# falcon-xu/DeViT

Measured on AMD Instinct MI355X. Metric: images/sec distill_sub step (DeiT-B->dedeit, bs256, 224^2), higher is better.
Workload: dtype bf16; 1 GPU; distill_sub step dedeit<-deit_base_distilled_patch16_224, num_division=4 (C=25), bs=256/GPU, 224x224, hard distillation, drop_path 0.1, AdamW+EMA; classes=25, global_batch=256, parallelism=dp1

## Files before the change

### devit_amd/_lib.py

```python
import ctypes as C
import os

import torch

_HERE = os.path.dirname(os.path.abspath(__file__))
LIB_PATH = os.environ.get("DEVIT_LIB_PATH") or os.path.join(_HERE, "libdevit_hip.so")

EPI_STORE_BF16, EPI_GELU_BF16, EPI_RESIDUAL_F32, EPI_PATCH_F32, EPI_DGELU_BF16, EPI_ATOMIC_F32, EPI_STORE_F32 = range(7)


class Epilogue(C.Structure):
    _fields_ = [("kind", C.c_int), ("out", C.c_void_p), ("ldc", C.c_int), ("bias", C.c_void_p),
                ("colscale", C.c_void_p), ("aux", C.c_void_p), ("aux_in", C.c_void_p), ("res", C.c_void_p),
                ("rowscale", C.c_void_p), ("rows_per_scale", C.c_int), ("pos", C.c_void_p),
                ("patch_tokens", C.c_int), ("extra_tokens", C.c_int), ("exact_gelu", C.c_int),
                ("out_batch_stride", C.c_longlong), ("m_valid", C.c_int), ("dtype16", C.c_int)]


class Operand(C.Structure):
    _fields_ = [("ptr", C.c_void_p), ("ld", C.c_int), ("kmajor", C.c_int), ("row_group", C.c_int),
                ("row_skip", C.c_int), ("batch_stride", C.c_longlong)]


ACT_LN1, ACT_MEAN1, ACT_RSTD1, ACT_QKV, ACT_ATTN_O, ACT_LSE, ACT_X1, ACT_ATT, ACT_LN2, ACT_MEAN2, ACT_RSTD2, ACT_H, ACT_H_PRE, \
    ACT_X2, ACT_COUNT = range(15)
BLK_SAVE, BLK_QKV_PAD, BLK_ATT = 1, 2, 4
BWD_DH_PRE, BWD_DLN2, BWD_DX1, BWD_G1, BWD_DATTN, BWD_DQKV, BWD_DLN1, BWD_LNWS, BWD_COUNT = range(9)


class BlockWeights(C.Structure):
    _fields_ = [(n, C.c_void_p) for n in ("n1w", "n1b", "qkv_b", "proj_b", "n2w", "n2b", "fc1_b", "fc2_b", "qkv_w16",
                                          "proj_w16", "fc1_w16", "fc2_w16", "head_gate", "neuron_gate")] + \
               [("num_heads", C.c_int), ("attn_width", C.c_int), ("hidden", C.c_int), ("dtype16", C.c_int), ("fc2_w16t", C.c_void_p)]


class BlockWgrads(C.Structure):
    _fields_ = [(n, C.c_void_p) for n in ("n1w", "n1b", "qkv_w", "qkv_b", "proj_w", "proj_b", "n2w", "n2b", "fc1_w",
                                          "fc1_b", "fc2_w", "fc2_b")]


class BlockActs(C.Structure):
    _fields_ = [("x", C.c_void_p), ("buf", C.c_void_p * 14), ("dp1", C.c_void_p), ("dp2", C.c_void_p), ("flags", C.c_int)]


class BlockBwdIO(C.Structure):
    _fields_ = [("dx", C.c_void_p), ("g2", C.c_void_p), ("dx_in", C.c_void_p), ("g_prev", C.c_void_p),
                ("prev_dp2", C.c_void_p), ("prev_fc2_b_grad", C.c_void_p), ("g2_bias_done", C.c_int),
                ("dqkv_add", C.c_void_p), ("ws", C.c_void_p * 8), ("lnws_bytes", C.c_size_t),
                ("defer_jobs", C.c_void_p), ("defer_count", C.c_void_p)]


class IndexJob(C.Structure):
    _fields_ = [("src", C.c_void_p), ("dst", C.c_void_p), ("idx", C.c_void_p), ("rows", C.c_int), ("cols", C.c_int),
                ("src_ld", C.c_int), ("dst_ld", C.c_int), ("mode", C.c_int), ("elem", C.c_int)]


class WgradJob(C.Structure):
    _fields_ = [("a", C.c_void_p), ("lda", C.c_int), ("a_cols", C.c_int), ("b", C.c_void_p), ("ldb", C.c_int), ("out", C.c_void_p),
                ("ldc", C.c_int), ("transposed", C.c_int), ("a_colsum", C.c_void_p)]


WGRAD_MAX_JOBS = 48
ABI_VERSION = 2
ABI_STRUCTS = {0: Epilogue, 1: Operand, 2: BlockWeights, 3: BlockWgrads, 4: BlockActs, 5: BlockBwdIO, 6: IndexJob, 7: WgradJob}


class DevitError(RuntimeError):
    pass


_P, _I, _F, _Z, _LL = C.c_void_p, C.c_int, C.c_float, C.c_size_t, C.c_longlong

SIGNATURES = {
    "devit_version": (_I, []),
    "devit_last_error": (C.c_char_p, []),
    "devit_check_device": (_I, [_I]),
    "devit_abi_struct_size": (_Z, [_I]),
    "devit_gemm_full_row_selected": (_I, [_I, _I, _I, _I]),
    "devit_wgrad_grouped": (_I, [C.POINTER(WgradJob), _I, _I, _I, _P]),
    "devit_gemm_bf16": (_I, [C.POINTER(Operand), C.POINTER(Operand), _I, _I, _I, _I, _I, C.POINTER(Epilogue), _P]),
    "devit_set_reserved_cus": (_I, [_I]),
    "devit_get_reserved_cus": (_I, []),
    "devit_layernorm_fwd": (_I, [_P, _I, _I, _I, _I, _P, _P, _F, _P, _P, _P, _P, _I, _P]),
    "devit_layernorm_bwd_workspace": (_Z, [_I, _I]),
    "devit_layernorm_bwd": (_I, [_P, _I, _P, _I, _I, _I, _I, _P, _P, _P, _P, _P, _P, _P, _I, _P, _P, _P, _I, _P, _Z, _P]),
    "devit_block_acts_sizes": (_I, [_I, _I, _I, _I, _I, _I, C.POINTER(C.c_size_t)]),
    "devit_block_bwd_sizes": (_I, [_I, _I, _I, _I, _I, C.POINTER(C.c_size_t)]),
    "devit_encoder_fwd": (_I, [_I, C.POINTER(BlockWeights), C.POINTER(BlockActs), _I, _I, _I, _F, _P]),
    "devit_block_bwd": (_I, [C.POINTER(BlockWeights), C.POINTER(BlockActs), C.POINTER(BlockWgrads), C.POINTER(BlockBwdIO),
                             _I, _I, _I, _F, _P]),
    "devit_attn_fwd": (_I, [_P, _P, _P, _P, _I, _I, _I, _I, _F, _I, _P]),
    "devit_attn_bwd": (_I, [_P, _P, _P, _P, _P, _P, _P, _I, _I, _I, _I, _F, _P]),
    "devit_attn_fwd_rows": (_I, [_P, _I, _P, _I, _P, _P, _P, _I, _I, _I, _I, _I, _F, _I, _P]),
    "devit_attn_bwd_rows": (_I, [_P, _I, _P, _I, _P, _P, _P, _P, _P, _I, _P, _I, _I, _I, _I, _I, _I, _F, _P]),
    "devit_index_copy": (_I, [_P, _I, _I, _P]),
    "devit_im2row_bf16": (_I, [_P, _P, _I, _I, _I, _I, _I, _I, _P]),
    "devit_mix_im2row_bf16": (_I, [_P, _P, _P, _I, _I, C.c_double, _I, _I, _I, _I, _P]),
    "devit_mix_targets": (_I, [_P, _P, _I, _I, C.c_double, C.c_double, _P]),
    "devit_embed_tokens": (_I, [_P, _P, _P, _P, _I, _I, _I, _P]),
    "devit_embed_bwd": (_I, [_P, _I, _I, _I, _I, _P, _P, _P, _P, _P, _I, _P]),
    "devit_cast_bf16": (_I, [_P, _P, _Z, _I, _P]),
    "devit_scale_cast_bf16": (_I, [_P, _P, _P, _I, _I, _I, _P]),
    "devit_colsum_workspace": (_Z, [_I, _I]),
    "devit_colsum_bf16": (_I, [_P, _I, _I, _I, _I, _I, _P, _I, _P, _Z, _P]),
    "devit_sgemm_small": (_I, [_P, _LL, _LL, _P, _LL, _LL, _P, _P, _I, _I, _I, _I, _F, _I, _P]),
    "devit_sumsq_workspace": (_Z, []),
    "devit_sumsq_f32": (_I, [_P, _Z, _P, _P, _Z, _P]),
    "devit_adamw_step": (_I, [_P, _P, _P, _P, _P, _P, _P, _P, _P, _Z, _F, _F, _F, _F, _F, _F, _F, _P]),
    "devit_cls_distill_loss": (_I, [_P, _P, _P, _P, _I, _I, _I, _F, _F, _P, _P, _P, _P]),
    "devit_token_mse": (_I, [_P, _P, _Z, _P, _P, _I, _P]),
    "devit_relation_stats": (_I, [_P, _P, _I, _I, _I, _I, _I, _P, _P, _P, _P, _P]),
    "devit_relation_grad": (_I, [_P, _P, _P, _P, _P, _I, _I, _I, _I, _I, _P, _I, _P]),
    "devit_gemm_f32": (_I, [_P, _LL, _LL, _LL, _LL, _P, _LL, _LL, _LL, _LL, _I, _I, _I, _I, _I, _LL, _LL, _I, _I, _F, _P, _I,
                            C.POINTER(Epilogue), _P]),
    "devit_softmax_rows_f32": (_I, [_P, _I, _I, _I, _F, _P, _P]),
    "devit_softmax_bwd_rows_f32": (_I, [_P, _P, _I, _I, _I, _F, _P]),
    "devit_im2row_f32": (_I, [_P, _P, _I, _P]),
    "devit_scale_rows_f32": (_I, [_P, _P, _P, _I, _I, _I, _P]),
    "devit_colsum_f32": (_I, [_P, _I, _I, _I, _P, _I, _P]),
    "devit_comm_unique_id": (_I, [_P]),
    "devit_comm_init": (_I, [_P, _I, _I, C.POINTER(C.c_void_p)]),
    "devit_comm_allreduce_f32": (_I, [_P, _P, _Z, _P]),
    "devit_comm_destroy": (_I, [_P]),
}

_lib = None
_checked_devices = set()


def load():
    global _lib
    if _lib is None:
        if not os.path.exists(LIB_PATH):
            raise DevitError(
                f"{LIB_PATH} not found: build it with `python -c 'import __graft_entry__ as g; g.build()'` "
                "(or devit_amd/csrc/build.sh).  devit_amd has no CPU / PyTorch fallback.")
        lib = C.CDLL(LIB_PATH)
        for name, (res, args) in SIGNATURES.items():
            fn = getattr(lib, name)
            fn.restype, fn.argtypes = res, args
        if lib.devit_version() != ABI_VERSION:
            raise DevitError(f"libdevit_hip.so ABI version {lib.devit_version()} != {ABI_VERSION} of this binding: rebuild (devit_amd/csrc/build.sh)")
        for which, cls in ABI_STRUCTS.items():
            if lib.devit_abi_struct_size(which) != C.sizeof(cls):
                raise DevitError(f"libdevit_hip.so: sizeof struct {which} = {lib.devit_abi_struct_size(which)}, the binding's {cls.__name__} has "
                                 f"{C.sizeof(cls)} bytes: header and binding disagree")
        _lib = lib
    return _lib


def require_device(t: torch.Tensor):
    if not t.is_cuda:
        raise DevitError("devit_amd ops run on MI355X (gfx950) only; got a %s tensor. There is no CPU fallback "
                         "(the CPU restatement lives in oracle/ and is test infrastructure)." % t.device)
    idx = t.device.index if t.device.index is not None else torch.cuda.current_device()
    if idx not in _checked_devices:
        call("devit_check_device", idx)
        _checked_devices.add(idx)


def call(name, *args):
    lib = load()
    rc = getattr(lib, name)(*args)
    if rc != 0:
        raise DevitError(f"{name} failed ({rc}): {lib.devit_last_error().decode()}")
    return rc


def stream_ptr():
    return C.c_void_p(torch.cuda.current_stream().cuda_stream)


def ptr(t):
    return None if t is None else C.c_void_p(t.data_ptr())
```

### devit_amd/csrc/devit_common.h

```cpp
#pragma once
#include <hip/hip_runtime.h>
#include <stdint.h>

#include "../../include/devit_hip.h"

typedef __attribute__((ext_vector_type(8))) __bf16 bf16x8;
typedef __attribute__((ext_vector_type(4))) __bf16 bf16x4;
typedef __attribute__((ext_vector_type(2))) __bf16 bf16x2;
typedef __attribute__((ext_vector_type(4))) short short4v;
typedef __attribute__((ext_vector_type(4))) float f32x4;
typedef __attribute__((ext_vector_type(2))) float f32x2;

#define LDS_PTR(p) ((__attribute__((address_space(3))) void*)(p))
#define GLB_PTR(p) ((const __attribute__((address_space(1))) void*)(p))

void devit_set_error(const char* fmt, ...);
#define DEVIT_CHECK(cond, code, ...)      \
  do {                                    \
    if (!(cond)) {                        \
      devit_set_error(__VA_ARGS__);       \
      return (code);                      \
    }                                     \
  } while (0)
#define DEVIT_LAUNCH_CHECK()                                            \
  do {                                                                  \
    hipError_t e__ = hipGetLastError();                                 \
    if (e__ != hipSuccess) {                                            \
      devit_set_error("%s:%d launch failed: %s", __FILE__, __LINE__,    \
                      hipGetErrorString(e__));                          \
      return DEVIT_ERR_LAUNCH;                                          \
    }                                                                   \
  } while (0)


__device__ __forceinline__ float bf2f(__bf16 v) { return (float)v; }
__device__ __forceinline__ __bf16 f2bf(float v) { return (__bf16)v; }

__device__ __forceinline__ float wave_sum(float v) {
#pragma unroll
  for (int o = 32; o > 0; o >>= 1) v += __shfl_xor(v, o, 64);
  return v;
}
__device__ __forceinline__ float wave_max(float v) {
#pragma unroll
  for (int o = 32; o > 0; o >>= 1) v = fmaxf(v, __shfl_xor(v, o, 64));
  return v;
}

constexpr float GELU_C0 = 1.59500523f, GELU_C1 = 7.40208836e-2f, GELU_C2 = -7.04591421e-4f;
constexpr float LOG2E = 1.44269504088896341f;
template <bool EXACT>
__device__ __forceinline__ float gelu_fwd(float x) {
  if (EXACT) return 0.5f * x * (1.0f + erff(x * 0.70710678118654752f));
  const float x2 = fminf(x * x, 36.0f);
  const float p = fmaf(fmaf(-GELU_C2 * LOG2E, x2, -GELU_C1 * LOG2E), x2, -GELU_C0 * LOG2E);
  const float t = __builtin_amdgcn_exp2f(x * p);
  return x * __builtin_amdgcn_rcpf(1.0f + t);
}
template <bool EXACT>
__device__ __forceinline__ float gelu_bwd(float x) {
  if (EXACT) {
    const float pdf = 0.3989422804014327f * __expf(-0.5f * x * x);
    return 0.5f * (1.0f + erff(x * 0.70710678118654752f)) + x * pdf;
  }
  const float x2 = fminf(x * x, 36.0f);
  const float p = fmaf(fmaf(-GELU_C2 * LOG2E, x2, -GELU_C1 * LOG2E), x2, -GELU_C0 * LOG2E);
  const float q = fmaf(fmaf(5.0f * GELU_C2, x2, 3.0f * GELU_C1), x2, GELU_C0);
  const float s = __builtin_amdgcn_rcpf(1.0f + __builtin_amdgcn_exp2f(x * p));
  return fmaf(x * fmaf(-s, s, s), q, s);
}

__device__ __forceinline__ void store16_stream(void* p, f32x4 v) { *(f32x4*)p = v; }
__device__ __forceinline__ void store8_stream(void* p, bf16x4 v) { *(bf16x4*)p = v; }
template <typename T>
__device__ __forceinline__ T load_stream(const T* p) {
  return __builtin_nontemporal_load(p);
}

__device__ __forceinline__ f32x4 mfma16(bf16x8 a, bf16x8 b, f32x4 c) {
  return __builtin_amdgcn_mfma_f32_16x16x32_bf16(a, b, c, 0, 0, 0);
}

typedef __attribute__((ext_vector_type(8))) _Float16 f16x8;
typedef __attribute__((ext_vector_type(4))) _Float16 f16x4;
template <bool F16>
__device__ __forceinline__ f32x4 mfma16t(bf16x8 a, bf16x8 b, f32x4 c) {
  if constexpr (F16)
    return __builtin_amdgcn_mfma_f32_16x16x32_f16(__builtin_bit_cast(f16x8, a), __builtin_bit_cast(f16x8, b), c, 0, 0, 0);
  else
    return __builtin_amdgcn_mfma_f32_16x16x32_bf16(a, b, c, 0, 0, 0);
}
template <bool F16>
__device__ __forceinline__ bf16x4 cvt4(f32x4 v) {
  if constexpr (F16) {
    const f16x4 h = {(_Float16)v[0], (_Float16)v[1], (_Float16)v[2], (_Float16)v[3]};
    return __builtin_bit_cast(bf16x4, h);
  } else {
    return (bf16x4){f2bf(v[0]), f2bf(v[1]), f2bf(v[2]), f2bf(v[3])};
  }
}
template <bool F16>
__device__ __forceinline__ bf16x8 cvt8(f32x4 a, f32x4 b) {
  if constexpr (F16) {
    const f16x8 h = {(_Float16)a[0], (_Float16)a[1], (_Float16)a[2], (_Float16)a[3],
                     (_Float16)b[0], (_Float16)b[1], (_Float16)b[2], (_Float16)b[3]};
    return __builtin_bit_cast(bf16x8, h);
  } else {
    return (bf16x8){f2bf(a[0]), f2bf(a[1]), f2bf(a[2]), f2bf(a[3]), f2bf(b[0]), f2bf(b[1]), f2bf(b[2]), f2bf(b[3])};
  }
}

template <typename V>
__device__ __forceinline__ void swap_half_rows(V& a, V& b, bool hi) {
  static_assert(sizeof(V) == 16, "16-byte chunks");
  typedef unsigned u32x4 __attribute__((ext_vector_type(4)));
  const u32x4 ua = __builtin_bit_cast(u32x4, a), ub = __builtin_bit_cast(u32x4, b);
  u32x4 recv;
#pragma unroll
  for (int e = 0; e < 4; ++e) {
    const unsigned send = hi ? ua[e] : ub[e];
    recv[e] = __builtin_amdgcn_update_dpp(0u, send, 0x128 , 0xf, 0xf, false);
  }
  u32x4 oa, obb;
#pragma unroll
  for (int e = 0; e < 4; ++e) {
    oa[e] = hi ? recv[e] : ua[e];
    obb[e] = hi ? ub[e] : recv[e];
  }
  a = __builtin_bit_cast(V, oa);
  b = __builtin_bit_cast(V, obb);
}

__device__ __forceinline__ bf16x4 lds_tr_read(const void* lds_addr) {
  short4v v = __builtin_amdgcn_ds_read_tr16_b64_v4i16((__attribute__((address_space(3))) short4v*)(lds_addr));
  return __builtin_bit_cast(bf16x4, v);
}
__device__ __forceinline__ bf16x8 cat8(bf16x4 lo, bf16x4 hi) {
  return __builtin_shufflevector(lo, hi, 0, 1, 2, 3, 4, 5, 6, 7);
}
```

### devit_amd/csrc/encoder.hip

```cpp
#include <mutex>

#include "devit_common.h"

namespace {

inline int pad_rows(int m) { return (m + 255) / 256 * 256; }
inline size_t align256(size_t b) { return (b + 255) / 256 * 256; }

inline int split_k_for(int out_rows, int out_cols, int ksteps) {
  const int tiles = (out_rows / 128) * (out_cols / 128);
  int s = 512 / (tiles > 0 ? tiles : 1);
  if (s > ksteps) s = ksteps;
  return s < 1 ? 1 : s;
}

struct Ctx {
  int M, Mp, B, N, D;
  float eps;
  void* stream;
};

int zero_pad(const Ctx& c, void* buf, int cols, size_t elem, int extra_rows = 0) {
  if (!buf) return DEVIT_OK;
  const int rows = c.Mp + extra_rows - c.M;
  if (rows <= 0) return DEVIT_OK;
  hipError_t e = hipMemsetAsync((char*)buf + (size_t)c.M * cols * elem, 0, (size_t)rows * cols * elem, (hipStream_t)c.stream);
  DEVIT_CHECK(e == hipSuccess, DEVIT_ERR_LAUNCH, "hipMemsetAsync: %s", hipGetErrorString(e));
  return DEVIT_OK;
}

devit_epilogue make_ep(int kind, void* out, int ldc, int m_valid, int dtype16 = 0) {
  devit_epilogue ep = {};
  ep.kind = kind;
  ep.out = out;
  ep.ldc = ldc;
  ep.m_valid = m_valid;
  ep.dtype16 = dtype16;
  return ep;
}

int linear_fwd(const Ctx& c, const void* x, const void* w, int Nout, int K, devit_epilogue ep) {
  devit_operand A = {x, K, 0, 0, 0, 0}, Bo = {w, K, 0, 0, 0, 0};
  return devit_gemm_bf16(&A, &Bo, c.Mp, Nout, K, 1, 1, &ep, c.stream);
}
int linear_dgrad(const Ctx& c, const void* dy, const void* w, int Nw, int K, devit_epilogue ep) {
  devit_operand A = {dy, Nw, 0, 0, 0, 0}, Bo = {w, K, 1, 0, 0, 0};
  return devit_gemm_bf16(&A, &Bo, c.Mp, K, Nw, 1, 1, &ep, c.stream);
}
int linear_wgrad(const Ctx& c, const void* dy, const void* x, float* w_grad, float* b_grad, int Nw, int K) {
  devit_operand A = {dy, Nw, 1, 0, 0, 0}, Bo = {x, K, 1, 0, 0, 0};
  devit_epilogue ep = make_ep(DEVIT_EPI_ATOMIC_F32, w_grad, K, 0);
  ep.aux = b_grad;
  return devit_gemm_bf16(&A, &Bo, Nw, K, c.Mp, 1, split_k_for(Nw, K, c.Mp / 64), &ep, c.stream);
}

bool wgrad_job(devit_wgrad_job* j, const void* dy, const void* x, float* w_grad, float* b_grad, int Nw, int K) {
  if (K == 384 && Nw % 128 == 0) {
    *j = devit_wgrad_job{dy, Nw, Nw, x, K, w_grad, K, 0, b_grad};
    return true;
  }
  if (Nw == 384 && K % 128 == 0 && b_grad == nullptr) {
    *j = devit_wgrad_job{x, K, K, dy, Nw, w_grad, K, 1, nullptr};
    return true;
  }
  return false;
}
int wgrad_mode() {
  const char* e = getenv("DEVIT_WGRADFR");
  return (e && *e) ? atoi(e) != 0 : 1;
}

#define TRY(x)                 \
  do {                         \
    int rc__ = (x);            \
    if (rc__ != DEVIT_OK) return rc__; \
  } while (0)

struct WgradSide {
  hipStream_t stream;
  hipEvent_t ev[5];
  bool ok = false;
};
constexpr int MAX_DEVICES = 16;
int wgrad_side(WgradSide** out) {
  const char* env = getenv("DEVIT_WGRAD_STREAM");
  const bool on = !(env && atoi(env) == 0);
  static WgradSide per_dev[MAX_DEVICES];
  static std::once_flag once[MAX_DEVICES];
  *out = nullptr;
  if (!on) return DEVIT_OK;
  int dev = 0;
  DEVIT_CHECK(hipGetDevice(&dev) == hipSuccess && dev >= 0, DEVIT_ERR_DEVICE, "devit_block_bwd: hipGetDevice");
  if (dev >= MAX_DEVICES) return DEVIT_OK;
  std::call_once(once[dev], [dev]() {
    WgradSide& s = per_dev[dev];
    if (hipStreamCreateWithFlags(&s.stream, hipStreamNonBlocking) != hipSuccess) return;
    for (auto& e : s.ev)
      if (hipEventCreateWithFlags(&e, hipEventDisableTiming) != hipSuccess) return;
    s.ok = true;
  });
  DEVIT_CHECK(per_dev[dev].ok, DEVIT_ERR_DEVICE, "devit_block_bwd: cannot create the weight-gradient stream / its events");
  *out = &per_dev[dev];
  return DEVIT_OK;
}

int check_dims(int B, int N, int D, int Da, int Hd) {
  DEVIT_CHECK(B > 0 && N > 0 && N <= 208 && D > 0 && D % 128 == 0 && Da > 0 && Da % 128 == 0 && Hd > 0 && Hd % 128 == 0,
              DEVIT_ERR_SHAPE, "block: B=%d N=%d D=%d attn_width=%d hidden=%d not supported", B, N, D, Da, Hd);
  return DEVIT_OK;
}

int block_fwd(const Ctx& c, const devit_block_weights& w, const devit_block_acts& a) {
  const int D = c.D, Da = w.attn_width, Hd = w.hidden, H = w.num_heads;
  TRY(check_dims(c.B, c.N, D, Da, Hd));
  DEVIT_CHECK(H > 0 && Da == H * 64, DEVIT_ERR_SHAPE, "block: attn_width %d != heads %d * 64", Da, H);
  const bool save = a.flags & DEVIT_BLK_SAVE;
  const int t16 = w.dtype16;
  DEVIT_CHECK(t16 == 0 || (t16 == 1 && !save), DEVIT_ERR_ARG,
              "devit_encoder_fwd: dtype16 = %d; f16 is the frozen-teacher forward (no DEVIT_BLK_SAVE: the backward kernels are bf16)", t16);
  void* const* b = a.buf;
  DEVIT_CHECK(a.x && b[DEVIT_ACT_LN1] && b[DEVIT_ACT_QKV] && b[DEVIT_ACT_ATTN_O] && b[DEVIT_ACT_X1] && b[DEVIT_ACT_LN2] &&
                  b[DEVIT_ACT_H] && b[DEVIT_ACT_X2],
              DEVIT_ERR_ARG, "devit_encoder_fwd: null activation buffer");
  DEVIT_CHECK(!save || (b[DEVIT_ACT_MEAN1] && b[DEVIT_ACT_RSTD1] && b[DEVIT_ACT_LSE] && b[DEVIT_ACT_MEAN2] &&
                        b[DEVIT_ACT_RSTD2] && b[DEVIT_ACT_H_PRE]),
              DEVIT_ERR_ARG, "devit_encoder_fwd: DEVIT_BLK_SAVE needs the mean/rstd/lse/h_pre buffers");
  DEVIT_CHECK(!(a.flags & DEVIT_BLK_ATT) || b[DEVIT_ACT_ATT], DEVIT_ERR_ARG, "devit_encoder_fwd: DEVIT_BLK_ATT needs att");
  TRY(zero_pad(c, b[DEVIT_ACT_LN1], D, 2));
  TRY(zero_pad(c, b[DEVIT_ACT_QKV], 3 * Da, 2, (a.flags & DEVIT_BLK_QKV_PAD) ? 128 : 0));
  TRY(zero_pad(c, b[DEVIT_ACT_ATTN_O], Da, 2));
  TRY(zero_pad(c, b[DEVIT_ACT_LN2], D, 2));
  TRY(zero_pad(c, b[DEVIT_ACT_H], Hd, 2));
  if (save) TRY(zero_pad(c, b[DEVIT_ACT_H_PRE], Hd, 2));
  TRY(devit_layernorm_fwd(a.x, c.M, D, 0, 0, w.n1w, w.n1b, c.eps, b[DEVIT_ACT_LN1], nullptr,
                          save ? (float*)b[DEVIT_ACT_MEAN1] : nullptr, save ? (float*)b[DEVIT_ACT_RSTD1] : nullptr, t16, c.stream));
  {
    devit_epilogue ep = make_ep(DEVIT_EPI_STORE_BF16, b[DEVIT_ACT_QKV], 3 * Da, c.M, t16);
    ep.bias = w.qkv_b;
    TRY(linear_fwd(c, b[DEVIT_ACT_LN1], w.qkv_w16, 3 * Da, D, ep));
  }
  TRY(devit_attn_fwd(b[DEVIT_ACT_QKV], b[DEVIT_ACT_ATTN_O], save ? (float*)b[DEVIT_ACT_LSE] : nullptr, w.head_gate, c.B, c.N, H,
                     64, 0.125f, t16, c.stream));
  {
    devit_epilogue ep = make_ep(DEVIT_EPI_RESIDUAL_F32, b[DEVIT_ACT_X1], D, c.M, t16);
    ep.bias = w.proj_b;
    ep.res = a.x;
    ep.rowscale = a.dp1;
    ep.rows_per_scale = c.N;
    ep.aux = (a.flags & DEVIT_BLK_ATT) ? b[DEVIT_ACT_ATT] : nullptr;
    TRY(linear_fwd(c, b[DEVIT_ACT_ATTN_O], w.proj_w16, D, Da, ep));
  }
  TRY(devit_layernorm_fwd((const float*)b[DEVIT_ACT_X1], c.M, D, 0, 0, w.n2w, w.n2b, c.eps, b[DEVIT_ACT_LN2], nullptr,
                          save ? (float*)b[DEVIT_ACT_MEAN2] : nullptr, save ? (float*)b[DEVIT_ACT_RSTD2] : nullptr, t16, c.stream));
  {
    devit_epilogue ep = make_ep(DEVIT_EPI_GELU_BF16, b[DEVIT_ACT_H], Hd, c.M, t16);
    ep.bias = w.fc1_b;
    ep.colscale = w.neuron_gate;
    ep.aux = save ? b[DEVIT_ACT_H_PRE] : nullptr;
    TRY(linear_fwd(c, b[DEVIT_ACT_LN2], w.fc1_w16, Hd, D, ep));
  }
  {
    devit_epilogue ep = make_ep(DEVIT_EPI_RESIDUAL_F32, b[DEVIT_ACT_X2], D, c.M, t16);
    ep.bias = w.fc2_b;
    ep.res = (const float*)b[DEVIT_ACT_X1];
    ep.rowscale = a.dp2;
    ep.rows_per_scale = c.N;
    if (w.fc2_w16t && !t16 && devit_gemm_full_row_selected(c.Mp, D, Hd, DEVIT_EPI_RESIDUAL_F32)) {
      devit_operand A = {b[DEVIT_ACT_H], Hd, 0, 0, 0, 0}, Bo = {w.fc2_w16t, D, 1, 0, 0, 0};
      TRY(devit_gemm_bf16(&A, &Bo, c.Mp, D, Hd, 1, 1, &ep, c.stream));
    } else {
      TRY(linear_fwd(c, b[DEVIT_ACT_H], w.fc2_w16, D, Hd, ep));
    }
  }
  return DEVIT_OK;
}

}

extern "C" int devit_block_acts_sizes(int B, int N, int D, int Da, int Hd, int flags, size_t* sizes) {
  DEVIT_CHECK(sizes != nullptr, DEVIT_ERR_ARG, "devit_block_acts_sizes: null");
  TRY(check_dims(B, N, D, Da, Hd));
  const size_t M = (size_t)B * N, Mp = pad_rows((int)M);
  const bool save = flags & DEVIT_BLK_SAVE;
  sizes[DEVIT_ACT_LN1] = Mp * D * 2;
  sizes[DEVIT_ACT_MEAN1] = sizes[DEVIT_ACT_RSTD1] = sizes[DEVIT_ACT_MEAN2] = sizes[DEVIT_ACT_RSTD2] = save ? M * 4 : 0;
  sizes[DEVIT_ACT_QKV] = (Mp + ((flags & DEVIT_BLK_QKV_PAD) ? 128 : 0)) * 3 * (size_t)Da * 2;
  sizes[DEVIT_ACT_ATTN_O] = Mp * Da * 2;
  sizes[DEVIT_ACT_LSE] = save ? (size_t)B * (Da / 64) * N * 4 : 0;
  sizes[DEVIT_ACT_X1] = M * D * 4;
  sizes[DEVIT_ACT_ATT] = (flags & DEVIT_BLK_ATT) ? M * D * 2 : 0;
  sizes[DEVIT_ACT_LN2] = Mp * D * 2;
  sizes[DEVIT_ACT_H] = Mp * Hd * 2;
  sizes[DEVIT_ACT_H_PRE] = save ? Mp * Hd * 2 : 0;
  sizes[DEVIT_ACT_X2] = M * D * 4;
  for (int i = 0; i < DEVIT_ACT_COUNT; ++i) sizes[i] = align256(sizes[i]);
  return DEVIT_OK;
}

extern "C" int devit_block_bwd_sizes(int B, int N, int D, int Da, int Hd, size_t* sizes) {
  DEVIT_CHECK(sizes != nullptr, DEVIT_ERR_ARG, "devit_block_bwd_sizes: null");
  TRY(check_dims(B, N, D, Da, Hd));
  const size_t M = (size_t)B * N, Mp = pad_rows((int)M);
  sizes[DEVIT_BWD_DH_PRE] = Mp * Hd * 2;
  sizes[DEVIT_BWD_DLN2] = sizes[DEVIT_BWD_G1] = sizes[DEVIT_BWD_DLN1] = Mp * D * 2;
  sizes[DEVIT_BWD_DATTN] = Mp * (size_t)Da * 2;
  sizes[DEVIT_BWD_DX1] = M * D * 4;
  sizes[DEVIT_BWD_DQKV] = Mp * 3 * (size_t)Da * 2;
  sizes[DEVIT_BWD_LNWS] = devit_layernorm_bwd_workspace((int)M, D);
  for (int i = 0; i < DEVIT_BWD_COUNT; ++i) sizes[i] = align256(sizes[i]);
  return DEVIT_OK;
}

extern "C" int devit_encoder_fwd(int nblocks, const devit_block_weights* w, const devit_block_acts* acts, int B, int N, int D,
                                 float eps, void* stream) {
  DEVIT_CHECK(nblocks > 0 && w && acts, DEVIT_ERR_ARG, "devit_encoder_fwd: bad argument");
  Ctx c{B * N, pad_rows(B * N), B, N, D, eps, stream};
  for (int i = 0; i < nblocks; ++i) {
    DEVIT_CHECK(i == 0 || acts[i].x == (const float*)acts[i - 1].buf[DEVIT_ACT_X2], DEVIT_ERR_ARG,
                "devit_encoder_fwd: block %d does not read block %d's output", i, i - 1);
    TRY(block_fwd(c, w[i], acts[i]));
  }
  return DEVIT_OK;
}

extern "C" int devit_block_bwd(const devit_block_weights* wp, const devit_block_acts* ap, const devit_block_wgrads* gp,
                               const devit_block_bwd_io* io, int B, int N, int D, float eps, void* stream) {
  DEVIT_CHECK(wp && ap && gp && io, DEVIT_ERR_ARG, "devit_block_bwd: null argument");
  const devit_block_weights& w = *wp;
  const devit_block_acts& a = *ap;
  const devit_block_wgrads& g = *gp;
  const int Hd = w.hidden, H = w.num_heads, Da = w.attn_width;
  TRY(check_dims(B, N, D, Da, Hd));
  DEVIT_CHECK(H > 0 && Da == H * 64, DEVIT_ERR_SHAPE, "devit_block_bwd: attn_width %d != heads %d * 64", Da, H);
  DEVIT_CHECK(a.flags & DEVIT_BLK_SAVE, DEVIT_ERR_ARG, "devit_block_bwd: the forward ran without DEVIT_BLK_SAVE");
  DEVIT_CHECK(w.dtype16 == 0, DEVIT_ERR_ARG, "devit_block_bwd: f16 blocks have no backward");
  DEVIT_CHECK(io->dx && io->g2 && io->dx_in, DEVIT_ERR_ARG, "devit_block_bwd: dx / g2 / dx_in");
  for (int i = 0; i < DEVIT_BWD_COUNT; ++i) DEVIT_CHECK(io->ws[i], DEVIT_ERR_ARG, "devit_block_bwd: workspace %d is null", i);
  DEVIT_CHECK(g.n1w && g.n1b && g.qkv_w && g.qkv_b && g.proj_w && g.proj_b && g.n2w && g.n2b && g.fc1_w && g.fc1_b &&
                  g.fc2_w && g.fc2_b, DEVIT_ERR_ARG, "devit_block_bwd: null gradient accumulator");
  Ctx c{B * N, pad_rows(B * N), B, N, D, eps, stream};
  WgradSide* sd = nullptr;
  TRY(wgrad_side(&sd));
  Ctx cs = c;
  bool forked = false;
  auto fork = [&](int i) -> int {
    if (!sd) return DEVIT_OK;
    DEVIT_CHECK(hipEventRecord(sd->ev[i], (hipStream_t)stream) == hipSuccess && hipStreamWaitEvent(sd->stream, sd->ev[i], 0) == hipSuccess,
                DEVIT_ERR_LAUNCH, "devit_block_bwd: cannot fork the weight-gradient stream");
    cs.stream = sd->stream;
    forked = true;
    return DEVIT_OK;
  };
  const int rc = [&]() -> int {
  void* const* b = a.buf;
  void* dh_pre = io->ws[DEVIT_BWD_DH_PRE];
  void* dln2 = io->ws[DEVIT_BWD_DLN2];
  float* dx1 = (float*)io->ws[DEVIT_BWD_DX1];
  void* g1 = io->ws[DEVIT_BWD_G1];
  void* dattn = io->ws[DEVIT_BWD_DATTN];
  void* dqkv = io->ws[DEVIT_BWD_DQKV];
  void* dln1 = io->ws[DEVIT_BWD_DLN1];
  TRY(zero_pad(c, dh_pre, Hd, 2));
  TRY(zero_pad(c, dln2, D, 2));
  TRY(zero_pad(c, g1, D, 2));
  TRY(zero_pad(c, dattn, Da, 2));
  TRY(zero_pad(c, dqkv, 3 * Da, 2));
  TRY(zero_pad(c, dln1, D, 2));
  TRY(zero_pad(c, io->g_prev, D, 2));
  const int wmode = (D == 384 && c.Mp / 64 >= 3) ? wgrad_mode() : 0;
  if (io->defer_count) *io->defer_count = 0;
  devit_wgrad_job jobs[4];
  int nj = 0;
  auto wgrad = [&](int ev, const void* dy, const void* x, float* w_grad, float* b_grad, int Nw, int K) -> int {
    if (wmode && wgrad_job(&jobs[nj], dy, x, w_grad, b_grad, Nw, K)) {
      ++nj;
      return DEVIT_OK;
    }
    TRY(fork(ev));
    return linear_wgrad(cs, dy, x, w_grad, b_grad, Nw, K);
  };
  auto flush = [&](int ev) -> int {
    if (io->defer_jobs) {
      for (int i = 0; i < nj; ++i) io->defer_jobs[i] = jobs[i];
      if (io->defer_count) *io->defer_count = nj;
      nj = 0;
      return DEVIT_OK;
    }
    if (nj == 0) return DEVIT_OK;
    TRY(fork(ev));
    const int n = nj;
    nj = 0;
    return devit_wgrad_grouped(jobs, n, c.Mp, 0, cs.stream);
  };
  bool fc2_bias_here = !io->g2_bias_done;
  if (fc2_bias_here && wmode && Hd % 128 == 0 && io->lnws_bytes >= devit_colsum_workspace(c.Mp, D)) {
    TRY(devit_colsum_bf16(io->g2, c.Mp, D, D, 0, 0, g.fc2_b, 1, io->ws[DEVIT_BWD_LNWS], io->lnws_bytes, stream));
    fc2_bias_here = false;
  }
  TRY(wgrad(0, io->g2, b[DEVIT_ACT_H], g.fc2_w, fc2_bias_here ? g.fc2_b : nullptr, D, Hd));
  {
    devit_epilogue ep = make_ep(DEVIT_EPI_DGELU_BF16, dh_pre, Hd, c.M);
    ep.colscale = w.neuron_gate;
    ep.aux_in = b[DEVIT_ACT_H_PRE];
    TRY(linear_dgrad(c, io->g2, w.fc2_w16, D, Hd, ep));
  }
  TRY(linear_dgrad(c, dh_pre, w.fc1_w16, Hd, D, make_ep(DEVIT_EPI_STORE_BF16, dln2, D, c.M)));
  TRY(wgrad(1, dh_pre, b[DEVIT_ACT_LN2], g.fc1_w, g.fc1_b, Hd, D));
  TRY(devit_layernorm_bwd(dln2, 0, (const float*)b[DEVIT_ACT_X1], c.M, D, 0, 0, (const float*)b[DEVIT_ACT_MEAN2],
                          (const float*)b[DEVIT_ACT_RSTD2], w.n2w, io->dx, dx1, g1, a.dp1, N, g.n2w, g.n2b, g.proj_b, 1,
                          io->ws[DEVIT_BWD_LNWS], io->lnws_bytes, stream));
  TRY(linear_dgrad(c, g1, w.proj_w16, D, Da, make_ep(DEVIT_EPI_STORE_BF16, dattn, Da, c.M)));
  TRY(wgrad(2, g1, b[DEVIT_ACT_ATTN_O], g.proj_w, nullptr, D, Da));
  TRY(devit_attn_bwd(b[DEVIT_ACT_QKV], b[DEVIT_ACT_ATTN_O], dattn, (const float*)b[DEVIT_ACT_LSE], w.head_gate, io->dqkv_add,
                     dqkv, B, N, H, 64, 0.125f, stream));
  TRY(linear_dgrad(c, dqkv, w.qkv_w16, 3 * Da, D, make_ep(DEVIT_EPI_STORE_BF16, dln1, D, c.M)));
  TRY(wgrad(3, dqkv, b[DEVIT_ACT_LN1], g.qkv_w, g.qkv_b, 3 * Da, D));
  TRY(flush(3));
  TRY(devit_layernorm_bwd(dln1, 0, a.x, c.M, D, 0, 0, (const float*)b[DEVIT_ACT_MEAN1], (const float*)b[DEVIT_ACT_RSTD1],
                          w.n1w, dx1, io->dx_in, io->g_prev, io->prev_dp2, N, g.n1w, g.n1b,
                          io->g_prev ? io->prev_fc2_b_grad : nullptr, 1, io->ws[DEVIT_BWD_LNWS], io->lnws_bytes, stream));
  return DEVIT_OK;
  }();
  if (sd && forked) {
    const bool joined = hipEventRecord(sd->ev[4], sd->stream) == hipSuccess && hipStreamWaitEvent((hipStream_t)stream, sd->ev[4], 0) == hipSuccess;
    if (rc == DEVIT_OK) DEVIT_CHECK(joined, DEVIT_ERR_LAUNCH, "devit_block_bwd: cannot join the weight-gradient stream");
  }
  return rc;
}
```

### devit_amd/csrc/gemm.hip

```cpp
#include <stdlib.h>

#include <type_traits>

#include "devit_common.h"

namespace {

constexpr int BK = 64;
#ifndef DEVIT_PP_SPREAD
#define DEVIT_PP_SPREAD 0
#endif
#ifndef DEVIT_PP_SPLIT
#define DEVIT_PP_SPLIT 1
#endif
#ifndef DEVIT_PP_MFMA_AT
#define DEVIT_PP_MFMA_AT 1
#endif
#ifdef DEVIT_DMA_A_NT
constexpr bool DMA_A_NT = true;
#else
constexpr bool DMA_A_NT = false;
#endif
#ifdef DEVIT_DMA_B_NT
constexpr bool DMA_B_NT = true;
#else
constexpr bool DMA_B_NT = false;
#endif
#ifndef DEVIT_RAGGED_MIN_K
#define DEVIT_RAGGED_MIN_K 384
#endif

struct FastDiv {
  unsigned mul, shift;
  int d;
};
__host__ inline FastDiv make_fastdiv(int d) {
  FastDiv f;
  f.d = d;
  unsigned s = 0;
  while ((1ll << s) < d) ++s;
  f.shift = 31 + s;
  f.mul = (unsigned)(((1ull << f.shift) / (unsigned long long)d) + 1ull);
  return f;
}
__device__ __forceinline__ int fdiv(int n, const FastDiv& f) {
  return (int)(((unsigned long long)(unsigned)n * f.mul) >> f.shift);
}

struct GemmArgs {
  const __bf16* A;
  const __bf16* B;
  int lda, ldb;
  int a_group, a_skip, b_group, b_skip;
  long long a_bs, b_bs;
  int M, N, K;
  int tiles_m, tiles_n, split_k, total_tiles;
  FastDiv d_per_z, d_chunk, d_gn, d_last, d_split;
  int gn;
  devit_epilogue ep;
};

__device__ __forceinline__ int phys_row(int r, int group, int skip) {
  return group > 0 ? r + skip * (r / group + 1) : r;
}

__device__ __forceinline__ int swz_row(int row) { return ((row >> 1) & 7) ^ (((row >> 4) & 1) << 1); }
__device__ __forceinline__ int swz_krow(int krow) { return ((krow & 3) << 2) | (((krow >> 3) & 1) << 1); }

template <bool KM, int W, int NWAVES>
__device__ __forceinline__ unsigned lane_offset(int ld, int wave, int lane, int i, int valid) {
  constexpr int CNT = (W / 8) / NWAVES;
  const int slab = wave * CNT + i;
  if (!KM) {
    const int row = slab * 8 + (lane >> 3);
    const int chunk = (lane & 7) ^ swz_row(row);
    return (unsigned)(min(row, valid - 1) * ld + chunk * 8) * 2u;
  } else {
    constexpr int LPR = W / 8, RPS = 64 / LPR;
    const int krow = slab * RPS + lane / LPR;
    const int chunk = (lane % LPR) ^ swz_krow(krow);
    return (unsigned)(krow * ld + min(chunk, valid / 8 - 1) * 8) * 2u;
  }
}

template <bool NT = false>
__device__ __forceinline__ void dma2_uniform(const char* ubase, unsigned off0, unsigned off1, unsigned lds) {
  unsigned keep;
  if (NT) {
    asm volatile(
        "s_mov_b32 %0, m0\n\t"
        "s_mov_b32 m0, %1\n\t"
        "s_nop 2\n\t"
        "global_load_lds_dwordx4 %3, %2 nt\n\t"
        "s_add_u32 m0, %1, 0x400\n\t"
        "s_nop 0\n\t"
        "global_load_lds_dwordx4 %4, %2 nt\n\t"
        "s_mov_b32 m0, %0"
        : "=&s"(keep)
        : "s"(lds), "s"(ubase), "v"(off0), "v"(off1)
        : "memory", "scc");
    return;
  }
  asm volatile(
      "s_mov_b32 %0, m0\n\t"
      "s_mov_b32 m0, %1\n\t"
      "s_nop 2\n\t"
      "global_load_lds_dwordx4 %3, %2\n\t"
      "s_add_u32 m0, %1, 0x400\n\t"
      "s_nop 0\n\t"
      "global_load_lds_dwordx4 %4, %2\n\t"
      "s_mov_b32 m0, %0"
      : "=&s"(keep)
      : "s"(lds), "s"(ubase), "v"(off0), "v"(off1)
      : "memory", "scc");
}
__device__ __forceinline__ void dma2_perlane(const void* p0, const void* p1, unsigned lds) {
  unsigned keep;
  asm volatile(
      "s_mov_b32 %0, m0\n\t"
      "s_mov_b32 m0, %1\n\t"
      "s_nop 2\n\t"
      "global_load_lds_dwordx4 %2, off\n\t"
      "s_add_u32 m0, %1, 0x400\n\t"
      "s_nop 0\n\t"
      "global_load_lds_dwordx4 %3, off\n\t"
      "s_mov_b32 m0, %0"
      : "=&s"(keep)
      : "s"(lds), "v"(p0), "v"(p1)
      : "memory", "scc");
}

template <bool KM, int W, int NWAVES, bool NT = false>
__device__ __forceinline__ void stage_tile(const __bf16* org, int ld, int k0, int group, int skip,
                                           char* lds_tile, int wave, int lane, int valid = W, int only_pair = -1) {
  constexpr int CNT = (W / 8) / NWAVES;
  static_assert(CNT % 2 == 0, "slabs are issued in pairs");
  const unsigned lds0 = (unsigned)(size_t)LDS_PTR(lds_tile) + (unsigned)(wave * CNT) * 1024u;
  if (KM && group > 0) {
#pragma unroll
    for (int i = 0; i < CNT; i += 2) {
      const __bf16* src[2];
#pragma unroll
      for (int e = 0; e < 2; ++e) {
        constexpr int LPR = W / 8, RPS = 64 / LPR;
        const int slab = wave * CNT + i + e;
        const int krow = slab * RPS + lane / LPR;
        const int chunk = (lane % LPR) ^ swz_krow(krow);
        src[e] = org + (size_t)phys_row(k0 + krow, group, skip) * ld + chunk * 8;
      }
      dma2_perlane(src[0], src[1], lds0 + i * 1024u);
    }
    return;
  }
  const char* ubase = (const char*)org + (size_t)k0 * (KM ? (size_t)ld : (size_t)1) * 2;
#pragma unroll
  for (int i = 0; i < CNT; i += 2)
    if (only_pair < 0 || i == 2 * only_pair)
    dma2_uniform<NT>(ubase, lane_offset<KM, W, NWAVES>(ld, wave, lane, i, valid), lane_offset<KM, W, NWAVES>(ld, wave, lane, i + 1, valid),
                     lds0 + i * 1024u);
}

template <bool PAIRED>
__device__ __forceinline__ int tile_row(int j, int p) {
  return PAIRED ? 32 * (j >> 1) + 8 * (p >> 2) + 4 * (j & 1) + (p & 3) : 16 * j + p;
}

template <bool KM, int W, bool PAIRED>
__device__ __forceinline__ bf16x8 read_frag(const char* tile, int base, int j, int kk, int lane) {
  if (!KM) {
    const int row = base + tile_row<PAIRED>(j, lane & 15);
#ifdef DEVIT_GEMM_NOSWZ
    const int chunk = (kk * 4 + (lane >> 4));
#else
    const int chunk = (kk * 4 + (lane >> 4)) ^ swz_row(row);
#endif
    return *(const bf16x8*)(tile + row * 128 + chunk * 16);
  } else {
    const int G = lane >> 4, q = (lane >> 2) & 3, p = lane & 3;
    const int col0 = base + tile_row<PAIRED>(j, 4 * p);
    const int krow = kk * 32 + G * 8 + q;
    const int chunk = (col0 >> 3) ^ swz_krow(krow);
    const char* a = tile + krow * (W * 2) + chunk * 16 + ((col0 >> 2) & 1) * 8;
    return cat8(lds_tr_read(a), lds_tr_read(a + 4 * (W * 2)));
  }
}

template <int N>
__device__ __forceinline__ void wait_vmcnt() {
  asm volatile("s_waitcnt vmcnt(%0)" ::"n"(N) : "memory");
}

template <typename T>
__device__ __forceinline__ void st_out(T* p, T v) {
#ifdef DEVIT_GEMM_NOSTORE
  if (__builtin_expect(((size_t)p & 0xfffff0) == 0x7ffff0, 0))
#endif
  *p = v;
}

template <bool F16 = false>
__device__ __forceinline__ bf16x8 pack8(const float (&x)[8]) {
  if constexpr (F16) return cvt8<true>((f32x4){x[0], x[1], x[2], x[3]}, (f32x4){x[4], x[5], x[6], x[7]});
  typedef float f32x2 __attribute__((ext_vector_type(2)));
  typedef __bf16 bf16x2 __attribute__((ext_vector_type(2)));
  bf16x2 p[4];
#pragma unroll
  for (int e = 0; e < 4; ++e) p[e] = __builtin_convertvector((f32x2){x[2 * e], x[2 * e + 1]}, bf16x2);
  return (bf16x8){p[0][0], p[0][1], p[1][0], p[1][1], p[2][0], p[2][1], p[3][0], p[3][1]};
}

template <int KIND>
__device__ __forceinline__ void load_cols(const devit_epilogue& ep, int lane, int nw, int (&noff)[4], f32x4 (&bias)[4],
                                          f32x4 (&cs)[4]) {
  constexpr bool BF16_OUT = KIND == DEVIT_EPI_STORE_BF16 || KIND == DEVIT_EPI_GELU_BF16 || KIND == DEVIT_EPI_DGELU_BF16;
  constexpr bool SCALED = KIND == DEVIT_EPI_GELU_BF16 || KIND == DEVIT_EPI_DGELU_BF16;
#pragma unroll
  for (int j = 0; j < 4; ++j) {
    noff[j] = nw + tile_row<BF16_OUT>(j, 4 * (lane >> 4));
    if constexpr (KIND == DEVIT_EPI_DGELU_BF16) bias[j] = (f32x4){0.f, 0.f, 0.f, 0.f};
    else bias[j] = ep.bias ? *(const f32x4*)(ep.bias + noff[j]) : (f32x4){0.f, 0.f, 0.f, 0.f};
    if (SCALED) cs[j] = ep.colscale ? *(const f32x4*)(ep.colscale + noff[j]) : (f32x4){1.f, 1.f, 1.f, 1.f};
  }
}
template <int KIND>
__device__ __forceinline__ void settle_cols(f32x4 (&bias)[4], f32x4 (&cs)[4]) {
  constexpr bool SCALED = KIND == DEVIT_EPI_GELU_BF16 || KIND == DEVIT_EPI_DGELU_BF16;
#pragma unroll
  for (int j = 0; j < 4; ++j) {
    if (KIND != DEVIT_EPI_DGELU_BF16) asm volatile("" : "+v"(bias[j]));
    if (SCALED) asm volatile("" : "+v"(cs[j]));
  }
}

#ifndef DEVIT_F32_FULL_ROWS
#define DEVIT_F32_FULL_ROWS 1
#endif

template <int KIND, int MI, bool FULL, bool F16>
__device__ __forceinline__ void epilogue_f32_rows(const devit_epilogue& ep, f32x4 (&acc)[MI][4], const int (&noff)[4],
                                                  const f32x4 (&bias)[4], int lane, int mw, int m_lim, size_t ob) {
  constexpr int CHI = 2;
  const int c = lane & 15;
  const bool hi = c >= 8;
  const int colx = hi ? 16 : 0;
  auto row_off = [&](int m, int& tok) -> size_t {
    if (KIND == DEVIT_EPI_PATCH_F32) {
      const int b = m / ep.patch_tokens, t = m - b * ep.patch_tokens;
      tok = ep.extra_tokens + t;
      return ((size_t)b * (ep.patch_tokens + ep.extra_tokens) + tok) * ep.ldc;
    }
    tok = 0;
    return ob + (size_t)m * ep.ldc;
  };
#pragma unroll
  for (int i0 = 0; i0 < MI; i0 += CHI) {
    f32x4 gin[CHI][2][2];
    float rsc[CHI][2];
    size_t rowo[CHI][2];
    bool okr[CHI][2];
#pragma unroll
    for (int u = 0; u < CHI; ++u)
#pragma unroll
      for (int r = 0; r < 2; ++r) {
        const int m = mw + (i0 + u) * 16 + (c & 7) + 8 * r;
        const bool ok = FULL || m < m_lim;
        int tok;
        const size_t o = row_off(m, tok);
#pragma unroll
        for (int p = 0; p < 2; ++p) {
          const int col = noff[2 * p] + colx;
          if (KIND == DEVIT_EPI_PATCH_F32)
            gin[u][p][r] = ok ? *(const f32x4*)(ep.pos + (size_t)tok * ep.ldc + col) : (f32x4){0.f, 0.f, 0.f, 0.f};
          if (KIND == DEVIT_EPI_RESIDUAL_F32)
            gin[u][p][r] = ok ? load_stream((const f32x4*)(ep.res + o + col)) : (f32x4){0.f, 0.f, 0.f, 0.f};
        }
        if (KIND == DEVIT_EPI_RESIDUAL_F32) rsc[u][r] = (ok && ep.rowscale) ? ep.rowscale[m / ep.rows_per_scale] : 1.0f;
        rowo[u][r] = o;
        okr[u][r] = ok;
      }
#pragma unroll
    for (int u = 0; u < CHI; ++u) {
      const int i = i0 + u;
      f32x4 v[4];
#pragma unroll
      for (int j = 0; j < 4; ++j) v[j] = acc[i][j] + bias[j];
      if (KIND == DEVIT_EPI_RESIDUAL_F32 && ep.aux) {
        const int m = mw + i * 16 + c;
        if (FULL || m < m_lim) {
#pragma unroll
          for (int j = 0; j < 4; ++j) st_out((bf16x4*)((__bf16*)ep.aux + ob + (size_t)m * ep.ldc + noff[j]), cvt4<F16>(v[j]));
        }
      }
#pragma unroll
      for (int p = 0; p < 2; ++p) {
        swap_half_rows(v[2 * p], v[2 * p + 1], hi);
        const int col = noff[2 * p] + colx;
#pragma unroll
        for (int r = 0; r < 2; ++r) {
          f32x4 w = v[2 * p + r];
          if (KIND == DEVIT_EPI_PATCH_F32) w = w + gin[u][p][r];
          if (KIND == DEVIT_EPI_RESIDUAL_F32) w = gin[u][p][r] + rsc[u][r] * w;
          if (okr[u][r]) st_out((f32x4*)((float*)ep.out + rowo[u][r] + col), w);
        }
      }
    }
  }
}

template <int KIND, int MI, bool FULL, bool F16 = false>
__device__ __forceinline__ void epilogue_direct(const devit_epilogue& ep, f32x4 (&acc)[MI][4], const int (&noff)[4],
                                                const f32x4 (&bias)[4], const f32x4 (&cs)[4], int lane, int mw,
                                                int m_lim, size_t ob) {
  constexpr bool BF16_OUT = KIND == DEVIT_EPI_STORE_BF16 || KIND == DEVIT_EPI_GELU_BF16 || KIND == DEVIT_EPI_DGELU_BF16;
  if constexpr (!BF16_OUT && DEVIT_F32_FULL_ROWS) {
    epilogue_f32_rows<KIND, MI, FULL, F16>(ep, acc, noff, bias, lane, mw, m_lim, ob);
    return;
  }
  constexpr int CHI = 2;
  const int c = lane & 15;
#pragma unroll
  for (int i0 = 0; i0 < MI; i0 += CHI) {
    f32x4 gin[CHI][4];
    float rsc[CHI];
    bf16x8 pre[CHI][2];
    size_t rowo[CHI];
#pragma unroll
    for (int u = 0; u < CHI; ++u) {
      const int m = mw + (i0 + u) * 16 + c;
      const bool ok = FULL || m < m_lim;
      size_t o = ob + (size_t)m * ep.ldc;
      if (KIND == DEVIT_EPI_PATCH_F32) {
        const int b = m / ep.patch_tokens, t = m - b * ep.patch_tokens, tok = ep.extra_tokens + t;
        o = ((size_t)b * (ep.patch_tokens + ep.extra_tokens) + tok) * ep.ldc;
#pragma unroll
        for (int j = 0; j < 4; ++j)
          gin[u][j] = ok ? *(const f32x4*)(ep.pos + (size_t)tok * ep.ldc + noff[j]) : (f32x4){0.f, 0.f, 0.f, 0.f};
      }
      if (KIND == DEVIT_EPI_RESIDUAL_F32) {
#pragma unroll
        for (int j = 0; j < 4; ++j)
          gin[u][j] = ok ? load_stream((const f32x4*)(ep.res + o + noff[j])) : (f32x4){0.f, 0.f, 0.f, 0.f};
        rsc[u] = (ok && ep.rowscale) ? ep.rowscale[m / ep.rows_per_scale] : 1.0f;
      }
      if (KIND == DEVIT_EPI_DGELU_BF16) {
        const bf16x8 z = {0, 0, 0, 0, 0, 0, 0, 0};
#pragma unroll
        for (int q = 0; q < 2; ++q)
          pre[u][q] = ok ? load_stream((const bf16x8*)((const __bf16*)ep.aux_in + o + noff[2 * q])) : z;
      }
      rowo[u] = o;
    }
#pragma unroll
    for (int u = 0; u < CHI; ++u) {
      const int i = i0 + u;
      const bool ok = FULL || mw + i * 16 + c < m_lim;
      const size_t o = rowo[u];
      if constexpr (!BF16_OUT) {
#pragma unroll
        for (int j = 0; j < 4; ++j) {
          const f32x4 v = acc[i][j] + bias[j];
          if (KIND == DEVIT_EPI_STORE_F32) {
            if (ok) st_out((f32x4*)((float*)ep.out + o + noff[j]), v);
          } else if (KIND == DEVIT_EPI_PATCH_F32) {
            if (ok) st_out((f32x4*)((float*)ep.out + o + noff[j]), v + gin[u][j]);
          } else {
            if (ok) {
              if (ep.aux) {
                const bf16x4 pb = cvt4<F16>(v);
                st_out((bf16x4*)((__bf16*)ep.aux + o + noff[j]), pb);
              }
              st_out((f32x4*)((float*)ep.out + o + noff[j]), gin[u][j] + rsc[u] * v);
            }
          }
        }
      } else {
        bf16x8 outc[2], prec[2];
#pragma unroll
        for (int q = 0; q < 2; ++q) {
          float x[8];
#pragma unroll
          for (int e = 0; e < 8; ++e) x[e] = acc[i][2 * q + (e >> 2)][e & 3] + bias[2 * q + (e >> 2)][e & 3];
          if (KIND == DEVIT_EPI_GELU_BF16) {
            prec[q] = pack8<F16>(x);
#pragma unroll
            for (int e = 0; e < 8; ++e) x[e] = gelu_fwd<false>(x[e]) * cs[2 * q + (e >> 2)][e & 3];
          } else if (KIND == DEVIT_EPI_DGELU_BF16) {
#pragma unroll
            for (int e = 0; e < 8; ++e) x[e] = x[e] * cs[2 * q + (e >> 2)][e & 3] * gelu_bwd<false>(bf2f(pre[u][q][e]));
          }
          outc[q] = pack8<F16>(x);
        }
        const bool hi = c >= 8;
        const int mA = mw + i * 16 + (c & 7);
        const size_t oA = ob + (size_t)mA * ep.ldc + noff[0] + (hi ? 32 : 0), oB = oA + (size_t)8 * ep.ldc;
        const bool okA = FULL || mA < m_lim, okB = FULL || mA + 8 < m_lim;
        swap_half_rows(outc[0], outc[1], hi);
        if (KIND == DEVIT_EPI_GELU_BF16 && ep.aux) {
          swap_half_rows(prec[0], prec[1], hi);
          if (okA) st_out((bf16x8*)((__bf16*)ep.aux + oA), prec[0]);
          if (okB) st_out((bf16x8*)((__bf16*)ep.aux + oB), prec[1]);
        }
        if (okA) st_out((bf16x8*)((__bf16*)ep.out + oA), outc[0]);
        if (okB) st_out((bf16x8*)((__bf16*)ep.out + oB), outc[1]);
      }
    }
  }
}

__device__ __forceinline__ float sum8_bf16(bf16x8 v, float acc) {
  typedef __bf16 bf16x2v __attribute__((ext_vector_type(2)));
  const bf16x2v one = {(__bf16)1.0f, (__bf16)1.0f};
  acc = __builtin_amdgcn_fdot2_f32_bf16(__builtin_shufflevector(v, v, 0, 1), one, acc, false);
  acc = __builtin_amdgcn_fdot2_f32_bf16(__builtin_shufflevector(v, v, 2, 3), one, acc, false);
  acc = __builtin_amdgcn_fdot2_f32_bf16(__builtin_shufflevector(v, v, 4, 5), one, acc, false);
  acc = __builtin_amdgcn_fdot2_f32_bf16(__builtin_shufflevector(v, v, 6, 7), one, acc, false);
  return acc;
}

struct TileRef {
  const __bf16* a;
  const __bf16* b;
  int m0, n0, bz, kt0, nk;
};

template <int BM, int BN, bool A_KM, bool B_KM>
__device__ __forceinline__ TileRef decode_tile(const GemmArgs& g, int w) {
  const int zz = fdiv(w, g.d_per_z);
  const int r0 = w - zz * g.d_per_z.d;
  const int chunk = fdiv(r0, g.d_chunk);
  const int r1 = r0 - chunk * g.d_chunk.d;
  const bool lastc = (chunk + 1) * g.gn > g.tiles_n;
  const int tm = lastc ? fdiv(r1, g.d_last) : fdiv(r1, g.d_gn);
  const int tn = chunk * g.gn + r1 - tm * (lastc ? g.d_last.d : g.d_gn.d);
  const int bzq = fdiv(zz, g.d_split);
  const int z = zz - bzq * g.split_k, nk_total = g.K / BK;
  TileRef t;
  t.bz = bzq;
  t.m0 = tm * BM;
  t.n0 = tn * BN;
  t.kt0 = fdiv(z * nk_total, g.d_split);
  t.nk = fdiv((z + 1) * nk_total, g.d_split) - t.kt0;
  t.a = g.A + (size_t)t.bz * g.a_bs + (A_KM ? (size_t)t.m0 : (size_t)t.m0 * g.lda);
  t.b = g.B + (size_t)t.bz * g.b_bs + (B_KM ? (size_t)t.n0 : (size_t)t.n0 * g.ldb);
  return t;
}

template <int BM, int BN, int WAVES_M, int WAVES_N, int NSTAGE, bool A_KM, bool B_KM, int KIND, bool F16 = false>
__global__ __launch_bounds__(WAVES_M * WAVES_N * 64) __attribute__((amdgpu_waves_per_eu(2, 2)))
void gemm_kernel(const GemmArgs g) {
  static_assert(!F16 || (KIND != DEVIT_EPI_DGELU_BF16 && KIND != DEVIT_EPI_ATOMIC_F32 && !A_KM && !B_KM),
                "f16 operands: forward layouts / epilogues only (the frozen teacher has no backward)");
  extern __shared__ __attribute__((aligned(16))) char smem[];
  constexpr int NWAVES = WAVES_M * WAVES_N;
  constexpr int WM = BM / WAVES_M, WN = BN / WAVES_N, MI = WM / 16, NI = WN / 16;
  static_assert(WN == 64 && WM % 64 == 0, "wave tile must be (64 k) x 64");
  static_assert(NSTAGE == 2, "NSTAGE is the B ring depth; uniformly deeper rings at one workgroup per CU lost everywhere");
  constexpr bool DIRECT = KIND != DEVIT_EPI_ATOMIC_F32;
  constexpr bool PAIRED = KIND == DEVIT_EPI_STORE_BF16 || KIND == DEVIT_EPI_GELU_BF16 || KIND == DEVIT_EPI_DGELU_BF16;
  constexpr int A_TILE_BYTES = BM * BK * 2, B_TILE_BYTES = BN * BK * 2;
  constexpr bool PP = DIRECT && BM == 256 && BN == 256 && WAVES_M == 2;
  constexpr int NA = 3;
  constexpr int PER_A = (BM / 8) / NWAVES;
  constexpr int B_RING = NA * A_TILE_BYTES;
  const int tid = threadIdx.x, lane = tid & 63;
  const int wave = __builtin_amdgcn_readfirstlane(tid >> 6);
  const int wm = wave / WAVES_N, wn = wave % WAVES_N;
#ifdef DEVIT_GEMM_TSTAMP
  const unsigned long long t_entry = __builtin_amdgcn_s_memtime(), rt_entry = __builtin_amdgcn_s_memrealtime();
#endif

  const int xcd = blockIdx.x & 7, idx = blockIdx.x >> 3, stride = gridDim.x >> 3;
  int first, last;
  {
    const int q = g.total_tiles >> 3, r = g.total_tiles & 7;
    const int start = xcd * q + min(xcd, r);
    first = start + idx;
    last = start + q + (xcd < r ? 1 : 0);
  }
  if (first >= last) return;

  struct Cursor {
    TileRef ref;
    int tile, t;
    bool open;
  };
  Cursor pb{decode_tile<BM, BN, A_KM, B_KM>(g, first), first, 0, true};
  Cursor pa = pb;
  int a_slot = 0, b_slot = 0;
  bool a_last = false;
  auto step_cursor = [&](Cursor& c) {
    if (++c.t == c.ref.nk) {
      c.t = 0;
      c.tile += stride;
      if (DIRECT && c.tile < last) c.ref = decode_tile<BM, BN, A_KM, B_KM>(g, c.tile);
      else c.open = false;
    }
  };
  auto dma_a = [&](const Cursor& c) {
#ifdef DEVIT_GEMM_NODMA
    if (g.K < 0)
#endif
    stage_tile<A_KM, BM, NWAVES, DMA_A_NT>(c.ref.a, g.lda, (c.ref.kt0 + c.t) * BK, g.a_group, g.a_skip,
                                           smem + a_slot * A_TILE_BYTES, wave, lane);
    a_slot = a_slot + 1 == NA ? 0 : a_slot + 1;
  };
  auto dma_b = [&](const Cursor& c) {
#ifdef DEVIT_GEMM_NODMA
    if (g.K < 0)
#endif
    stage_tile<B_KM, BN, NWAVES, DMA_B_NT>(c.ref.b, g.ldb, (c.ref.kt0 + c.t) * BK, g.b_group, g.b_skip,
                                           smem + B_RING + b_slot * B_TILE_BYTES, wave, lane, min(BN, g.N - c.ref.n0));
    b_slot ^= 1;
  };
  auto issue_a = [&]() {
    a_last = pa.open;
    if (!pa.open) return;
    dma_a(pa);
    step_cursor(pa);
  };
  auto produce = [&]() {
    if (pb.open) {
      dma_b(pb);
      step_cursor(pb);
    }
    issue_a();
  };
  auto wait_stage = [&]() {
    if (a_last) wait_vmcnt<PER_A>();
    else wait_vmcnt<0>();
  };
  if constexpr (PP) {
    auto fence = [&]() {
      asm volatile("" ::: "memory");
      __builtin_amdgcn_sched_barrier(0);
    };
    auto bar = [&]() {
      fence();
      __builtin_amdgcn_s_barrier();
      fence();
    };
    issue_a();
    produce();
    wait_vmcnt<0>();
    bar();
#if DEVIT_PP_SPREAD
    auto dma_half = [&](Cursor& c, bool is_a, int h) {
      if (is_a) {
        stage_tile<A_KM, BM, NWAVES, DMA_A_NT>(c.ref.a, g.lda, (c.ref.kt0 + c.t) * BK, g.a_group, g.a_skip,
                                               smem + a_slot * A_TILE_BYTES, wave, lane, BM, h);
        if (h == 1) a_slot = a_slot + 1 == NA ? 0 : a_slot + 1;
      } else {
        stage_tile<B_KM, BN, NWAVES, DMA_B_NT>(c.ref.b, g.ldb, (c.ref.kt0 + c.t) * BK, g.b_group, g.b_skip,
                                               smem + B_RING + b_slot * B_TILE_BYTES, wave, lane, min(BN, g.N - c.ref.n0), h);
        if (h == 1) b_slot ^= 1;
      }
      if (h == 1) step_cursor(c);
    };
    auto slot_q = [&](auto qc) {
      constexpr int q = decltype(qc)::value;
      if (q == 0) { if (pb.open) dma_half(pb, false, 0); }
      if (q == 1) { if (pb.open) dma_half(pb, false, 1); }
      if (q == 2) { a_last = pa.open; if (pa.open) dma_half(pa, true, 0); }
      if (q == 3) { if (pa.open) dma_half(pa, true, 1); wait_stage(); }
    };
    auto spread_slot = [&](auto pc) {
      constexpr int p = decltype(pc)::value;
      if (wm == 0) slot_q(std::integral_constant<int, p>());
      else slot_q(std::integral_constant<int, (p + 1) & 3>());
    };
    if (wm == 1) slot_q(std::integral_constant<int, 0>());
#endif
    int ca_slot = 0, cb_slot = 0;
#ifdef DEVIT_GEMM_TSTAMP
    unsigned long long* tdbg = g.ep.pos ? (unsigned long long*)g.ep.pos + ((size_t)blockIdx.x * NWAVES + wave) * 48 : nullptr;
    int tcount = 0;
    if (tdbg && lane == 0) {
      tdbg[40] = t_entry;
      tdbg[42] = rt_entry;
      tdbg[44] = __builtin_amdgcn_s_memtime();
    }
#endif
    for (int tile = first; tile < last; tile += stride) {
      const TileRef ct = decode_tile<BM, BN, A_KM, B_KM>(g, tile);
      f32x4 acc[MI][NI];
#pragma unroll
      for (int i = 0; i < MI; ++i)
#pragma unroll
        for (int j = 0; j < NI; ++j) acc[i][j] = (f32x4){0.f, 0.f, 0.f, 0.f};
      const devit_epilogue& ep = g.ep;
      const int nw = ct.n0 + wn * WN;
#ifdef DEVIT_GEMM_TSTAMP
      if (tdbg && lane == 0 && tcount < 8) tdbg[tcount * 3 + 0] = __builtin_amdgcn_s_memtime();
#endif
      int noff[4];
      f32x4 bias[4], cs[4];
#ifdef DEVIT_GEMM_STAMP
      unsigned long long stamp[12];
#pragma unroll
      for (int q = 0; q < 12; ++q) stamp[q] = 0;
#define DEVIT_STAMP(q) do { if (t == 3 && tile == first) stamp[q] = __builtin_amdgcn_s_memtime(); } while (0)
#else
#define DEVIT_STAMP(q) do { } while (0)
#endif
      if (wm == 1) bar();
      for (int t = 0; t < ct.nk; ++t) {
        const char* cur_a = smem + ca_slot * A_TILE_BYTES;
        const char* cur_b = smem + B_RING + cb_slot * B_TILE_BYTES;
        ca_slot = ca_slot + 1 == NA ? 0 : ca_slot + 1;
        cb_slot ^= 1;
#if !DEVIT_PP_SPREAD && !DEVIT_PP_SPLIT
        produce();
#endif
        if (t == ct.nk - 1 && nw < g.N) load_cols<KIND>(ep, lane, nw, noff, bias, cs);
#pragma unroll
        for (int kk = 0; kk < 2; ++kk) {
          bf16x8 af[MI], bfr[NI];
#ifdef DEVIT_GEMM_NOREAD
#pragma unroll
          for (int j = 0; j < NI; ++j) asm volatile("" : "=v"(bfr[j]));
#pragma unroll
          for (int i = 0; i < MI; ++i) asm volatile("" : "=v"(af[i]));
#else
#pragma unroll
          for (int j = 0; j < NI; ++j) bfr[j] = read_frag<B_KM, BN, PAIRED>(cur_b, wn * WN, j, kk, lane);
#pragma unroll
          for (int i = 0; i < MI; ++i) af[i] = read_frag<A_KM, BM, false>(cur_a, wm * WM, i, kk, lane);
#endif
          DEVIT_STAMP(kk * 6 + 0);
#if DEVIT_PP_SPREAD
          fence();
          if (kk == 0) spread_slot(std::integral_constant<int, 0>());
          else spread_slot(std::integral_constant<int, 2>());
          fence();
#elif DEVIT_PP_SPLIT
          fence();
          if (kk == 0) {
            if (pb.open) {
              dma_b(pb);
              step_cursor(pb);
            }
          } else {
            issue_a();
            wait_stage();
          }
          fence();
#else
          if (kk == 1) wait_stage();
#endif
          DEVIT_STAMP(kk * 6 + 1);
          asm volatile("s_waitcnt lgkmcnt(0)" ::: "memory");
          DEVIT_STAMP(kk * 6 + 2);
          bar();
          DEVIT_STAMP(kk * 6 + 3);
#ifdef DEVIT_GEMM_NOMFMA
#pragma unroll
          for (int j = 0; j < NI; ++j) asm volatile("" ::"v"(bfr[j]));
#pragma unroll
          for (int i = 0; i < MI; ++i) asm volatile("" ::"v"(af[i]));
#else
#pragma unroll
          for (int i = 0; i < MI; ++i) {
#pragma unroll
            for (int j = 0; j < NI; ++j) acc[i][j] = mfma16t<F16>(bfr[j], af[i], acc[i][j]);
#if DEVIT_PP_SPREAD
            if (i == DEVIT_PP_MFMA_AT) {
              fence();
              if (kk == 0) spread_slot(std::integral_constant<int, 1>());
              else spread_slot(std::integral_constant<int, 3>());
              fence();
            }
#endif
          }
#endif
          DEVIT_STAMP(kk * 6 + 4);
          bar();
          DEVIT_STAMP(kk * 6 + 5);
        }
#ifdef DEVIT_GEMM_TSTAMP
        if (tdbg && lane == 0 && tcount == 1 && t < 16 && (g.M & 1)) tdbg[24 + t] = __builtin_amdgcn_s_memtime();
#endif
      }
#ifdef DEVIT_GEMM_TSTAMP
      if (tdbg && lane == 0 && tcount < 8) tdbg[tcount * 3 + 1] = __builtin_amdgcn_s_memtime();
#endif
      if (wm == 0) bar();
#ifdef DEVIT_GEMM_STAMP
      if (tile == first && lane == 0 && g.ep.pos != nullptr) {
        unsigned long long* dbg = (unsigned long long*)g.ep.pos + ((size_t)blockIdx.x * NWAVES + wave) * 12;
#pragma unroll
        for (int q = 0; q < 12; ++q) dbg[q] = stamp[q];
      }
#endif
      if (nw < g.N) {
        settle_cols<KIND>(bias, cs);
        const size_t ob = (size_t)ct.bz * ep.out_batch_stride;
        const int m_lim = ep.m_valid > 0 ? ep.m_valid : g.M;
        if (ct.m0 + BM <= m_lim) epilogue_direct<KIND, MI, true, F16>(ep, acc, noff, bias, cs, lane, ct.m0 + wm * WM, m_lim, ob);
        else epilogue_direct<KIND, MI, false, F16>(ep, acc, noff, bias, cs, lane, ct.m0 + wm * WM, m_lim, ob);
      }
#ifdef DEVIT_GEMM_TSTAMP
      if (tdbg && lane == 0 && tcount < 8) tdbg[tcount * 3 + 2] = __builtin_amdgcn_s_memtime();
      ++tcount;
#endif
    }
#ifdef DEVIT_GEMM_TSTAMP
    if (tdbg && lane == 0) {
      tdbg[41] = __builtin_amdgcn_s_memtime();
      tdbg[43] = __builtin_amdgcn_s_memrealtime();
      tdbg[45] = tcount;
    }
#endif
    return;
  }

  issue_a();
  produce();

  auto advance = [&]() {
    wait_stage();
    __builtin_amdgcn_s_barrier();
    produce();
  };

  int ca_slot = 0, cb_slot = 0;
  bool primed = false;
  for (int tile = first; tile < last; tile += stride) {
    const TileRef ct = decode_tile<BM, BN, A_KM, B_KM>(g, tile);
    f32x4 acc[MI][NI];
#pragma unroll
    for (int i = 0; i < MI; ++i)
#pragma unroll
      for (int j = 0; j < NI; ++j) acc[i][j] = (f32x4){0.f, 0.f, 0.f, 0.f};
    float rsum[MI];
#pragma unroll
    for (int i = 0; i < MI; ++i) rsum[i] = 0.f;
    const bool rowsum_on = KIND == DEVIT_EPI_ATOMIC_F32 && g.ep.aux != nullptr && wn == 0;
    int rs_wait = 0;
    if (rowsum_on) rs_wait = (ct.n0 / BN - ct.kt0 % g.tiles_n + g.tiles_n) % g.tiles_n;

    auto kstep = [&]() {
      const char* cur_a = smem + ca_slot * A_TILE_BYTES;
      const char* cur_b = smem + B_RING + cb_slot * B_TILE_BYTES;
      ca_slot = ca_slot + 1 == NA ? 0 : ca_slot + 1;
      cb_slot ^= 1;
      const bool rs_now = KIND == DEVIT_EPI_ATOMIC_F32 && rowsum_on && rs_wait == 0;
#ifdef DEVIT_GEMM_NOCOMPUTE
      if (g.K < 0)
#endif
#pragma unroll
      for (int kk = 0; kk < 2; ++kk) {
        bf16x8 af[MI], bfr[NI];
#pragma unroll
        for (int j = 0; j < NI; ++j) bfr[j] = read_frag<B_KM, BN, PAIRED>(cur_b, wn * WN, j, kk, lane);
#pragma unroll
        for (int i = 0; i < MI; ++i) af[i] = read_frag<A_KM, BM, false>(cur_a, wm * WM, i, kk, lane);
#pragma unroll
        for (int i = 0; i < MI; ++i)
#pragma unroll
          for (int j = 0; j < NI; ++j)
            acc[i][j] = DIRECT ? mfma16t<F16>(bfr[j], af[i], acc[i][j]) : mfma16t<F16>(af[i], bfr[j], acc[i][j]);
        if constexpr (KIND == DEVIT_EPI_ATOMIC_F32) {
          if (rs_now) {
#pragma unroll
            for (int i = 0; i < MI; ++i) rsum[i] = sum8_bf16(af[i], rsum[i]);
          }
        }
      }
      if constexpr (KIND == DEVIT_EPI_ATOMIC_F32) rs_wait = rs_wait == 0 ? g.tiles_n - 1 : rs_wait - 1;
    };
    const devit_epilogue& ep = g.ep;
    const int nw = ct.n0 + wn * WN;
    for (int t = 0; t < ct.nk - 1; ++t) {
      if (t > 0 || !primed) advance();
      kstep();
    }
    if (ct.nk > 1 || !primed) advance();
    int noff[4];
    f32x4 bias[4], cs[4];
    if constexpr (DIRECT) load_cols<KIND>(ep, lane, nw, noff, bias, cs);
    kstep();
    if constexpr (DIRECT) settle_cols<KIND>(bias, cs);
    primed = DIRECT && tile + stride < last;
    if (primed) advance();

    const size_t ob = (size_t)ct.bz * ep.out_batch_stride;
    const int m_lim = ep.m_valid > 0 ? ep.m_valid : g.M;
    if constexpr (DIRECT) {
      if (ct.m0 + BM <= m_lim) epilogue_direct<KIND, MI, true, F16>(ep, acc, noff, bias, cs, lane, ct.m0 + wm * WM, m_lim, ob);
      else epilogue_direct<KIND, MI, false, F16>(ep, acc, noff, bias, cs, lane, ct.m0 + wm * WM, m_lim, ob);
    } else {
      __syncthreads();
      float* cw = (float*)smem + wave * 4096;
      float* out = (float*)ep.out + ob;
      auto do_pass = [&](auto pass_c) {
        constexpr int pass = decltype(pass_c)::value;
#pragma unroll
        for (int i = 0; i < 4; ++i)
#pragma unroll
          for (int j = 0; j < 4; ++j)
#pragma unroll
            for (int r = 0; r < 4; ++r)
              cw[(i * 16 + (lane >> 4) * 4 + r) * 64 + j * 16 + (lane & 15)] = acc[pass * 4 + i][j][r];
        const int mw = ct.m0 + wm * WM + pass * 64;
        for (int row = 0; row < 64; ++row) {
          const float v = cw[row * 64 + lane];
#if defined(DEVIT_GEMM_NOATOMIC)
          if (mw + row < m_lim && v == 1.2345e30f) out[(size_t)(mw + row) * ep.ldc + nw + lane] = v;
#else
          if (mw + row < m_lim) unsafeAtomicAdd(out + (size_t)(mw + row) * ep.ldc + nw + lane, v);
#endif
        }
      };
      do_pass(std::integral_constant<int, 0>());
      if constexpr (MI > 4) do_pass(std::integral_constant<int, 1>());
      if (rowsum_on) {
        float* rs_out = (float*)ep.aux;
#pragma unroll
        for (int i = 0; i < MI; ++i) {
          float v = rsum[i];
          v += __shfl_xor(v, 16, 64);
          v += __shfl_xor(v, 32, 64);
          const int row = ct.m0 + wm * WM + i * 16 + lane;
          if (lane < 16 && row < m_lim) unsafeAtomicAdd(rs_out + row, v);
        }
      }
      if (pb.tile < last) {
        __syncthreads();
        pb.ref = decode_tile<BM, BN, A_KM, B_KM>(g, pb.tile);
        pb.t = 0;
        pb.open = true;
        pa = pb;
        a_slot = ca_slot;
        b_slot = cb_slot;
        issue_a();
        produce();
      }
    }
  }
}

#include "gemm4_kloop.inc"

template <int KIND, bool F16>
__global__ __launch_bounds__(256) __attribute__((amdgpu_waves_per_eu(1, 1)))
void gemm4_kernel(const GemmArgs g) {
  static_assert(KIND != DEVIT_EPI_ATOMIC_F32 && KIND != DEVIT_EPI_DGELU_BF16 && !F16, "forward layouts, DIRECT epilogues, bf16");
  extern __shared__ __attribute__((aligned(16))) char smem[];
  constexpr int BM = 256, BN = 256, NWAVES = 4;
  constexpr bool PAIRED = KIND == DEVIT_EPI_STORE_BF16 || KIND == DEVIT_EPI_GELU_BF16;
  constexpr int A_TILE_BYTES = BM * BK * 2, B_TILE_BYTES = BN * BK * 2, B_RING = 3 * A_TILE_BYTES;
  const int tid = threadIdx.x, lane = tid & 63;
  const int wave = __builtin_amdgcn_readfirstlane(tid >> 6);
  const int wm = wave >> 1, wn = wave & 1;

  const int xcd = blockIdx.x & 7, idx = blockIdx.x >> 3, stride = gridDim.x >> 3;
  int first, last;
  {
    const int q = g.total_tiles >> 3, r = g.total_tiles & 7;
    const int start = xcd * q + min(xcd, r);
    first = start + idx;
    last = start + q + (xcd < r ? 1 : 0);
  }
  if (first >= last) return;
#ifdef DEVIT_GEMM4_STAMP
  const unsigned long long t_entry = __builtin_amdgcn_s_memtime(), rt_entry = __builtin_amdgcn_s_memrealtime();
  unsigned long long st_sum[8] = {0, 0, 0, 0, 0, 0, 0, 0};
#endif

  const unsigned lda64 = (unsigned)g.lda * 64u, ldb64 = (unsigned)g.ldb * 64u;
  const unsigned wave_lds = (unsigned)(size_t)LDS_PTR(smem) + (unsigned)wave * 8192u;

  TileRef ct = decode_tile<BM, BN, false, false>(g, first);
#pragma unroll
  for (int st = 0; st < 2; ++st) {
    stage_tile<false, BM, NWAVES>(ct.a, g.lda, (ct.kt0 + st) * BK, 0, 0, smem + st * A_TILE_BYTES, wave, lane);
    stage_tile<false, BN, NWAVES>(ct.b, g.ldb, (ct.kt0 + st) * BK, 0, 0, smem + B_RING + st * B_TILE_BYTES, wave, lane);
  }
  wait_vmcnt<0>();
  __builtin_amdgcn_s_barrier();
  asm volatile("" ::: "memory");
  unsigned g3 = 0, g2 = B_RING;
  const unsigned wv = (unsigned)wave;

  for (int tile = first; tile < last; tile += stride) {
    const bool has_next = tile + stride < last;
    const TileRef nt = has_next ? decode_tile<BM, BN, false, false>(g, tile + stride) : ct;
    const __bf16* a_ptr = ct.a + (size_t)ct.kt0 * BK;
    const __bf16* b_ptr = ct.b + (size_t)ct.kt0 * BK;
    const __bf16* a_next = nt.a + (size_t)nt.kt0 * BK;
    const __bf16* b_next = nt.b + (size_t)nt.kt0 * BK;
    const unsigned nk = (unsigned)ct.nk;
    const devit_epilogue& ep = g.ep;
    unsigned dsA[4], dsB[4], dmaA[4], dmaB[4];
    {
      int lane_k;
      asm volatile("v_mbcnt_lo_u32_b32 %0, -1, 0\n\tv_mbcnt_hi_u32_b32 %0, -1, %0" : "=v"(lane_k));
      const int c = lane_k & 15, gq = lane_k >> 4;
  #pragma unroll
      for (int kk = 0; kk < 2; ++kk)
  #pragma unroll
        for (int par = 0; par < 2; ++par) {
          const int rowA = wm * 128 + 16 * par + c;
          dsA[kk * 2 + par] = (unsigned)(rowA * 128 + (((kk * 4 + gq) ^ swz_row(rowA)) * 16));
          const int rowB = wn * 128 + tile_row<PAIRED>(par, c);
          dsB[kk * 2 + par] = (unsigned)(rowB * 128 + (((kk * 4 + gq) ^ swz_row(rowB)) * 16));
        }
  #pragma unroll
      for (int i = 0; i < 4; ++i) {
        dmaA[i] = lane_offset<false, BM, NWAVES>(g.lda, wave, lane_k, i, BM);
        dmaB[i] = lane_offset<false, BN, NWAVES>(g.ldb, wave, lane_k, i, BN);
      }
    }
    unsigned t0, t1, t2, t3;
#ifdef DEVIT_GEMM4_STAMP
    unsigned d0, d1, d2, d3;
    const unsigned long long ts0 = __builtin_amdgcn_s_memtime();
    asm volatile(DEVIT_GEMM4_KLOOP_STAMPED_ASM
                 : [g3] "+s"(g3), [g2] "+s"(g2), [t0] "=&v"(t0), [t1] "=&v"(t1), [t2] "=&v"(t2), [t3] "=&v"(t3),
                   [d0] "=&s"(d0), [d1] "=&s"(d1), [d2] "=&s"(d2), [d3] "=&s"(d3)
                 : [aptr] "s"(a_ptr), [bptr] "s"(b_ptr), [anext] "s"(a_next), [bnext] "s"(b_next), [nk] "s"(nk),
                   [lda64] "s"(lda64), [ldb64] "s"(ldb64), [wlds] "s"(wave_lds), [wv] "s"(wv),
                   [dsa0] "v"(dsA[0]), [dsa1] "v"(dsA[1]), [dsa2] "v"(dsA[2]), [dsa3] "v"(dsA[3]),
                   [dsb0] "v"(dsB[0]), [dsb1] "v"(dsB[1]), [dsb2] "v"(dsB[2]), [dsb3] "v"(dsB[3]),
                   [dmaa0] "v"(dmaA[0]), [dmaa1] "v"(dmaA[1]), [dmaa2] "v"(dmaA[2]), [dmaa3] "v"(dmaA[3]),
                   [dmab0] "v"(dmaB[0]), [dmab1] "v"(dmaB[1]), [dmab2] "v"(dmaB[2]), [dmab3] "v"(dmaB[3])
                 : DEVIT_GEMM4_KLOOP_STAMPED_CLOBBERS);
    const unsigned long long ts1 = __builtin_amdgcn_s_memtime();
    st_sum[0] += 1; st_sum[1] += ts1 - ts0; st_sum[3] += d0; st_sum[4] += d1; st_sum[5] += d2; st_sum[6] += d3;
    if (tile == first) st_sum[7] = ts1 - ts0;
#else
    asm volatile(DEVIT_GEMM4_KLOOP_ASM
                 : [g3] "+s"(g3), [g2] "+s"(g2), [t0] "=&v"(t0), [t1] "=&v"(t1), [t2] "=&v"(t2), [t3] "=&v"(t3)
                 : [aptr] "s"(a_ptr), [bptr] "s"(b_ptr), [anext] "s"(a_next), [bnext] "s"(b_next), [nk] "s"(nk),
                   [lda64] "s"(lda64), [ldb64] "s"(ldb64), [wlds] "s"(wave_lds), [wv] "s"(wv),
                   [dsa0] "v"(dsA[0]), [dsa1] "v"(dsA[1]), [dsa2] "v"(dsA[2]), [dsa3] "v"(dsA[3]),
                   [dsb0] "v"(dsB[0]), [dsb1] "v"(dsB[1]), [dsb2] "v"(dsB[2]), [dsb3] "v"(dsB[3]),
                   [dmaa0] "v"(dmaA[0]), [dmaa1] "v"(dmaA[1]), [dmaa2] "v"(dmaA[2]), [dmaa3] "v"(dmaA[3]),
                   [dmab0] "v"(dmaB[0]), [dmab1] "v"(dmaB[1]), [dmab2] "v"(dmaB[2]), [dmab3] "v"(dmaB[3])
                 : DEVIT_GEMM4_KLOOP_CLOBBERS);
#endif
    int lane_e;
    asm volatile("v_mbcnt_lo_u32_b32 %0, -1, 0\n\tv_mbcnt_hi_u32_b32 %0, -1, %0" : "=v"(lane_e));
    int noff[2][4];
    f32x4 bias[2][4], cs[2][4];
#pragma unroll
    for (int h = 0; h < 2; ++h) load_cols<KIND>(ep, lane_e, ct.n0 + wn * 128 + h * 64, noff[h], bias[h], cs[h]);
    const size_t ob = (size_t)ct.bz * ep.out_batch_stride;
    const int m_lim = ep.m_valid > 0 ? ep.m_valid : g.M;
    const bool full = ct.m0 + BM <= m_lim;
    auto chunk = [&](auto hc, auto ic) {
      constexpr int H = decltype(hc)::value, I0 = decltype(ic)::value;
      f32x4 acc[2][4];
      gemm4_read_acc<H, I0>(acc);
      const int mw = ct.m0 + wm * 128 + I0 * 16;
      if (full) epilogue_direct<KIND, 2, true, F16>(ep, acc, noff[H], bias[H], cs[H], lane_e, mw, m_lim, ob);
      else epilogue_direct<KIND, 2, false, F16>(ep, acc, noff[H], bias[H], cs[H], lane_e, mw, m_lim, ob);
    };
    auto half = [&](auto hc) {
      chunk(hc, std::integral_constant<int, 0>());
      chunk(hc, std::integral_constant<int, 2>());
      chunk(hc, std::integral_constant<int, 4>());
      chunk(hc, std::integral_constant<int, 6>());
    };
    half(std::integral_constant<int, 0>());
    half(std::integral_constant<int, 1>());
#ifdef DEVIT_GEMM4_STAMP
    st_sum[2] += __builtin_amdgcn_s_memtime() - ts1;
#endif
    ct = nt;
  }
  wait_vmcnt<0>();
#ifdef DEVIT_GEMM4_STAMP
  if (g.ep.pos && KIND != DEVIT_EPI_PATCH_F32 && lane == 0) {
    unsigned long long* dbg = (unsigned long long*)g.ep.pos + ((size_t)blockIdx.x * NWAVES + wave) * 16;
#pragma unroll
    for (int q = 0; q < 8; ++q) dbg[q] = st_sum[q];
    dbg[8] = t_entry; dbg[9] = __builtin_amdgcn_s_memtime(); dbg[10] = rt_entry; dbg[11] = __builtin_amdgcn_s_memrealtime();
  }
#endif
}

#include "gemmfr_kloop.inc"

typedef float f32x32 __attribute__((ext_vector_type(32)));

__device__ __forceinline__ unsigned fr_dma_off_b(int ld, int wave, int lane, int i) {
  const int piece = (wave * 12 + i) * 64 + lane, krow = piece / 48, c = piece % 48;
  return (unsigned)((krow - 16 * wave) * ld + ((c ^ swz_krow(krow)) * 8)) * 2u;
}

__device__ __forceinline__ int fr_b_row(int u, int wave, int K) {
  const int r = 64 * u - 32 + 16 * wave;
  return r < 0 ? r + K : (r >= K ? r - K : r);
}

template <int KIND>
__global__ __launch_bounds__(256) __attribute__((amdgpu_waves_per_eu(1, 1)))
void gemmfr_kernel(const GemmArgs g) {
  static_assert(KIND == DEVIT_EPI_RESIDUAL_F32 || KIND == DEVIT_EPI_STORE_BF16, "the student's N = 384 launches");
  extern __shared__ __attribute__((aligned(16))) char smem[];
  constexpr int BM = 256, BN = 384, NWAVES = 4;
  constexpr bool PAIRED = KIND == DEVIT_EPI_STORE_BF16;
  constexpr int A_SLOT = BM * BK * 2, B_SLOT = BN * BK * 2, B_RING = 2 * A_SLOT;
  const int tid = threadIdx.x, lane = tid & 63;
  const int wave = __builtin_amdgcn_readfirstlane(tid >> 6);
  const int wm = wave >> 1, wn = wave & 1;

  const int xcd = blockIdx.x & 7, idx = blockIdx.x >> 3, stride = gridDim.x >> 3;
  int first, last;
  {
    const int q = g.total_tiles >> 3, r = g.total_tiles & 7;
    const int start = xcd * q + min(xcd, r);
    first = start + idx;
    last = start + q + (xcd < r ? 1 : 0);
  }
  if (first >= last) return;
#ifdef DEVIT_GEMMFR_STAMP
  const unsigned long long t_entry = __builtin_amdgcn_s_memtime();
  unsigned long long st_sum[6] = {0, 0, 0, 0, 0, 0};
#endif

  const unsigned lda64 = (unsigned)g.lda * 64u, ldbs = (unsigned)g.ldb * 128u, kb = (unsigned)g.K * (unsigned)g.ldb * 2u;
  const unsigned lds_base = (unsigned)(size_t)LDS_PTR(smem);
  const unsigned wldsa = lds_base + (unsigned)wave * 8192u, wldsb = lds_base + (unsigned)wave * 12288u;

  TileRef ct = decode_tile<BM, BN, false, true>(g, first);
#pragma unroll
  for (int st = 0; st < 2; ++st) {
    stage_tile<false, BM, NWAVES, true>(ct.a, g.lda, (ct.kt0 + st) * BK, 0, 0, smem + st * A_SLOT, wave, lane);
    const char* ub = (const char*)(ct.b + (size_t)fr_b_row(st, wave, g.K) * g.ldb);
    const unsigned lds0 = lds_base + (unsigned)(B_RING + st * B_SLOT) + (unsigned)wave * 12288u;
#pragma unroll
    for (int i = 0; i < 12; i += 2)
      dma2_uniform<false>(ub, fr_dma_off_b(g.ldb, wave, lane, i), fr_dma_off_b(g.ldb, wave, lane, i + 1), lds0 + i * 1024u);
  }
  wait_vmcnt<0>();
  __builtin_amdgcn_s_barrier();
  asm volatile("" ::: "memory");
  unsigned acur = 0;
  const unsigned wv = (unsigned)wave;
  const unsigned bv2 = (unsigned)fr_b_row(2, wave, g.K) * (unsigned)g.ldb * 2u;
  const unsigned bplo = (unsigned)(uintptr_t)ct.b, bphi = (unsigned)((uintptr_t)ct.b >> 32);
#ifdef DEVIT_GEMMFR_STAMP
  st_sum[5] = __builtin_amdgcn_s_memtime() - t_entry;
#endif

  for (int tile = first; tile < last; tile += stride) {
    const bool has_next = tile + stride < last;
    const TileRef nt = has_next ? decode_tile<BM, BN, false, true>(g, tile + stride) : ct;
    const __bf16* a_ptr = ct.a + (size_t)ct.kt0 * BK;
    const __bf16* a_next = nt.a + (size_t)nt.kt0 * BK;
    const unsigned nk = (unsigned)ct.nk, hasnext = (unsigned)__builtin_amdgcn_readfirstlane(has_next ? 1 : 0);
    const devit_epilogue& ep = g.ep;
    unsigned dsA[4], dsB[8], dmaA[4], dmaB[12];
    {
      int lane_k;
      asm volatile("v_mbcnt_lo_u32_b32 %0, -1, 0\n\tv_mbcnt_hi_u32_b32 %0, -1, %0" : "=v"(lane_k));
      const int c = lane_k & 15, gq = lane_k >> 4;
#pragma unroll
      for (int kk = 0; kk < 2; ++kk)
#pragma unroll
        for (int par = 0; par < 2; ++par) {
          const int rowA = wm * 128 + 16 * par + c;
          dsA[kk * 2 + par] = (unsigned)(rowA * 128 + (((kk * 4 + gq) ^ swz_row(rowA)) * 16));
        }
      const int q4 = (lane_k >> 2) & 3, p = lane_k & 3;
#pragma unroll
      for (int x3 = 0; x3 < 4; ++x3) {
        const unsigned row = (unsigned)((gq * 8 + q4) * (BN * 2) + 64 * (x3 ^ q4));
        if constexpr (PAIRED) {
          dsB[x3] = row + (unsigned)(16 * (p ^ ((gq & 1) << 1)));
          dsB[4 + x3] = 0;
        } else {
#pragma unroll
          for (int jp = 0; jp < 2; ++jp) dsB[2 * x3 + jp] = row + (unsigned)(32 * (jp ^ (gq & 1)) + 16 * (p >> 1) + 8 * (p & 1));
        }
      }
#pragma unroll
      for (int i = 0; i < 4; ++i) dsA[i] += lds_base;
#pragma unroll
      for (int i = 0; i < 8; ++i) dsB[i] += lds_base;
#pragma unroll
      for (int i = 0; i < 4; ++i) dmaA[i] = lane_offset<false, BM, NWAVES>(g.lda, wave, lane_k, i, BM);
#pragma unroll
      for (int i = 0; i < 12; ++i) dmaB[i] = fr_dma_off_b(g.ldb, wave, lane_k, i);
    }
    unsigned t0, t1, t2, t3, t4, t5, t6, t7, t8, t9;
    f32x32 c0, c1, c2, c3;
#ifdef DEVIT_GEMMFR_STAMP
    unsigned d1, d2;
    const unsigned long long ts0 = __builtin_amdgcn_s_memtime();
#define DEVIT_FR_STAMP_OUT , [d1] "=&s"(d1), [d2] "=&s"(d2)
#define DEVIT_FR_ASM(O) DEVIT_GEMMFR_KLOOP_##O##_STAMPED_ASM
#define DEVIT_FR_CLOB(O) DEVIT_GEMMFR_KLOOP_##O##_STAMPED_CLOBBERS
#else
#define DEVIT_FR_STAMP_OUT
#define DEVIT_FR_ASM(O) DEVIT_GEMMFR_KLOOP_##O##_ASM
#define DEVIT_FR_CLOB(O) DEVIT_GEMMFR_KLOOP_##O##_CLOBBERS
#endif
#define DEVIT_FR_STATEMENT(O)                                                                                                   \
    asm volatile(DEVIT_FR_ASM(O)                                                                                                \
                 : [c0] "=&{v[128:159]}"(c0), [c1] "=&{v[160:191]}"(c1), [c2] "=&{v[192:223]}"(c2), [c3] "=&{v[224:255]}"(c3),  \
                   [acur] "+s"(acur), [t0] "=&v"(t0), [t1] "=&v"(t1), [t2] "=&v"(t2), [t3] "=&v"(t3), [t4] "=&v"(t4),           \
                   [t5] "=&v"(t5), [t6] "=&v"(t6), [t7] "=&v"(t7), [t8] "=&v"(t8), [t9] "=&v"(t9) DEVIT_FR_STAMP_OUT            \
                 : [aptr] "s"(a_ptr), [anext] "s"(a_next), [bplo] "s"(bplo), [bphi] "s"(bphi), [bv2] "s"(bv2), [kb] "s"(kb),    \
                   [nk] "s"(nk), [hasnext] "s"(hasnext), [lda64] "s"(lda64), [ldbs] "s"(ldbs), [wldsa] "s"(wldsa),              \
                   [wldsb] "s"(wldsb), [wv] "s"(wv),                                                                            \
                   [dsa0] "v"(dsA[0]), [dsa1] "v"(dsA[1]), [dsa2] "v"(dsA[2]), [dsa3] "v"(dsA[3]),                              \
                   [dsb0] "v"(dsB[0]), [dsb1] "v"(dsB[1]), [dsb2] "v"(dsB[2]), [dsb3] "v"(dsB[3]),                              \
                   [dsb4] "v"(dsB[4]), [dsb5] "v"(dsB[5]), [dsb6] "v"(dsB[6]), [dsb7] "v"(dsB[7]),                              \
                   [dmaa0] "v"(dmaA[0]), [dmaa1] "v"(dmaA[1]), [dmaa2] "v"(dmaA[2]), [dmaa3] "v"(dmaA[3]),                      \
                   [dmab0] "v"(dmaB[0]), [dmab1] "v"(dmaB[1]), [dmab2] "v"(dmaB[2]), [dmab3] "v"(dmaB[3]),                      \
                   [dmab4] "v"(dmaB[4]), [dmab5] "v"(dmaB[5]), [dmab6] "v"(dmaB[6]), [dmab7] "v"(dmaB[7]),                      \
                   [dmab8] "v"(dmaB[8]), [dmab9] "v"(dmaB[9]), [dmab10] "v"(dmaB[10]), [dmab11] "v"(dmaB[11])                   \
                 : DEVIT_FR_CLOB(O))
    if constexpr (PAIRED) DEVIT_FR_STATEMENT(PAIRED);
    else DEVIT_FR_STATEMENT(NATURAL);
#undef DEVIT_FR_STATEMENT
#undef DEVIT_FR_STAMP_OUT
#undef DEVIT_FR_ASM
#undef DEVIT_FR_CLOB
#ifdef DEVIT_GEMMFR_STAMP
    const unsigned long long ts1 = __builtin_amdgcn_s_memtime();
    st_sum[0] += 1; st_sum[1] += ts1 - ts0; st_sum[3] += d1; st_sum[4] += d2;
#endif
    int lane_e;
    asm volatile("v_mbcnt_lo_u32_b32 %0, -1, 0\n\tv_mbcnt_hi_u32_b32 %0, -1, %0" : "=v"(lane_e));
    const size_t ob = (size_t)ct.bz * ep.out_batch_stride;
    const int m_lim = ep.m_valid > 0 ? ep.m_valid : g.M;
    const bool full = ct.m0 + BM <= m_lim;
    f32x4 cs[4];
    auto run = [&](f32x4 (&acc)[2][4], const int (&noff)[4], const f32x4 (&bias)[4], int i0) {
      const int mw = ct.m0 + wm * 128 + i0 * 16;
      if (full) epilogue_direct<KIND, 2, true, false>(ep, acc, noff, bias, cs, lane_e, mw, m_lim, ob);
      else epilogue_direct<KIND, 2, false, false>(ep, acc, noff, bias, cs, lane_e, mw, m_lim, ob);
    };
    {
      int noff[4];
      f32x4 bias[4];
      load_cols<KIND>(ep, lane_e, ct.n0 + wn * 192 + 128, noff, bias, cs);
      auto from_v = [&](const f32x32& c, int i0) {
        f32x4 acc[2][4];
#pragma unroll
        for (int u = 0; u < 2; ++u)
#pragma unroll
          for (int j = 0; j < 4; ++j)
            acc[u][j] = (f32x4){c[16 * u + 4 * j], c[16 * u + 4 * j + 1], c[16 * u + 4 * j + 2], c[16 * u + 4 * j + 3]};
        run(acc, noff, bias, i0);
      };
      from_v(c0, 0);
      from_v(c1, 2);
      from_v(c2, 4);
      from_v(c3, 6);
    }
    auto group = [&](auto hc) {
      constexpr int H = decltype(hc)::value;
      int noff[4];
      f32x4 bias[4];
      load_cols<KIND>(ep, lane_e, ct.n0 + wn * 192 + H * 64, noff, bias, cs);
      auto chunk = [&](auto ic) {
        constexpr int I0 = decltype(ic)::value;
        f32x4 acc[2][4];
        gemmfr_read_acc<H, I0>(acc);
        run(acc, noff, bias, I0);
      };
      chunk(std::integral_constant<int, 0>());
      chunk(std::integral_constant<int, 2>());
      chunk(std::integral_constant<int, 4>());
      chunk(std::integral_constant<int, 6>());
    };
    group(std::integral_constant<int, 0>());
    group(std::integral_constant<int, 1>());
#ifdef DEVIT_GEMMFR_STAMP
    st_sum[2] += __builtin_amdgcn_s_memtime() - ts1;
#endif
    ct = nt;
  }
  wait_vmcnt<0>();
#ifdef DEVIT_GEMMFR_STAMP
  if (g.ep.pos && lane == 0) {
    unsigned long long* dbg = (unsigned long long*)g.ep.pos + ((size_t)blockIdx.x * NWAVES + wave) * 8;
#pragma unroll
    for (int q = 0; q < 6; ++q) dbg[q] = st_sum[q];
    dbg[6] = t_entry; dbg[7] = __builtin_amdgcn_s_memtime();
  }
#endif
}

constexpr int WGRAD_MAX_JOBS = 48;
struct WgJob {
  const __bf16* a;
  const __bf16* b;
  float* out;
  float* colsum;
  int lda, ldb, ldc, a_cols, transposed, tile0;
};
struct WgArgs {
  WgJob job[WGRAD_MAX_JOBS];
  int njobs, tiles, split, nk_total, total;
  unsigned long long* dbg;
};

__global__ __launch_bounds__(256) __attribute__((amdgpu_waves_per_eu(1, 1)))
void wgradfr_kernel(const WgArgs g) {
  extern __shared__ __attribute__((aligned(16))) char smem[];
  constexpr int BM = 256, BN = 384, NWAVES = 4;
  constexpr int A_SLOT = BM * BK * 2, B_SLOT = BN * BK * 2, B_RING = 2 * A_SLOT;
  const int tid = threadIdx.x, lane = tid & 63;
  const int wave = __builtin_amdgcn_readfirstlane(tid >> 6);
  const int wm = wave >> 1, wn = wave & 1;

  int L;
  {
    const int xcd = blockIdx.x & 7, idx = blockIdx.x >> 3;
    const int q = g.total >> 3, r = g.total & 7;
    if (idx >= q + (xcd < r ? 1 : 0)) return;
    L = xcd * q + min(xcd, r) + idx;
  }
#ifdef DEVIT_GEMMFR_STAMP
  const unsigned long long t_entry = __builtin_amdgcn_s_memtime();
#endif
  const int z = L / g.tiles, t = L - z * g.tiles;
  int ji = 0;
  for (int j = 1; j < g.njobs; ++j)
    if (t >= g.job[j].tile0) ji = j;
  const WgJob& jb = g.job[ji];
  const int m0 = (t - jb.tile0) * BM;
  const int valid = min(BM, jb.a_cols - m0);
  const int kt0 = (int)((long long)z * g.nk_total / g.split);
  const int nk_i = (int)((long long)(z + 1) * g.nk_total / g.split) - kt0;
  const int lda = jb.lda, ldb = jb.ldb;
  const __bf16* a_tile = jb.a + (size_t)kt0 * BK * lda + m0;
  const __bf16* b_sl = jb.b + (size_t)kt0 * BK * ldb;
  const int Ks = nk_i * BK;

  const unsigned ldas = (unsigned)lda * 128u, ldbs = (unsigned)ldb * 128u, kb = (unsigned)Ks * (unsigned)ldb * 2u;
  const unsigned lds_base = (unsigned)(size_t)LDS_PTR(smem);
  const unsigned wldsa = lds_base + (unsigned)wave * 8192u, wldsb = lds_base + (unsigned)wave * 12288u;

#pragma unroll
  for (int st = 0; st < 2; ++st) {
    stage_tile<true, BM, NWAVES, true>(a_tile, lda, st * BK, 0, 0, smem + st * A_SLOT, wave, lane, valid);
    const char* ub = (const char*)(b_sl + (size_t)fr_b_row(st, wave, Ks) * ldb);
    const unsigned lds0 = lds_base + (unsigned)(B_RING + st * B_SLOT) + (unsigned)wave * 12288u;
#pragma unroll
    for (int i = 0; i < 12; i += 2)
      dma2_uniform<false>(ub, fr_dma_off_b(ldb, wave, lane, i), fr_dma_off_b(ldb, wave, lane, i + 1), lds0 + i * 1024u);
  }
  wait_vmcnt<0>();
  __builtin_amdgcn_s_barrier();
  asm volatile("" ::: "memory");
#ifdef DEVIT_GEMMFR_STAMP
  const unsigned long long t_primed = __builtin_amdgcn_s_memtime();
#endif
  unsigned acur = 0;
  const unsigned wv = (unsigned)wave, nk = (unsigned)nk_i;
  const unsigned bv2 = (unsigned)fr_b_row(2, wave, Ks) * (unsigned)ldb * 2u;
  const unsigned bplo = (unsigned)(uintptr_t)b_sl, bphi = (unsigned)((uintptr_t)b_sl >> 32);
  const unsigned ones = jb.colsum ? 0x3f803f80u : 0u;

  unsigned dsA[4], dsB[4], dmaA[8], dmaB[12];
  {
    int lane_k;
    asm volatile("v_mbcnt_lo_u32_b32 %0, -1, 0\n\tv_mbcnt_hi_u32_b32 %0, -1, %0" : "=v"(lane_k));
    const int gq = lane_k >> 4, q4 = (lane_k >> 2) & 3, p = lane_k & 3;
#pragma unroll
    for (int x = 0; x < 4; ++x) {
      dsA[x] = lds_base + (unsigned)((gq * 8 + q4) * (BM * 2) + 256 * wm + 64 * (x ^ q4) + 16 * (p ^ ((gq & 1) << 1)));
      dsB[x] = lds_base + (unsigned)((gq * 8 + q4) * (BN * 2) + 64 * (x ^ q4) + 16 * (p ^ ((gq & 1) << 1)));
    }
#pragma unroll
    for (int i = 0; i < 8; ++i) dmaA[i] = lane_offset<true, BM, NWAVES>(lda, wave, lane_k, i, valid);
#pragma unroll
    for (int i = 0; i < 12; ++i) dmaB[i] = fr_dma_off_b(ldb, wave, lane_k, i);
  }
  unsigned t0, t1, t2, t3, t4, t5, t6, t7;
  float rs0 = 0.f, rs1 = 0.f, rs2 = 0.f, rs3 = 0.f;
  f32x32 c0, c1, c2, c3;
#ifdef DEVIT_GEMMFR_STAMP
  unsigned d1, d2;
  const unsigned long long ts0 = __builtin_amdgcn_s_memtime();
#define DEVIT_WG_STAMP_OUT , [d1] "=&s"(d1), [d2] "=&s"(d2)
#define DEVIT_WG_ASM DEVIT_WGRADFR_KLOOP_STAMPED_ASM
#define DEVIT_WG_CLOB DEVIT_WGRADFR_KLOOP_STAMPED_CLOBBERS
#else
#define DEVIT_WG_STAMP_OUT
#define DEVIT_WG_ASM DEVIT_WGRADFR_KLOOP_ASM
#define DEVIT_WG_CLOB DEVIT_WGRADFR_KLOOP_CLOBBERS
#endif
  asm volatile(DEVIT_WG_ASM
               : [c0] "=&{v[128:159]}"(c0), [c1] "=&{v[160:191]}"(c1), [c2] "=&{v[192:223]}"(c2), [c3] "=&{v[224:255]}"(c3),
                 [acur] "+s"(acur), [t0] "=&v"(t0), [t1] "=&v"(t1), [t2] "=&v"(t2), [t3] "=&v"(t3), [t4] "=&v"(t4),
                 [t5] "=&v"(t5), [t6] "=&v"(t6), [t7] "=&v"(t7), [rs0] "+v"(rs0), [rs1] "+v"(rs1), [rs2] "+v"(rs2), [rs3] "+v"(rs3) DEVIT_WG_STAMP_OUT
               : [aptr] "s"(a_tile), [bplo] "s"(bplo), [bphi] "s"(bphi), [bv2] "s"(bv2), [kb] "s"(kb), [nk] "s"(nk), [ldas] "s"(ldas),
                 [ldbs] "s"(ldbs), [wldsa] "s"(wldsa), [wldsb] "s"(wldsb), [wv] "s"(wv), [ones] "s"(ones),
                 [dsa0] "v"(dsA[0]), [dsa1] "v"(dsA[1]), [dsa2] "v"(dsA[2]), [dsa3] "v"(dsA[3]),
                 [dsb0] "v"(dsB[0]), [dsb1] "v"(dsB[1]), [dsb2] "v"(dsB[2]), [dsb3] "v"(dsB[3]),
                 [dmaa0] "v"(dmaA[0]), [dmaa1] "v"(dmaA[1]), [dmaa2] "v"(dmaA[2]), [dmaa3] "v"(dmaA[3]),
                 [dmaa4] "v"(dmaA[4]), [dmaa5] "v"(dmaA[5]), [dmaa6] "v"(dmaA[6]), [dmaa7] "v"(dmaA[7]),
                 [dmab0] "v"(dmaB[0]), [dmab1] "v"(dmaB[1]), [dmab2] "v"(dmaB[2]), [dmab3] "v"(dmaB[3]),
                 [dmab4] "v"(dmaB[4]), [dmab5] "v"(dmaB[5]), [dmab6] "v"(dmaB[6]), [dmab7] "v"(dmaB[7]),
                 [dmab8] "v"(dmaB[8]), [dmab9] "v"(dmaB[9]), [dmab10] "v"(dmaB[10]), [dmab11] "v"(dmaB[11])
               : DEVIT_WG_CLOB);
#undef DEVIT_WG_STAMP_OUT
#undef DEVIT_WG_ASM
#undef DEVIT_WG_CLOB
#ifdef DEVIT_GEMMFR_STAMP
  const unsigned long long ts1 = __builtin_amdgcn_s_memtime();
#endif
  __syncthreads();
  int lane_e;
  asm volatile("v_mbcnt_lo_u32_b32 %0, -1, 0\n\tv_mbcnt_hi_u32_b32 %0, -1, %0" : "=v"(lane_e));
  constexpr int PITCH = 196;
  float* cw = (float*)smem + wave * (32 * PITCH);
  const int gq = lane_e >> 4, c = lane_e & 15;
  const bool wave_valid = wm * 128 < valid;
  float* wrow = cw + (8 * (c >> 2) + (c & 3)) * PITCH + 8 * gq;
  auto stage = [&](const f32x4 (&acc)[2][4], int H) {
#pragma unroll
    for (int u = 0; u < 2; ++u)
#pragma unroll
      for (int j = 0; j < 4; ++j) *(f32x4*)(wrow + 4 * u * PITCH + 32 * ((4 * H + j) >> 1) + 4 * (j & 1)) = acc[u][j];
  };
  auto flush = [&](int k) {
    asm volatile("s_waitcnt lgkmcnt(0)" ::: "memory");
    const int mb = m0 + wm * 128 + 32 * k;
    if (!jb.transposed) {
      float* o = jb.out + (size_t)mb * jb.ldc + wn * 192 + lane_e;
#pragma unroll 4
      for (int row = 0; row < 32; ++row) {
        const float* src = cw + row * PITCH + lane_e;
        const float v0 = src[0], v1 = src[64], v2 = src[128];
        float* d = o + (size_t)row * jb.ldc;
        unsafeAtomicAdd(d, v0);
        unsafeAtomicAdd(d + 64, v1);
        unsafeAtomicAdd(d + 128, v2);
      }
    } else {
      const int row = lane_e & 31, nsub = lane_e >> 5;
      float* o = jb.out + (size_t)(wn * 192 + nsub) * jb.ldc + mb + row;
      const float* src = cw + row * PITCH + nsub;
#pragma unroll 4
      for (int n2 = 0; n2 < 96; ++n2) unsafeAtomicAdd(o + (size_t)(2 * n2) * jb.ldc, src[2 * n2]);
    }
    asm volatile("s_waitcnt lgkmcnt(0)" ::: "memory");
  };
  auto from_v = [&](const f32x32& cv) {
    f32x4 acc[2][4];
#pragma unroll
    for (int u = 0; u < 2; ++u)
#pragma unroll
      for (int j = 0; j < 4; ++j)
        acc[u][j] = (f32x4){cv[16 * u + 4 * j], cv[16 * u + 4 * j + 1], cv[16 * u + 4 * j + 2], cv[16 * u + 4 * j + 3]};
    stage(acc, 2);
  };
  auto pass = [&](auto kc, const f32x32& cv) {
    constexpr int k = decltype(kc)::value;
    if (wave_valid) {
      from_v(cv);
      f32x4 acc[2][4];
      gemmfr_read_acc<0, 2 * k>(acc);
      stage(acc, 0);
      gemmfr_read_acc<1, 2 * k>(acc);
      stage(acc, 1);
      flush(k);
    }
  };
  pass(std::integral_constant<int, 0>(), c0);
  pass(std::integral_constant<int, 1>(), c1);
  pass(std::integral_constant<int, 2>(), c2);
  pass(std::integral_constant<int, 3>(), c3);
  if (jb.colsum && wave_valid) {
    float rs[4] = {rs0, rs1, rs2, rs3};
#pragma unroll
    for (int x = 0; x < 4; ++x) {
      float v = rs[x];
      v += __shfl_xor(v, 16, 64);
      v += __shfl_xor(v, 32, 64);
      const int i = 2 * x + wn;
      const int row = wm * 128 + 32 * (i >> 1) + 8 * (c >> 2) + 4 * (i & 1) + (c & 3);
      if (lane_e < 16) unsafeAtomicAdd(jb.colsum + m0 + row, v);
    }
  }
#ifdef DEVIT_GEMMFR_STAMP
  if (g.dbg && lane == 0) {
    unsigned long long* dbg = g.dbg + ((size_t)blockIdx.x * NWAVES + wave) * 8;
    const unsigned long long t_exit = __builtin_amdgcn_s_memtime();
    dbg[0] = nk; dbg[1] = t_primed - t_entry; dbg[2] = ts1 - ts0; dbg[3] = d1; dbg[4] = d2; dbg[5] = t_exit - ts1; dbg[6] = t_entry; dbg[7] = t_exit;
  }
#endif
}

bool aligned16(const void* p) { return (((uintptr_t)p) & 15) == 0; }

int g_reserved_cus = -1;

int reserved_cus() {
  if (g_reserved_cus < 0) {
    const char* e = getenv("DEVIT_RESERVE_CUS");
    int n = e ? atoi(e) : 0;
    g_reserved_cus = (n >= 0 && n <= 128) ? n / 8 * 8 : 0;
  }
  return g_reserved_cus;
}

}

extern "C" int devit_gemm_full_row_selected(int M, int N, int K, int kind) {
  if (!(M > 0 && M % 256 == 0 && N == 384 && K % BK == 0 && K / BK >= 3 && (kind == DEVIT_EPI_RESIDUAL_F32 || kind == DEVIT_EPI_STORE_BF16)))
    return 0;
  const char* e = getenv("DEVIT_GEMMFR");
  return (e && *e) ? atoi(e) != 0 : M / 256 >= 64;
}

#ifdef DEVIT_GEMMFR_STAMP
static unsigned long long* g_wgrad_dbg = nullptr;
extern "C" DEVIT_API void devit_wgrad_debug_buffer(void* p) { g_wgrad_dbg = (unsigned long long*)p; }
#endif

extern "C" int devit_wgrad_grouped(const devit_wgrad_job* jobs, int njobs, int K, int split_k, void* stream) {
  DEVIT_CHECK(jobs && njobs >= 1 && njobs <= WGRAD_MAX_JOBS, DEVIT_ERR_ARG, "devit_wgrad_grouped: 1..%d jobs (host array)", WGRAD_MAX_JOBS);
  DEVIT_CHECK(K > 0 && K % BK == 0, DEVIT_ERR_SHAPE, "devit_wgrad_grouped: K=%d must be a multiple of %d", K, BK);
  WgArgs g;
  int tiles = 0;
  for (int j = 0; j < njobs; ++j) {
    const devit_wgrad_job& q = jobs[j];
    DEVIT_CHECK(q.a && q.b && q.out, DEVIT_ERR_ARG, "devit_wgrad_grouped: job %d: null pointer", j);
    DEVIT_CHECK(q.a_cols > 0 && q.a_cols % 128 == 0 && q.lda >= q.a_cols && q.ldb >= 384 && q.lda % 8 == 0 && q.ldb % 8 == 0, DEVIT_ERR_SHAPE,
                "devit_wgrad_grouped: job %d: a_cols=%d (a multiple of 128) lda=%d ldb=%d (>= 384 columns are read)", j, q.a_cols, q.lda, q.ldb);
    DEVIT_CHECK(aligned16(q.a) && aligned16(q.b) && ((uintptr_t)q.out & 3) == 0 && q.ldc >= (q.transposed ? q.a_cols : 384), DEVIT_ERR_ARG,
                "devit_wgrad_grouped: job %d: operands must be 16-byte aligned, ldc=%d too small", j, q.ldc);
    g.job[j] = WgJob{(const __bf16*)q.a, (const __bf16*)q.b, q.out, q.a_colsum, q.lda, q.ldb, q.ldc, q.a_cols, q.transposed, tiles};
    tiles += (q.a_cols + 255) / 256;
  }
  static int cus = 0;
  if (cus == 0) {
    int dev = 0, n = 0;
    DEVIT_CHECK(hipGetDevice(&dev) == hipSuccess && hipDeviceGetAttribute(&n, hipDeviceAttributeMultiprocessorCount, dev) == hipSuccess && n >= 8,
                DEVIT_ERR_DEVICE, "devit_wgrad_grouped: cannot query the CU count");
    cus = n;
  }
  const int nk_total = K / BK;
  if (split_k <= 0) {
    const int avail = cus - reserved_cus() >= 8 ? cus - reserved_cus() : 8;
    int best = 1;
    double best_cost = 1e30;
    for (int sk = 1; sk <= 64 && nk_total / sk >= 3; ++sk) {
      const long long units = (long long)tiles * sk;
      const double rounds = (double)((units + avail - 1) / avail);
      const double cost = 2.1 * ((nk_total + sk - 1) / sk) * rounds + 0.30 * (double)units;
      if (cost < best_cost - 1e-9) {
        best_cost = cost;
        best = sk;
      }
    }
    split_k = best;
  }
  DEVIT_CHECK(split_k >= 1 && nk_total / split_k >= 3, DEVIT_ERR_SHAPE, "devit_wgrad_grouped: K=%d gives %d K-steps, fewer than 3 per slice at split_k=%d",
              K, nk_total, split_k);
  g.njobs = njobs; g.tiles = tiles; g.split = split_k; g.nk_total = nk_total; g.total = tiles * split_k;
#ifdef DEVIT_GEMMFR_STAMP
  g.dbg = g_wgrad_dbg;
#else
  g.dbg = nullptr;
#endif
  constexpr int lds = (256 + 384) * 128 * 2;
  static bool attr = false;
  if (!attr) {
    hipError_t e = hipFuncSetAttribute((const void*)wgradfr_kernel, hipFuncAttributeMaxDynamicSharedMemorySize, lds);
    DEVIT_CHECK(e == hipSuccess, DEVIT_ERR_LAUNCH, "hipFuncSetAttribute: %s", hipGetErrorString(e));
    attr = true;
  }
  hipLaunchKernelGGL(wgradfr_kernel, dim3((unsigned)((g.total + 7) / 8 * 8)), dim3(256), lds, (hipStream_t)stream, g);
  DEVIT_LAUNCH_CHECK();
  return DEVIT_OK;
}

extern "C" int devit_set_reserved_cus(int n) {
  DEVIT_CHECK(n >= 0 && n <= 128 && n % 8 == 0, DEVIT_ERR_ARG,
              "devit_set_reserved_cus: %d is not a multiple of 8 in [0, 128] (one share per XCD)", n);
  g_reserved_cus = n;
  return DEVIT_OK;
}

extern "C" int devit_get_reserved_cus(void) { return reserved_cus(); }

extern "C" int devit_gemm_bf16(const devit_operand* Aop, const devit_operand* Bop, int M, int N, int K, int batch,
                               int split_k, const devit_epilogue* ep, void* stream) {
  DEVIT_CHECK(Aop && Bop && Aop->ptr && Bop->ptr && ep && ep->out, DEVIT_ERR_ARG, "devit_gemm_bf16: null pointer");
  const void* A = Aop->ptr;
  const void* B = Bop->ptr;
  const int lda = Aop->ld, ldb = Bop->ld, a_kmajor = Aop->kmajor, b_kmajor = Bop->kmajor;
  DEVIT_CHECK(M > 0 && N > 0 && K > 0 && M % 128 == 0 && N % 128 == 0 && K % BK == 0 && batch >= 1, DEVIT_ERR_SHAPE,
              "devit_gemm_bf16: M=%d N=%d K=%d must be multiples of %d/%d/%d", M, N, K, 128, 128, BK);
  DEVIT_CHECK(lda % 8 == 0 && ldb % 8 == 0 && aligned16(A) && aligned16(B) && aligned16(ep->out) &&
                  ep->ldc % 8 == 0 && Aop->batch_stride % 8 == 0 && Bop->batch_stride % 8 == 0 &&
                  ep->out_batch_stride % 8 == 0,
              DEVIT_ERR_ARG, "devit_gemm_bf16: pointers / strides must be 16-byte aligned");
  DEVIT_CHECK(ep->kind >= DEVIT_EPI_STORE_BF16 && ep->kind <= DEVIT_EPI_STORE_F32, DEVIT_ERR_ARG,
              "devit_gemm_bf16: bad epilogue kind %d", ep->kind);
  DEVIT_CHECK(split_k >= 1 && (split_k == 1 || ep->kind == DEVIT_EPI_ATOMIC_F32) && split_k <= K / BK,
              DEVIT_ERR_ARG, "devit_gemm_bf16: split_k=%d only with ATOMIC_F32 and <= K/64", split_k);
  DEVIT_CHECK((a_kmajor ? lda >= M : lda >= K) && (b_kmajor ? ldb >= N : ldb >= K), DEVIT_ERR_ARG,
              "devit_gemm_bf16: leading dimension too small");
  DEVIT_CHECK((a_kmajor || Aop->row_group == 0) && (b_kmajor || Bop->row_group == 0), DEVIT_ERR_ARG,
              "devit_gemm_bf16: row_group/skip only for k-major operands");
  if (ep->kind == DEVIT_EPI_RESIDUAL_F32)
    DEVIT_CHECK(ep->res && (!ep->rowscale || ep->rows_per_scale > 0), DEVIT_ERR_ARG, "RESIDUAL: res / rows_per_scale");
  if (ep->kind == DEVIT_EPI_PATCH_F32)
    DEVIT_CHECK(ep->pos && ep->patch_tokens > 0 && (ep->m_valid > 0 ? ep->m_valid : M) % ep->patch_tokens == 0 && batch == 1,
                DEVIT_ERR_ARG,
                "PATCH: pos / tokens");
  if (ep->kind == DEVIT_EPI_DGELU_BF16)
    DEVIT_CHECK(ep->aux_in != nullptr && ep->bias == nullptr, DEVIT_ERR_ARG, "DGELU: needs aux_in, takes no bias (it is a dgrad)");
  if (ep->kind == DEVIT_EPI_ATOMIC_F32 && ep->aux)
    DEVIT_CHECK(batch == 1, DEVIT_ERR_ARG, "ATOMIC: the fused row sums of A (aux) need batch == 1");
  DEVIT_CHECK(ep->exact_gelu == 0, DEVIT_ERR_ARG, "devit_gemm_bf16: exact_gelu=1 (erff) is not built; the fused GELU is the "
              "fitted x * sigmoid(x * P(x^2)) form, |error| <= 2.6e-5 (devit_common.h); precision=\"f32\" uses erff");

  const bool f16 = ep->dtype16 != 0;
  DEVIT_CHECK(ep->dtype16 == 0 || ep->dtype16 == 1, DEVIT_ERR_ARG, "devit_gemm_bf16: dtype16 must be 0 (bf16) or 1 (f16)");
  DEVIT_CHECK(!f16 || (!a_kmajor && !b_kmajor && ep->kind != DEVIT_EPI_DGELU_BF16 && ep->kind != DEVIT_EPI_ATOMIC_F32),
              DEVIT_ERR_ARG, "devit_gemm_bf16: f16 operands are built for the forward layouts / epilogues only");
  GemmArgs g;
  g.A = (const __bf16*)A; g.B = (const __bf16*)B;
  g.lda = lda; g.ldb = ldb;
  g.a_group = Aop->row_group; g.a_skip = Aop->row_skip; g.b_group = Bop->row_group; g.b_skip = Bop->row_skip;
  g.a_bs = Aop->batch_stride; g.b_bs = Bop->batch_stride;
  g.M = M; g.N = N; g.K = K;
  g.tiles_m = 0; g.tiles_n = 0; g.split_k = split_k;
  g.ep = *ep;
  const int variant = (a_kmajor ? 2 : 0) + (b_kmajor ? 1 : 0);
  const bool f16_in = ep->dtype16 != 0;
  const bool light_epi = ep->kind == DEVIT_EPI_STORE_BF16 || ep->kind == DEVIT_EPI_STORE_F32;
  const bool gelu_epi = ep->kind == DEVIT_EPI_GELU_BF16 || ep->kind == DEVIT_EPI_DGELU_BF16;
  int cfg = 1;
  const bool ragged_ok = ((variant == 0 && (light_epi || ep->kind == DEVIT_EPI_GELU_BF16)) ||
                          (variant == 1 && ep->kind == DEVIT_EPI_DGELU_BF16)) && N % 256 == 128 && N >= 1024;
  const bool patch_wide = ep->kind == DEVIT_EPI_PATCH_F32 && K >= 768 && N % 256 == 0;
  const bool resid_wide = ep->kind == DEVIT_EPI_RESIDUAL_F32 && K >= 768 && N % 256 == 0 && variant == 0 && !f16_in;
  if (M % 256 == 0 && (N % 256 == 0 || ragged_ok) && (K >= 1536 || (K >= DEVIT_RAGGED_MIN_K && light_epi) || gelu_epi || patch_wide || resid_wide) && variant != 3) cfg = 3;
  if (cfg == 3 && (long long)(M / 256) * ((N + 255) / 256) * batch < 64) cfg = 1;
  static const int exact = getenv("DEVIT_GEMM_FORCE") ? atoi(getenv("DEVIT_GEMM_FORCE")) : 0;
  if (exact == 1 || (exact == 3 && M % 256 == 0 && (N % 256 == 0 || ragged_ok) && variant != 3)) cfg = exact;
  const bool b_dense = Bop->row_group == 0 && Bop->row_skip == 0;
  const bool use_fr = !f16 && split_k == 1 && batch == 1 && variant == 1 && b_dense && !(exact == 1 && ep->kind != DEVIT_EPI_RESIDUAL_F32) &&
                      devit_gemm_full_row_selected(M, N, K, ep->kind);
  DEVIT_CHECK(use_fr || !(variant == 1 && ep->kind == DEVIT_EPI_RESIDUAL_F32), DEVIT_ERR_ARG,
              "devit_gemm_bf16: the fp32 residual epilogue with a k-major weight runs on the full-row kernel only (N == 384, "
              "M %% 256 == 0, >= 64 row tiles, K >= 192, DEVIT_GEMMFR != 0, no row_group / row_skip on B): M=%d N=%d K=%d row_group=%d", M, N, K,
              Bop->row_group);
  if (use_fr) cfg = 4;
  const int bm = cfg == 1 ? 128 : 256, bn = cfg == 4 ? 384 : bm;
  g.tiles_m = M / bm;
  g.tiles_n = (N + bn - 1) / bn;
  {
    static const int gn_env = getenv("DEVIT_GEMM_GN") ? atoi(getenv("DEVIT_GEMM_GN")) : 0;
    const int per_xcd = (cfg == 1 ? 64 : 32);
    int target = 1;
    while ((target + 1) * (target + 1) * bn <= per_xcd * bm + (target + 1) * bn) ++target;
    const int nchunks = (g.tiles_n + target - 1) / target;
    g.gn = gn_env > 0 ? gn_env : (g.tiles_n + nchunks - 1) / nchunks;
    if (g.gn > g.tiles_n) g.gn = g.tiles_n;
  }
  const long long tiles = (long long)g.tiles_m * g.tiles_n * split_k * batch;
  DEVIT_CHECK(tiles < (1ll << 31), DEVIT_ERR_SHAPE, "devit_gemm_bf16: too many tiles");
  g.total_tiles = (int)tiles;
  g.d_per_z = make_fastdiv(g.tiles_m * g.tiles_n);
  g.d_chunk = make_fastdiv(g.gn * g.tiles_m);
  g.d_gn = make_fastdiv(g.gn);
  g.d_last = make_fastdiv(g.tiles_n % g.gn ? g.tiles_n % g.gn : g.gn);
  g.d_split = make_fastdiv(split_k);
  static int cus = 0;
  if (cus == 0) {
    int dev = 0, n = 0;
    DEVIT_CHECK(hipGetDevice(&dev) == hipSuccess &&
                    hipDeviceGetAttribute(&n, hipDeviceAttributeMultiprocessorCount, dev) == hipSuccess && n >= 8,
                DEVIT_ERR_DEVICE, "devit_gemm_bf16: cannot query the CU count");
    cus = n;
  }
  static const int occ_env = getenv("DEVIT_GEMM_OCC") ? atoi(getenv("DEVIT_GEMM_OCC")) : 0;
  const int occ = cfg == 4 ? 1 : occ_env > 0 ? occ_env : (cfg == 1 ? 2 : 1);
  const int avail = cus - reserved_cus() >= 8 ? cus - reserved_cus() : 8;
  long long nwg = ((long long)avail * occ) / 8 * 8;
  if (nwg > (tiles + 7) / 8 * 8) nwg = (tiles + 7) / 8 * 8;
  hipStream_t s = (hipStream_t)stream;
#define DEVIT_LAUNCH_ONE_T(BM_, BN_, WMM_, WNN_, NS_, AKM_, BKM_, KIND_, F16_)                                   \
  do {                                                                                                         \
    constexpr int ring = (3 * BM_ + 2 * BN_) * 128, stagebytes = WMM_ * WNN_ * 16384;                             \
    constexpr int lds = (KIND_ == DEVIT_EPI_ATOMIC_F32 && stagebytes > ring) ? stagebytes : ring;              \
    static bool attr = false;                                                                                  \
    if (!attr) {                                                                                               \
      hipError_t e = hipFuncSetAttribute((const void*)gemm_kernel<BM_, BN_, WMM_, WNN_, NS_, AKM_, BKM_, KIND_, F16_>, \
                                         hipFuncAttributeMaxDynamicSharedMemorySize, lds);                     \
      DEVIT_CHECK(e == hipSuccess, DEVIT_ERR_LAUNCH, "hipFuncSetAttribute: %s", hipGetErrorString(e));         \
      attr = true;                                                                                             \
    }                                                                                                          \
    hipLaunchKernelGGL((gemm_kernel<BM_, BN_, WMM_, WNN_, NS_, AKM_, BKM_, KIND_, F16_>), dim3((unsigned)nwg),  \
                       dim3(WMM_* WNN_ * 64), lds, s, g);                                                      \
  } while (0)
#define DEVIT_LAUNCH_ONE(BM_, BN_, WMM_, WNN_, NS_, AKM_, BKM_, KIND_) DEVIT_LAUNCH_ONE_T(BM_, BN_, WMM_, WNN_, NS_, AKM_, BKM_, KIND_, false)
#define DEVIT_LAUNCH_FWD16(BM_, BN_, WMM_, WNN_, NS_, KIND_)                                                   \
  do {                                                                                                         \
    if (f16) DEVIT_LAUNCH_ONE_T(BM_, BN_, WMM_, WNN_, NS_, false, false, KIND_, true);                         \
    else DEVIT_LAUNCH_ONE_T(BM_, BN_, WMM_, WNN_, NS_, false, false, KIND_, false);                            \
  } while (0)
#define DEVIT_LAUNCH_GEMM(BM_, BN_, WMM_, WNN_, NS_)                                                           \
  do {                                                                                                         \
    const int key = variant * 16 + ep->kind;                                                                   \
    switch (key) {                                                                                             \
      case 0 * 16 + DEVIT_EPI_STORE_BF16: DEVIT_LAUNCH_FWD16(BM_, BN_, WMM_, WNN_, NS_, DEVIT_EPI_STORE_BF16); break;       \
      case 0 * 16 + DEVIT_EPI_STORE_F32: DEVIT_LAUNCH_FWD16(BM_, BN_, WMM_, WNN_, NS_, DEVIT_EPI_STORE_F32); break;         \
      case 0 * 16 + DEVIT_EPI_GELU_BF16: DEVIT_LAUNCH_FWD16(BM_, BN_, WMM_, WNN_, NS_, DEVIT_EPI_GELU_BF16); break;         \
      case 0 * 16 + DEVIT_EPI_RESIDUAL_F32: DEVIT_LAUNCH_FWD16(BM_, BN_, WMM_, WNN_, NS_, DEVIT_EPI_RESIDUAL_F32); break;   \
      case 0 * 16 + DEVIT_EPI_PATCH_F32: DEVIT_LAUNCH_FWD16(BM_, BN_, WMM_, WNN_, NS_, DEVIT_EPI_PATCH_F32); break;         \
      case 1 * 16 + DEVIT_EPI_STORE_BF16: DEVIT_LAUNCH_ONE(BM_, BN_, WMM_, WNN_, NS_, false, true, DEVIT_EPI_STORE_BF16); break;        \
      case 1 * 16 + DEVIT_EPI_STORE_F32: DEVIT_LAUNCH_ONE(BM_, BN_, WMM_, WNN_, NS_, false, true, DEVIT_EPI_STORE_F32); break;          \
      case 1 * 16 + DEVIT_EPI_DGELU_BF16: DEVIT_LAUNCH_ONE(BM_, BN_, WMM_, WNN_, NS_, false, true, DEVIT_EPI_DGELU_BF16); break;        \
      case 3 * 16 + DEVIT_EPI_ATOMIC_F32:    \
      case 3 * 16 + DEVIT_EPI_STORE_F32:     \
        if (int rc_ = [&](auto small) -> int {                                                                 \
          if constexpr (decltype(small)::value) {                                                              \
            if (ep->kind == DEVIT_EPI_ATOMIC_F32) DEVIT_LAUNCH_ONE(BM_, BN_, WMM_, WNN_, NS_, true, true, DEVIT_EPI_ATOMIC_F32);  \
            else DEVIT_LAUNCH_ONE(BM_, BN_, WMM_, WNN_, NS_, true, true, DEVIT_EPI_STORE_F32);                  \
            return 0;                                                                                          \
          } else {                                                                                             \
            devit_set_error("devit_gemm_bf16: k-major x k-major operands run on 128x128 tiles only");          \
            return DEVIT_ERR_ARG;                                                                              \
          }                                                                                                    \
        }(std::integral_constant<bool, BM_ == 128>())) return rc_;                                             \
        break;                                                                                                 \
      default:                                                                                                 \
        DEVIT_CHECK(false, DEVIT_ERR_ARG, "devit_gemm_bf16: layout %d with epilogue %d is not instantiated", variant, ep->kind); \
    }                                                                                                          \
  } while (0)
  const char* gemm4_env = getenv("DEVIT_GEMM4");
  const bool gemm4_ok = cfg == 3 && variant == 0 && !f16 && N % 256 == 0 && K / BK >= 3 && split_k == 1 &&
                        ep->kind != DEVIT_EPI_DGELU_BF16 && ep->kind != DEVIT_EPI_ATOMIC_F32;
  const bool gemm4_pays = (ep->kind == DEVIT_EPI_STORE_BF16 || ep->kind == DEVIT_EPI_RESIDUAL_F32) && K >= 768 && batch == 1;
  const bool use4 = gemm4_ok && (gemm4_env ? atoi(gemm4_env) != 0 : gemm4_pays);
#define DEVIT_LAUNCH_GEMM4(KIND_)                                                                              \
  do {                                                                                                         \
    constexpr int lds = (3 * 256 + 2 * 256) * 128;                                                             \
    static bool attr = false;                                                                                  \
    if (!attr) {                                                                                               \
      hipError_t e = hipFuncSetAttribute((const void*)gemm4_kernel<KIND_, false>,                              \
                                         hipFuncAttributeMaxDynamicSharedMemorySize, lds);                     \
      DEVIT_CHECK(e == hipSuccess, DEVIT_ERR_LAUNCH, "hipFuncSetAttribute: %s", hipGetErrorString(e));         \
      attr = true;                                                                                             \
    }                                                                                                          \
    hipLaunchKernelGGL((gemm4_kernel<KIND_, false>), dim3((unsigned)nwg), dim3(256), lds, s, g);               \
  } while (0)
#define DEVIT_LAUNCH_GEMMFR(KIND_)                                                                              \
  do {                                                                                                         \
    constexpr int lds = (256 + 384) * 128 * 2;                                                                 \
    static bool attr = false;                                                                                  \
    if (!attr) {                                                                                               \
      hipError_t e = hipFuncSetAttribute((const void*)gemmfr_kernel<KIND_>,                                    \
                                         hipFuncAttributeMaxDynamicSharedMemorySize, lds);                     \
      DEVIT_CHECK(e == hipSuccess, DEVIT_ERR_LAUNCH, "hipFuncSetAttribute: %s", hipGetErrorString(e));         \
      attr = true;                                                                                             \
    }                                                                                                          \
    hipLaunchKernelGGL((gemmfr_kernel<KIND_>), dim3((unsigned)nwg), dim3(256), lds, s, g);                     \
  } while (0)
  if (cfg == 4) {
    if (ep->kind == DEVIT_EPI_STORE_BF16) DEVIT_LAUNCH_GEMMFR(DEVIT_EPI_STORE_BF16);
    else DEVIT_LAUNCH_GEMMFR(DEVIT_EPI_RESIDUAL_F32);
  } else if (use4) {
    switch (ep->kind) {
      case DEVIT_EPI_STORE_BF16: DEVIT_LAUNCH_GEMM4(DEVIT_EPI_STORE_BF16); break;
      case DEVIT_EPI_STORE_F32: DEVIT_LAUNCH_GEMM4(DEVIT_EPI_STORE_F32); break;
      case DEVIT_EPI_GELU_BF16: DEVIT_LAUNCH_GEMM4(DEVIT_EPI_GELU_BF16); break;
      case DEVIT_EPI_RESIDUAL_F32: DEVIT_LAUNCH_GEMM4(DEVIT_EPI_RESIDUAL_F32); break;
      case DEVIT_EPI_PATCH_F32: DEVIT_LAUNCH_GEMM4(DEVIT_EPI_PATCH_F32); break;
      default: DEVIT_CHECK(false, DEVIT_ERR_ARG, "devit_gemm_bf16: epilogue %d has no four-wave instantiation", ep->kind);
    }
  } else if (cfg == 3) DEVIT_LAUNCH_GEMM(256, 256, 2, 4, 2);
  else DEVIT_LAUNCH_GEMM(128, 128, 2, 2, 2);
#undef DEVIT_LAUNCH_GEMM4
#undef DEVIT_LAUNCH_GEMMFR
#undef DEVIT_LAUNCH_ONE
#undef DEVIT_LAUNCH_ONE_T
#undef DEVIT_LAUNCH_FWD16
#undef DEVIT_LAUNCH_GEMM
  DEVIT_LAUNCH_CHECK();
  return DEVIT_OK;
}
```

### devit_amd/csrc/layernorm.hip

```cpp
#include <type_traits>

#include "devit_common.h"

namespace {

constexpr int LN_MAX_NV = 8;

struct LnFwdArgs {
  const float* x;
  const float* gamma;
  const float* beta;
  __bf16* y_bf16;
  float* y_f32;
  float* mean;
  float* rstd;
  int rows, D, in_group, in_stride;
  float eps;
  int f16;
};

__device__ __forceinline__ size_t ln_in_row(int r, int group, int stride) {
  return group > 0 ? (size_t)(r / group) * stride + (r % group) : (size_t)r;
}

template <int NV, bool RAG = false>
__global__ __launch_bounds__(256) void ln_fwd_kernel(const LnFwdArgs a) {
  const int lane = threadIdx.x & 63, l32 = lane & 31, sub = lane >> 5;
  const int half_global = (blockIdx.x * 4 + (threadIdx.x >> 6)) * 2 + sub;
  const int nhalves = gridDim.x * 8;
  f32x4 gm[NV], bt[NV];
  bool ok[NV];
#pragma unroll
  for (int v = 0; v < NV; ++v) {
    ok[v] = !RAG || (v * 32 + l32) * 4 < a.D;
    gm[v] = ok[v] ? *(const f32x4*)(a.gamma + (v * 32 + l32) * 4) : (f32x4){0.f, 0.f, 0.f, 0.f};
    bt[v] = ok[v] ? *(const f32x4*)(a.beta + (v * 32 + l32) * 4) : (f32x4){0.f, 0.f, 0.f, 0.f};
  }
  const float invD = 1.0f / (float)a.D;
  const int trips = (a.rows + nhalves - 1) / nhalves;
  for (int it = 0; it < trips; ++it) {
    const int rr = half_global + it * nhalves;
    const bool live = rr < a.rows;
    const int r = live ? rr : a.rows - 1;
    const float* xr = a.x + ln_in_row(r, a.in_group, a.in_stride) * a.D;
    f32x4 xv[NV];
    float s = 0.f;
#pragma unroll
    for (int v = 0; v < NV; ++v) {
      xv[v] = ok[v] ? load_stream((const f32x4*)(xr + (v * 32 + l32) * 4)) : (f32x4){0.f, 0.f, 0.f, 0.f};
      s += (xv[v][0] + xv[v][1]) + (xv[v][2] + xv[v][3]);
    }
#pragma unroll
    for (int o = 16; o > 0; o >>= 1) s += __shfl_xor(s, o, 64);
    const float mu = s * invD;
    float q = 0.f;
#pragma unroll
    for (int v = 0; v < NV; ++v) {
#pragma unroll
      for (int e = 0; e < 4; ++e) {
        const float d = ok[v] ? xv[v][e] - mu : 0.f;
        q = fmaf(d, d, q);
      }
    }
#pragma unroll
    for (int o = 16; o > 0; o >>= 1) q += __shfl_xor(q, o, 64);
    const float rs = rsqrtf(q * invD + a.eps);
    if (!live) continue;
    if (l32 == 0) {
      if (a.mean) a.mean[r] = mu;
      if (a.rstd) a.rstd[r] = rs;
    }
#pragma unroll
    for (int v = 0; v < NV; ++v) {
      const f32x4 y = (xv[v] - mu) * rs * gm[v] + bt[v];
      const size_t o = (size_t)r * a.D + (v * 32 + l32) * 4;
      if (RAG && !ok[v]) continue;
      if (a.y_bf16) *(bf16x4*)(a.y_bf16 + o) = a.f16 ? cvt4<true>(y) : cvt4<false>(y);
      if (a.y_f32) *(f32x4*)(a.y_f32 + o) = y;
    }
  }
}

struct LnBwdArgs {
  const void* dy;
  const float* x;
  const float* mean;
  const float* rstd;
  const float* gamma;
  const float* dres;
  float* dx;
  __bf16* dx_bf16;
  const float* rowscale;
  int rows_per_scale;
  float* partial;
  int rows, D, in_group, in_stride, dy_is_f32;
};

template <int NV, bool RAG = false>
__global__ __launch_bounds__(256) void ln_bwd_kernel(const LnBwdArgs a) {
  __shared__ float red[4][3][NV * 128];
  const int lane = threadIdx.x & 63, wv = threadIdx.x >> 6, hl = lane & 31, half = lane >> 5;
  const int slot = (blockIdx.x * 4 + wv) * 2 + half;
  const int nslots = gridDim.x * 8;
  f32x4 gm[NV], dg[NV], db[NV], dsum[NV];
  bool ok[NV];
#pragma unroll
  for (int v = 0; v < NV; ++v) {
    ok[v] = !RAG || v * 128 + hl * 4 < a.D;
    gm[v] = ok[v] ? *(const f32x4*)(a.gamma + v * 128 + hl * 4) : (f32x4){0.f, 0.f, 0.f, 0.f};
    dg[v] = (f32x4){0.f, 0.f, 0.f, 0.f};
    db[v] = (f32x4){0.f, 0.f, 0.f, 0.f};
    dsum[v] = (f32x4){0.f, 0.f, 0.f, 0.f};
  }
  const float invD = 1.0f / (float)a.D;
  const int nit = (a.rows + nslots - 1) / nslots;
  for (int it = 0; it < nit; ++it) {
    const int r = slot + it * nslots;
    const bool live = r < a.rows;
    const size_t pr = ln_in_row(live ? r : 0, a.in_group, a.in_stride);
    const float* xr = a.x + pr * a.D;
    const float mu = live ? a.mean[r] : 0.f, rs = live ? a.rstd[r] : 0.f;
    f32x4 xh[NV], g[NV], dyv[NV];
    float s1 = 0.f, s2 = 0.f;
#pragma unroll
    for (int v = 0; v < NV; ++v) {
      const int c = v * 128 + hl * 4;
      f32x4 xv = {0.f, 0.f, 0.f, 0.f};
      dyv[v] = (f32x4){0.f, 0.f, 0.f, 0.f};
      if (live && ok[v]) {
        xv = load_stream((const f32x4*)(xr + c));
        if (a.dy_is_f32) {
          dyv[v] = load_stream((const f32x4*)((const float*)a.dy + (size_t)r * a.D + c));
        } else {
          const bf16x4 t = load_stream((const bf16x4*)((const __bf16*)a.dy + (size_t)r * a.D + c));
          dyv[v] = (f32x4){bf2f(t[0]), bf2f(t[1]), bf2f(t[2]), bf2f(t[3])};
        }
      }
      xh[v] = ok[v] ? (xv - mu) * rs : (f32x4){0.f, 0.f, 0.f, 0.f};
      g[v] = dyv[v] * gm[v];
      dg[v] += dyv[v] * xh[v];
      db[v] += dyv[v];
#pragma unroll
      for (int e = 0; e < 4; ++e) {
        s1 += g[v][e];
        s2 += g[v][e] * xh[v][e];
      }
    }
#pragma unroll
    for (int o = 16; o > 0; o >>= 1) {
      s1 += __shfl_xor(s1, o, 64);
      s2 += __shfl_xor(s2, o, 64);
    }
    const float m1 = s1 * invD, m2 = s2 * invD;
    if (live) {
      const float rsc = (a.dx_bf16 && a.rowscale) ? a.rowscale[pr / a.rows_per_scale] : 1.0f;
#pragma unroll
      for (int v = 0; v < NV; ++v) {
        const size_t o = pr * a.D + v * 128 + hl * 4;
        if (RAG && !ok[v]) continue;
        f32x4 d = rs * (g[v] - m1 - xh[v] * m2);
        if (a.dres) d += load_stream((const f32x4*)(a.dres + o));
        *(f32x4*)(a.dx + o) = d;
        if (a.dx_bf16) {
          const bf16x4 ob = {f2bf(d[0] * rsc), f2bf(d[1] * rsc), f2bf(d[2] * rsc), f2bf(d[3] * rsc)};
          *(bf16x4*)(a.dx_bf16 + o) = ob;
          dsum[v] += (f32x4){bf2f(ob[0]), bf2f(ob[1]), bf2f(ob[2]), bf2f(ob[3])};
        }
      }
    }
  }
#pragma unroll
  for (int v = 0; v < NV; ++v) {
#pragma unroll
    for (int e = 0; e < 4; ++e) {
      dg[v][e] += __shfl_xor(dg[v][e], 32, 64);
      db[v][e] += __shfl_xor(db[v][e], 32, 64);
      dsum[v][e] += __shfl_xor(dsum[v][e], 32, 64);
    }
    if (half == 0 && ok[v]) {
      *(f32x4*)&red[wv][0][v * 128 + hl * 4] = dg[v];
      *(f32x4*)&red[wv][1][v * 128 + hl * 4] = db[v];
      *(f32x4*)&red[wv][2][v * 128 + hl * 4] = dsum[v];
    }
  }
  __syncthreads();
  for (int i = threadIdx.x; i < 3 * a.D; i += 256) {
    const int which = i / a.D, c = i - which * a.D;
    a.partial[((size_t)blockIdx.x * 3 + which) * a.D + c] =
        red[0][which][c] + red[1][which][c] + red[2][which][c] + red[3][which][c];
  }
}

__global__ __launch_bounds__(1024) void colsum_partials_kernel(const float* partial, int nparts, int D, float* out0,
                                                               float* out1, float* out2, int accumulate) {
  __shared__ float red[32][33];
  const int ncols = 3 * D;
  const int cl = threadIdx.x & 31, grp = threadIdx.x >> 5;
  const int c = blockIdx.x * 32 + cl;
  float s = 0.f;
  if (c < ncols) {
#pragma unroll 4
    for (int p = grp; p < nparts; p += 32) s += partial[(size_t)p * ncols + c];
  }
  red[grp][cl] = s;
  __syncthreads();
  if (grp == 0 && c < ncols) {
    float t = 0.f;
#pragma unroll
    for (int i = 0; i < 32; ++i) t += red[i][cl];
    float* dst = c < D ? out0 + c : (c < 2 * D ? out1 + (c - D) : (out2 ? out2 + (c - 2 * D) : nullptr));
    if (dst) *dst = accumulate ? *dst + t : t;
  }
}

template <typename Args, typename F>
int dispatch_nv(int D, F&& f) {
  if (D % 128) {
    switch ((D + 127) / 128) {
      case 1: f(std::integral_constant<int, 1>(), std::true_type()); return 0;
      case 2: f(std::integral_constant<int, 2>(), std::true_type()); return 0;
      case 3: f(std::integral_constant<int, 3>(), std::true_type()); return 0;
      default: return -1;
    }
  }
  switch (D / 128) {
    case 1: f(std::integral_constant<int, 1>(), std::false_type()); return 0;
    case 2: f(std::integral_constant<int, 2>(), std::false_type()); return 0;
    case 3: f(std::integral_constant<int, 3>(), std::false_type()); return 0;
    case 4: f(std::integral_constant<int, 4>(), std::false_type()); return 0;
    case 6: f(std::integral_constant<int, 6>(), std::false_type()); return 0;
    case 8: f(std::integral_constant<int, 8>(), std::false_type()); return 0;
    default: return -1;
  }
}

}

extern "C" int devit_layernorm_fwd(const float* x, int rows, int D, int in_group, int in_stride,
                                   const float* gamma, const float* beta, float eps, void* y_bf16, float* y_f32,
                                   float* mean, float* rstd, int dtype16, void* stream) {
  DEVIT_CHECK(x && gamma && beta && (y_bf16 || y_f32), DEVIT_ERR_ARG, "devit_layernorm_fwd: null pointer");
  DEVIT_CHECK(dtype16 == 0 || dtype16 == 1, DEVIT_ERR_ARG, "devit_layernorm_fwd: dtype16 must be 0 (bf16) or 1 (f16)");
  DEVIT_CHECK(rows > 0 && D > 0 && D % 64 == 0 && D <= LN_MAX_NV * 128, DEVIT_ERR_SHAPE,
              "devit_layernorm_fwd: D=%d must be a multiple of 64 (of 128 above 384), <= 1024", D);
  LnFwdArgs a{x, gamma, beta, (__bf16*)y_bf16, y_f32, mean, rstd, rows, D, in_group, in_stride, eps, dtype16};
  const int grid = rows < 8 * 2048 ? (rows + 7) / 8 : 2048;
  int rc = dispatch_nv<LnFwdArgs>(D, [&](auto nv, auto rag) {
    hipLaunchKernelGGL((ln_fwd_kernel<decltype(nv)::value, decltype(rag)::value>), dim3(grid), dim3(256), 0, (hipStream_t)stream, a);
  });
  DEVIT_CHECK(rc == 0, DEVIT_ERR_SHAPE, "devit_layernorm_fwd: unsupported D=%d", D);
  DEVIT_LAUNCH_CHECK();
  return DEVIT_OK;
}

static int ln_bwd_grid(int rows) { return rows < 8 * 1024 ? (rows + 7) / 8 : 1024; }

extern "C" size_t devit_layernorm_bwd_workspace(int rows, int D) {
  return (size_t)ln_bwd_grid(rows) * 3 * D * sizeof(float);
}

extern "C" int devit_layernorm_bwd(const void* dy, int dy_is_f32, const float* x, int rows, int D, int in_group,
                                   int in_stride, const float* mean, const float* rstd, const float* gamma,
                                   const float* dres, float* dx, void* dx_bf16, const float* rowscale,
                                   int rows_per_scale, float* dgamma, float* dbeta, float* dx_bf16_colsum,
                                   int accumulate, void* workspace, size_t workspace_bytes, void* stream) {
  DEVIT_CHECK(dy && x && mean && rstd && gamma && dx && dgamma && dbeta && workspace, DEVIT_ERR_ARG,
              "devit_layernorm_bwd: null pointer");
  DEVIT_CHECK(rows > 0 && D > 0 && D % 64 == 0 && D <= LN_MAX_NV * 128, DEVIT_ERR_SHAPE, "devit_layernorm_bwd: D=%d", D);
  DEVIT_CHECK(workspace_bytes >= devit_layernorm_bwd_workspace(rows, D), DEVIT_ERR_ARG,
              "devit_layernorm_bwd: workspace too small");
  DEVIT_CHECK(!rowscale || rows_per_scale > 0, DEVIT_ERR_ARG, "devit_layernorm_bwd: rows_per_scale");
  DEVIT_CHECK(!dx_bf16_colsum || dx_bf16, DEVIT_ERR_ARG, "devit_layernorm_bwd: dx_bf16_colsum needs dx_bf16");
  const int grid = ln_bwd_grid(rows);
  LnBwdArgs a{dy, x, mean, rstd, gamma, dres, dx, (__bf16*)dx_bf16, rowscale, rows_per_scale,
              (float*)workspace, rows, D, in_group, in_stride, dy_is_f32};
  int rc = dispatch_nv<LnBwdArgs>(D, [&](auto nv, auto rag) {
    hipLaunchKernelGGL((ln_bwd_kernel<decltype(nv)::value, decltype(rag)::value>), dim3(grid), dim3(256), 0, (hipStream_t)stream, a);
  });
  DEVIT_CHECK(rc == 0, DEVIT_ERR_SHAPE, "devit_layernorm_bwd: unsupported D=%d", D);
  DEVIT_LAUNCH_CHECK();
  hipLaunchKernelGGL(colsum_partials_kernel, dim3((3 * D + 31) / 32), dim3(1024), 0, (hipStream_t)stream,
                     (const float*)workspace, grid, D, dgamma, dbeta, dx_bf16_colsum, accumulate);
  DEVIT_LAUNCH_CHECK();
  return DEVIT_OK;
}
```

### include/devit_hip.h

```cpp
#ifndef DEVIT_HIP_H
#define DEVIT_HIP_H

#include <stddef.h>
#include <stdint.h>

#ifdef __cplusplus
extern "C" {
#endif

#define DEVIT_ABI_VERSION 2
#define DEVIT_API __attribute__((visibility("default")))

enum {
  DEVIT_OK = 0,
  DEVIT_ERR_SHAPE = -1,
  DEVIT_ERR_ARG = -2,
  DEVIT_ERR_LAUNCH = -3,
  DEVIT_ERR_DEVICE = -4
};

DEVIT_API int devit_version(void);
DEVIT_API const char* devit_last_error(void);
DEVIT_API int devit_check_device(int dev);
DEVIT_API size_t devit_abi_struct_size(int which);

typedef enum {
  DEVIT_EPI_STORE_BF16 = 0,
  DEVIT_EPI_GELU_BF16 = 1,
  DEVIT_EPI_RESIDUAL_F32 = 2,
  DEVIT_EPI_PATCH_F32 = 3,
  DEVIT_EPI_DGELU_BF16 = 4,
  DEVIT_EPI_ATOMIC_F32 = 5,
  DEVIT_EPI_STORE_F32 = 6
} devit_epilogue_kind;

typedef struct {
  int kind;
  void* out;
  int ldc;
  const float* bias;
  const float* colscale;
  void* aux;
  const void* aux_in;
  const float* res;
  const float* rowscale;
  int rows_per_scale;
  const float* pos;
  int patch_tokens;
  int extra_tokens;
  int exact_gelu;
  long long out_batch_stride;
  int m_valid;
  int dtype16;
} devit_epilogue;

typedef struct {
  const void* ptr;
  int ld;
  int kmajor;
  int row_group, row_skip;
  long long batch_stride;
} devit_operand;

DEVIT_API int devit_gemm_bf16(const devit_operand* A, const devit_operand* B, int M, int N, int K, int batch, int split_k,
                    const devit_epilogue* ep, void* stream);
DEVIT_API int devit_gemm_full_row_selected(int M, int N, int K, int kind);
DEVIT_API int devit_set_reserved_cus(int n);
DEVIT_API int devit_get_reserved_cus(void);

typedef struct {
  const void* a;
  int lda, a_cols;
  const void* b;
  int ldb;
  float* out;
  int ldc, transposed;
  float* a_colsum;
} devit_wgrad_job;
DEVIT_API int devit_wgrad_grouped(const devit_wgrad_job* jobs, int njobs, int K, int split_k, void* stream);

DEVIT_API int devit_layernorm_fwd(const float* x, int rows, int D, int in_group, int in_stride, const float* gamma,
                        const float* beta, float eps, void* y_bf16, float* y_f32, float* mean, float* rstd,
                        int dtype16 , void* stream);
DEVIT_API size_t devit_layernorm_bwd_workspace(int rows, int D);
DEVIT_API int devit_layernorm_bwd(const void* dy, int dy_is_f32, const float* x, int rows, int D, int in_group, int in_stride,
                        const float* mean, const float* rstd, const float* gamma, const float* dres, float* dx,
                        void* dx_bf16, const float* rowscale, int rows_per_scale, float* dgamma, float* dbeta,
                        float* dx_bf16_colsum, int accumulate, void* workspace, size_t workspace_bytes, void* stream);

DEVIT_API int devit_attn_fwd(const void* qkv, void* out, float* lse, const float* head_gate, int B, int N, int H, int head_dim,
                   float scale, int dtype16 , void* stream);
DEVIT_API int devit_attn_bwd(const void* qkv, const void* out, const void* dout, const float* lse, const float* head_gate,
                   const void* dqkv_add, void* dqkv, int B, int N, int H, int head_dim, float scale, void* stream);
DEVIT_API int devit_attn_fwd_rows(const void* q, int q_ld, const void* kv, int kv_ld, void* out, float* lse, const float* head_gate,
                        int B, int NQ, int N, int H, int head_dim, float scale, int dtype16, void* stream);
DEVIT_API int devit_attn_bwd_rows(const void* q, int q_ld, const void* kv, int kv_ld, const void* out, const void* dout,
                        const float* lse, const float* head_gate, void* dq, int dq_ld, void* dkv, int dkv_ld, int B, int NQ,
                        int N, int H, int head_dim, float scale, void* stream);

typedef struct {
  const float *n1w, *n1b, *qkv_b, *proj_b, *n2w, *n2b, *fc1_b, *fc2_b;
  const void *qkv_w16, *proj_w16, *fc1_w16, *fc2_w16;
  const float *head_gate, *neuron_gate;
  int num_heads, attn_width, hidden;
  int dtype16;
  const void* fc2_w16t;
} devit_block_weights;

typedef struct {
  float *n1w, *n1b, *qkv_w, *qkv_b, *proj_w, *proj_b, *n2w, *n2b, *fc1_w, *fc1_b, *fc2_w, *fc2_b;
} devit_block_wgrads;

enum { DEVIT_ACT_LN1 = 0, DEVIT_ACT_MEAN1, DEVIT_ACT_RSTD1, DEVIT_ACT_QKV, DEVIT_ACT_ATTN_O, DEVIT_ACT_LSE, DEVIT_ACT_X1,
       DEVIT_ACT_ATT, DEVIT_ACT_LN2, DEVIT_ACT_MEAN2, DEVIT_ACT_RSTD2, DEVIT_ACT_H, DEVIT_ACT_H_PRE, DEVIT_ACT_X2,
       DEVIT_ACT_COUNT };
enum { DEVIT_BLK_SAVE = 1, DEVIT_BLK_QKV_PAD = 2, DEVIT_BLK_ATT = 4 };

typedef struct {
  const float* x;
  void* buf[DEVIT_ACT_COUNT];
  const float *dp1, *dp2;
  int flags;
} devit_block_acts;

enum { DEVIT_BWD_DH_PRE = 0, DEVIT_BWD_DLN2, DEVIT_BWD_DX1, DEVIT_BWD_G1, DEVIT_BWD_DATTN, DEVIT_BWD_DQKV, DEVIT_BWD_DLN1,
       DEVIT_BWD_LNWS, DEVIT_BWD_COUNT };

typedef struct {
  const float* dx;
  const void* g2;
  float* dx_in;
  void* g_prev;
  const float* prev_dp2;
  float* prev_fc2_b_grad;
  int g2_bias_done;
  const void* dqkv_add;
  void* ws[DEVIT_BWD_COUNT];
  size_t lnws_bytes;
  devit_wgrad_job* defer_jobs;
  int* defer_count;
} devit_block_bwd_io;

DEVIT_API int devit_block_acts_sizes(int B, int N, int D, int attn_width, int hidden, int flags, size_t* sizes );
DEVIT_API int devit_block_bwd_sizes(int B, int N, int D, int attn_width, int hidden, size_t* sizes );
DEVIT_API int devit_encoder_fwd(int nblocks, const devit_block_weights* w, const devit_block_acts* acts, int B, int N, int D,
                      float eps, void* stream);
DEVIT_API int devit_block_bwd(const devit_block_weights* w, const devit_block_acts* acts, const devit_block_wgrads* grads,
                    const devit_block_bwd_io* io, int B, int N, int D, float eps, void* stream);

typedef struct {
  const void* src;
  void* dst;
  const int* idx;
  int rows, cols;
  int src_ld, dst_ld;
  int mode;
  int elem;
} devit_index_job;
DEVIT_API int devit_index_copy(const devit_index_job* jobs_device, int njobs, int blocks_per_job, void* stream);

DEVIT_API int devit_im2row_bf16(const float* img, void* rows, int B, int C, int H, int W, int patch, int dtype16, void* stream);
DEVIT_API int devit_mix_im2row_bf16(const float* img, void* rows , void* rows_f16 , int B, int mode,
                          double lam, int y0, int y1, int x0, int x1, void* stream);
DEVIT_API int devit_mix_targets(const long long* labels, float* targets, int B, int C, double lam, double smoothing, void* stream);
DEVIT_API int devit_embed_tokens(const float* cls, const float* dist, const float* pos, float* x, int B, int T, int D,
                       void* stream);
DEVIT_API int devit_embed_bwd(const float* dx, int B, int T, int D, int ntok, float* dpos, float* dcls, float* ddist,
                    float* dbias, void* dx_bf16, int accumulate, void* stream);

DEVIT_API int devit_cast_bf16(const float* src, void* dst, size_t n, int dtype16, void* stream);

DEVIT_API int devit_scale_cast_bf16(const float* src, void* dst, const float* rowscale, int rows_per_scale, int M, int D,
                          void* stream);

DEVIT_API size_t devit_colsum_workspace(int M, int N);
DEVIT_API int devit_colsum_bf16(const void* y, int M, int N, int ld, int row_group, int row_skip, float* out, int accumulate,
                      void* workspace, size_t workspace_bytes, void* stream);

DEVIT_API int devit_sgemm_small(const float* A, long long sam, long long sak, const float* B, long long sbn, long long sbk,
                      const float* bias, float* C, int ldc, int M, int N, int K, float alpha, int accumulate,
                      void* stream);

DEVIT_API size_t devit_sumsq_workspace(void);
DEVIT_API int devit_sumsq_f32(const float* g, size_t n, float* out, void* workspace, size_t workspace_bytes, void* stream);
DEVIT_API int devit_adamw_step(float* p, const float* g, float* m, float* v, float* ema, void* p_bf16,
                     const unsigned char* no_decay4, const float* gnorm_sq, const float* dyn, size_t n, float beta1,
                     float beta2, float eps, float weight_decay, float max_norm, float ema_decay, float grad_scale,
                     void* stream);

DEVIT_API int devit_cls_distill_loss(const float* logits, const float* logits_kd, const float* teacher_logits,
                           const float* soft_targets, int B, int C, int kind, float alpha, float tau, float* loss3,
                           float* dlogits, float* dlogits_kd, void* stream);

DEVIT_API int devit_token_mse(const float* a, const float* b, size_t n, float* loss, float* da, int accumulate, void* stream);

DEVIT_API int devit_relation_stats(const float* gram_t, const float* gram_s, int B, int N, int ldr, int head_dim_t,
                         int head_dim_s, float* lse_t, float* lse_s, float* row_kl, float* loss, void* stream);
DEVIT_API int devit_relation_grad(const float* gram_t, const float* gram_s, const float* lse_t, const float* lse_s,
                        const float* upstream, int B, int N, int ldr, int head_dim_t, int head_dim_s, void* S_out,
                        int out_is_f32, void* stream);

DEVIT_API int devit_gemm_f32(const float* A, long long sam, long long sak, long long a_bs_outer, long long a_bs_inner,
                   const float* B, long long sbn, long long sbk, long long b_bs_outer, long long b_bs_inner, int M, int N,
                   int K, int batch, int batch_inner, long long c_bs_outer, long long c_bs_inner, int k_group, int k_skip,
                   float alpha, const float* batch_scale, int accumulate, const devit_epilogue* ep, void* stream);
DEVIT_API int devit_softmax_rows_f32(float* S, int rows, int ncols, int ld, float scale, float* lse, void* stream);
DEVIT_API int devit_softmax_bwd_rows_f32(const float* P, float* dP, int rows, int ncols, int ld, float scale, void* stream);
DEVIT_API int devit_im2row_f32(const float* img, float* rows, int B, void* stream);
DEVIT_API int devit_scale_rows_f32(const float* src, float* dst, const float* rowscale, int rows_per_scale, int M, int D,
                         void* stream);
DEVIT_API int devit_colsum_f32(const float* y, int M, int N, int ld, float* out, int accumulate, void* stream);

#define DEVIT_COMM_ID_BYTES 128
DEVIT_API int devit_comm_unique_id(void* id );
DEVIT_API int devit_comm_init(const void* id, int rank, int world, void** comm);
DEVIT_API int devit_comm_allreduce_f32(void* comm, float* buf, size_t count, void* stream);
DEVIT_API int devit_comm_destroy(void* comm);

#ifdef __cplusplus
}
#endif
#endif
```

Baseline: 11180 images/sec.

## Fuse fc1/qkv dgrad GEMM with LayerNorm backward in full-row kernel epilogue

Adds an LN-backward epilogue to the full-row (N=384) GEMM kernel. The dgrad output tile is staged in LDS, and the kernel computes the LayerNorm backward (dx, bf16 dx, dgamma/dbeta/colsum partials) before a separate finish reduction. The encoder backward uses this fused path for the fc1 and qkv dgrad when the shape qualifies. The aim is to avoid the round trip of the dln tensor through global memory and one kernel launch per site. In exchange the GEMM epilogue becomes longer and more register-heavy, and the path requires one tile per workgroup.

```diff
diff --git a/devit_amd/_lib.py b/devit_amd/_lib.py
--- a/devit_amd/_lib.py
+++ b/devit_amd/_lib.py
@@ -84,6 +84,8 @@
     "devit_layernorm_fwd": (_I, [_P, _I, _I, _I, _I, _P, _P, _F, _P, _P, _P, _P, _I, _P]),
     "devit_layernorm_bwd_workspace": (_Z, [_I, _I]),
     "devit_layernorm_bwd": (_I, [_P, _I, _P, _I, _I, _I, _I, _P, _P, _P, _P, _P, _P, _P, _I, _P, _P, _P, _I, _P, _Z, _P]),
+    "devit_dgrad_layernorm_bwd_fused": (_I, [_I, _I, _I]),
+    "devit_dgrad_layernorm_bwd": (_I, [_P, _P, _I, _I, _P, _P, _I, _I, _P, _P, _P, _P, _P, _P, _P, _I, _P, _P, _P, _I, _P, _Z, _P]),
     "devit_block_acts_sizes": (_I, [_I, _I, _I, _I, _I, _I, C.POINTER(C.c_size_t)]),
     "devit_block_bwd_sizes": (_I, [_I, _I, _I, _I, _I, C.POINTER(C.c_size_t)]),
     "devit_encoder_fwd": (_I, [_I, C.POINTER(BlockWeights), C.POINTER(BlockActs), _I, _I, _I, _F, _P]),
diff --git a/devit_amd/csrc/devit_common.h b/devit_amd/csrc/devit_common.h
--- a/devit_amd/csrc/devit_common.h
+++ b/devit_amd/csrc/devit_common.h
@@ -32,6 +32,9 @@
     }                                                                   \
   } while (0)
 
+
+int devit_layernorm_bwd_finish(const float* partial, int nparts, int D, float* dgamma, float* dbeta, float* dx_bf16_colsum,
+                               int accumulate, void* stream);
 
 __device__ __forceinline__ float bf2f(__bf16 v) { return (float)v; }
 __device__ __forceinline__ __bf16 f2bf(float v) { return (__bf16)v; }
diff --git a/devit_amd/csrc/encoder.hip b/devit_amd/csrc/encoder.hip
--- a/devit_amd/csrc/encoder.hip
+++ b/devit_amd/csrc/encoder.hip
@@ -304,21 +304,36 @@
     ep.aux_in = b[DEVIT_ACT_H_PRE];
     TRY(linear_dgrad(c, io->g2, w.fc2_w16, D, Hd, ep));
   }
-  TRY(linear_dgrad(c, dh_pre, w.fc1_w16, Hd, D, make_ep(DEVIT_EPI_STORE_BF16, dln2, D, c.M)));
-  TRY(wgrad(1, dh_pre, b[DEVIT_ACT_LN2], g.fc1_w, g.fc1_b, Hd, D));
-  TRY(devit_layernorm_bwd(dln2, 0, (const float*)b[DEVIT_ACT_X1], c.M, D, 0, 0, (const float*)b[DEVIT_ACT_MEAN2],
-                          (const float*)b[DEVIT_ACT_RSTD2], w.n2w, io->dx, dx1, g1, a.dp1, N, g.n2w, g.n2b, g.proj_b, 1,
-                          io->ws[DEVIT_BWD_LNWS], io->lnws_bytes, stream));
+  if (devit_dgrad_layernorm_bwd_fused(c.Mp, D, Hd)) {
+    TRY(devit_dgrad_layernorm_bwd(dh_pre, w.fc1_w16, c.Mp, Hd, dln2, (const float*)b[DEVIT_ACT_X1], c.M, D, (const float*)b[DEVIT_ACT_MEAN2],
+                                  (const float*)b[DEVIT_ACT_RSTD2], w.n2w, io->dx, dx1, g1, a.dp1, N, g.n2w, g.n2b, g.proj_b, 1,
+                                  io->ws[DEVIT_BWD_LNWS], io->lnws_bytes, stream));
+    TRY(wgrad(1, dh_pre, b[DEVIT_ACT_LN2], g.fc1_w, g.fc1_b, Hd, D));
+  } else {
+    TRY(linear_dgrad(c, dh_pre, w.fc1_w16, Hd, D, make_ep(DEVIT_EPI_STORE_BF16, dln2, D, c.M)));
+    TRY(wgrad(1, dh_pre, b[DEVIT_ACT_LN2], g.fc1_w, g.fc1_b, Hd, D));
+    TRY(devit_layernorm_bwd(dln2, 0, (const float*)b[DEVIT_ACT_X1], c.M, D, 0, 0, (const float*)b[DEVIT_ACT_MEAN2],
+                            (const float*)b[DEVIT_ACT_RSTD2], w.n2w, io->dx, dx1, g1, a.dp1, N, g.n2w, g.n2b, g.proj_b, 1,
+                            io->ws[DEVIT_BWD_LNWS], io->lnws_bytes, stream));
+  }
   TRY(linear_dgrad(c, g1, w.proj_w16, D, Da, make_ep(DEVIT_EPI_STORE_BF16, dattn, Da, c.M)));
   TRY(wgrad(2, g1, b[DEVIT_ACT_ATTN_O], g.proj_w, nullptr, D, Da));
   TRY(devit_attn_bwd(b[DEVIT_ACT_QKV], b[DEVIT_ACT_ATTN_O], dattn, (const float*)b[DEVIT_ACT_LSE], w.head_gate, io->dqkv_add,
                      dqkv, B, N, H, 64, 0.125f, stream));
-  TRY(linear_dgrad(c, dqkv, w.qkv_w16, 3 * Da, D, make_ep(DEVIT_EPI_STORE_BF16, dln1, D, c.M)));
-  TRY(wgrad(3, dqkv, b[DEVIT_ACT_LN1], g.qkv_w, g.qkv_b, 3 * Da, D));
-  TRY(flush(3));
-  TRY(devit_layernorm_bwd(dln1, 0, a.x, c.M, D, 0, 0, (const float*)b[DEVIT_ACT_MEAN1], (const float*)b[DEVIT_ACT_RSTD1],
-                          w.n1w, dx1, io->dx_in, io->g_prev, io->prev_dp2, N, g.n1w, g.n1b,
-                          io->g_prev ? io->prev_fc2_b_grad : nullptr, 1, io->ws[DEVIT_BWD_LNWS], io->lnws_bytes, stream));
+  if (devit_dgrad_layernorm_bwd_fused(c.Mp, D, 3 * Da)) {
+    TRY(devit_dgrad_layernorm_bwd(dqkv, w.qkv_w16, c.Mp, 3 * Da, dln1, a.x, c.M, D, (const float*)b[DEVIT_ACT_MEAN1],
+                                  (const float*)b[DEVIT_ACT_RSTD1], w.n1w, dx1, io->dx_in, io->g_prev, io->prev_dp2, N, g.n1w, g.n1b,
+                                  io->g_prev ? io->prev_fc2_b_grad : nullptr, 1, io->ws[DEVIT_BWD_LNWS], io->lnws_bytes, stream));
+    TRY(wgrad(3, dqkv, b[DEVIT_ACT_LN1], g.qkv_w, g.qkv_b, 3 * Da, D));
+    TRY(flush(3));
+  } else {
+    TRY(linear_dgrad(c, dqkv, w.qkv_w16, 3 * Da, D, make_ep(DEVIT_EPI_STORE_BF16, dln1, D, c.M)));
+    TRY(wgrad(3, dqkv, b[DEVIT_ACT_LN1], g.qkv_w, g.qkv_b, 3 * Da, D));
+    TRY(flush(3));
+    TRY(devit_layernorm_bwd(dln1, 0, a.x, c.M, D, 0, 0, (const float*)b[DEVIT_ACT_MEAN1], (const float*)b[DEVIT_ACT_RSTD1],
+                            w.n1w, dx1, io->dx_in, io->g_prev, io->prev_dp2, N, g.n1w, g.n1b,
+                            io->g_prev ? io->prev_fc2_b_grad : nullptr, 1, io->ws[DEVIT_BWD_LNWS], io->lnws_bytes, stream));
+  }
   return DEVIT_OK;
   }();
   if (sd && forked) {
diff --git a/devit_amd/csrc/gemm.hip b/devit_amd/csrc/gemm.hip
--- a/devit_amd/csrc/gemm.hip
+++ b/devit_amd/csrc/gemm.hip
@@ -3,6 +3,7 @@
 #include <type_traits>
 
 #include "devit_common.h"
+#include "ln_rows.h"
 
 namespace {
 
@@ -994,13 +995,30 @@
   return r < 0 ? r + K : (r >= K ? r - K : r);
 }
 
+constexpr int DEVIT_EPI_LNBWD = 64;
+template <int KIND>
+struct FrArgs {
+  GemmArgs g;
+};
+template <>
+struct FrArgs<DEVIT_EPI_LNBWD> {
+  GemmArgs g;
+  LnBwdArgs ln;
+};
+constexpr int LNF_PITCH = 832;
+constexpr int LNF_ROWS = 128;
+constexpr int LNF_RED = LNF_ROWS * LNF_PITCH;
+constexpr int LNF_SIDE = LNF_RED + 4 * 3 * 384 * 4, LNF_SIDE_PITCH = 272;
+static_assert(LNF_SIDE + LNF_ROWS * LNF_SIDE_PITCH <= (256 + 384) * 128 * 2, "the fused epilogue lives in the operand ring's LDS");
+
 template <int KIND>
 __global__ __launch_bounds__(256) __attribute__((amdgpu_waves_per_eu(1, 1)))
-void gemmfr_kernel(const GemmArgs g) {
-  static_assert(KIND == DEVIT_EPI_RESIDUAL_F32 || KIND == DEVIT_EPI_STORE_BF16, "the student's N = 384 launches");
+void gemmfr_kernel(const FrArgs<KIND> fa) {
+  static_assert(KIND == DEVIT_EPI_RESIDUAL_F32 || KIND == DEVIT_EPI_STORE_BF16 || KIND == DEVIT_EPI_LNBWD, "the student's N = 384 launches");
+  const GemmArgs& g = fa.g;
   extern __shared__ __attribute__((aligned(16))) char smem[];
   constexpr int BM = 256, BN = 384, NWAVES = 4;
-  constexpr bool PAIRED = KIND == DEVIT_EPI_STORE_BF16;
+  constexpr bool PAIRED = KIND != DEVIT_EPI_RESIDUAL_F32;
   constexpr int A_SLOT = BM * BK * 2, B_SLOT = BN * BK * 2, B_RING = 2 * A_SLOT;
   const int tid = threadIdx.x, lane = tid & 63;
   const int wave = __builtin_amdgcn_readfirstlane(tid >> 6);
@@ -1128,6 +1146,135 @@
     asm volatile("v_mbcnt_lo_u32_b32 %0, -1, 0\n\tv_mbcnt_hi_u32_b32 %0, -1, %0" : "=v"(lane_e));
     const size_t ob = (size_t)ct.bz * ep.out_batch_stride;
     const int m_lim = ep.m_valid > 0 ? ep.m_valid : g.M;
+    if constexpr (KIND == DEVIT_EPI_LNBWD) {
+      const LnBwdArgs& la = fa.ln;
+      const int gq = lane_e >> 4, c = lane_e & 15, hl = lane_e & 31, half = lane_e >> 5;
+      f32x4 cs[4];
+      float zf;
+      asm volatile("v_mov_b32 %0, 0" : "=v"(zf));
+      const f32x4 z4 = {zf, zf, zf, zf};
+      LnBwdCols<3> cols;
+      ln_bwd_cols_init<3, false>(la, hl, cols, z4);
+      float invD = 1.0f / 384.0f;
+      asm volatile("" : "+v"(invD));
+      const size_t zhi = (size_t)__builtin_bit_cast(unsigned, zf) << 32;
+      char* const srow = smem + (wm * 64 + c) * LNF_PITCH + (wn * 192 + 8 * gq) * 2;
+      char* const siderow = smem + LNF_SIDE + (wm * 64 + c) * LNF_SIDE_PITCH + (wn * 64 + 8 * gq) * 2;
+      auto put_v = [&](const f32x32& cv, int k) {
+        int noff[4];
+        f32x4 bias[4];
+        load_cols<DEVIT_EPI_STORE_BF16>(ep, lane_e, ct.n0 + wn * 192 + 128, noff, bias, cs);
+#pragma unroll
+        for (int u = 0; u < 2; ++u)
+#pragma unroll
+          for (int q = 0; q < 2; ++q) {
+            float x[8];
+#pragma unroll
+            for (int e = 0; e < 8; ++e) x[e] = cv[16 * u + 4 * (2 * q + (e >> 2)) + (e & 3)] + bias[2 * q + (e >> 2)][e & 3];
+            char* const dst = k < 2 ? srow + ((k & 1) * 32 + 16 * u) * LNF_PITCH + (128 + 32 * q) * 2
+                                    : siderow + ((k & 1) * 32 + 16 * u) * LNF_SIDE_PITCH + (32 * q) * 2;
+            *(bf16x8*)dst = pack8<false>(x);
+          }
+      };
+      auto put_a = [&](auto hc, auto ic) {
+        constexpr int H = decltype(hc)::value, I0 = decltype(ic)::value;
+        int noff[4];
+        f32x4 bias[4];
+        load_cols<DEVIT_EPI_STORE_BF16>(ep, lane_e, ct.n0 + wn * 192 + H * 64, noff, bias, cs);
+        f32x4 acc[2][4];
+        gemmfr_read_acc<H, I0>(acc);
+#pragma unroll
+        for (int u = 0; u < 2; ++u)
+#pragma unroll
+          for (int q = 0; q < 2; ++q) {
+            float x[8];
+#pragma unroll
+            for (int e = 0; e < 8; ++e) x[e] = acc[u][2 * q + (e >> 2)][e & 3] + bias[2 * q + (e >> 2)][e & 3];
+            *(bf16x8*)(srow + (((I0 >> 1) & 1) * 32 + 16 * u) * LNF_PITCH + (H * 64 + 32 * q) * 2) = pack8<false>(x);
+          }
+      };
+      constexpr int R = 2;
+      struct Pre {
+        f32x4 xv[3], dr[3];
+        float mu, rs, rsc;
+        int m;
+      };
+      auto fetch = [&](int q, Pre& p) {
+        const int lr = (q & 15) * 8 + wave * 2 + half;
+        const int m = ct.m0 + (lr >> 6) * 128 + 64 * (q >> 4) + (lr & 63);
+        const bool live = m < m_lim;
+        p.m = live ? m : -1;
+        p.rsc = (live && la.dx_bf16 && la.rowscale) ? la.rowscale[(unsigned)m / (unsigned)la.rows_per_scale] : 1.0f;
+        p.mu = live ? la.mean[m] : zf;
+        p.rs = live ? la.rstd[m] : zf;
+#pragma unroll
+        for (int v = 0; v < 3; ++v) {
+          const size_t o = (zhi | (unsigned)(live ? m : 0)) * 384 + v * 128 + hl * 4;
+          p.xv[v] = z4;
+          p.dr[v] = z4;
+          if (live) {
+            p.xv[v] = load_stream((const f32x4*)(la.x + o));
+            if (la.dres) p.dr[v] = load_stream((const f32x4*)(la.dres + o));
+          }
+        }
+      };
+      Pre cur[R], nxt[R];
+      auto ln_pass = [&](int P) {
+#pragma unroll 1
+        for (int t0 = 0; t0 < LNF_ROWS / 8; t0 += R) {
+          if (16 * P + t0 + R < 32) {
+#pragma unroll
+            for (int i = 0; i < R; ++i) fetch(16 * P + t0 + R + i, nxt[i]);
+          }
+#pragma unroll
+          for (int i = 0; i < R; ++i) {
+            const int lr = (t0 + i) * 8 + wave * 2 + half;
+            const bool live = cur[i].m >= 0;
+            LnBwdRow<3> in;
+            in.mu = cur[i].mu;
+            in.rs = cur[i].rs;
+#pragma unroll
+            for (int v = 0; v < 3; ++v) {
+              const int col = v * 128 + hl * 4;
+              in.xv[v] = cur[i].xv[v];
+              in.dyv[v] = z4;
+              if (live) {
+                const bool side = P == 1 && ((v == 1 && (col & 127) < 64) || (v == 2 && (col & 127) >= 64));
+                const char* src = side ? smem + LNF_SIDE + lr * LNF_SIDE_PITCH + ((v - 1) * 64 + (col & 63)) * 2 : smem + lr * LNF_PITCH + col * 2;
+                const bf16x4 t = *(const bf16x4*)src;
+                in.dyv[v] = (f32x4){bf2f(t[0]), bf2f(t[1]), bf2f(t[2]), bf2f(t[3])};
+              }
+            }
+            ln_bwd_row<3, false>(la, cols, in, live, zhi | (unsigned)(live ? cur[i].m : 0), lane_e, 384, invD, cur[i].rsc,
+                                 [&](int v, size_t) { return cur[i].dr[v]; });
+          }
+#pragma unroll
+          for (int i = 0; i < R; ++i) cur[i] = nxt[i];
+        }
+      };
+      wait_vmcnt<0>();
+      __syncthreads();
+#pragma unroll
+      for (int i = 0; i < R; ++i) fetch(i, cur[i]);
+      put_v(c0, 0);
+      put_v(c1, 1);
+      put_v(c2, 2);
+      put_v(c3, 3);
+      put_a(std::integral_constant<int, 0>(), std::integral_constant<int, 0>());
+      put_a(std::integral_constant<int, 1>(), std::integral_constant<int, 0>());
+      put_a(std::integral_constant<int, 0>(), std::integral_constant<int, 2>());
+      put_a(std::integral_constant<int, 1>(), std::integral_constant<int, 2>());
+      __syncthreads();
+      ln_pass(0);
+      __syncthreads();
+      put_a(std::integral_constant<int, 0>(), std::integral_constant<int, 4>());
+      put_a(std::integral_constant<int, 1>(), std::integral_constant<int, 4>());
+      put_a(std::integral_constant<int, 0>(), std::integral_constant<int, 6>());
+      put_a(std::integral_constant<int, 1>(), std::integral_constant<int, 6>());
+      __syncthreads();
+      ln_pass(1);
+      ln_bwd_cols_store<3>(la, cols, (float (*)[3][384])(smem + LNF_RED), wave, lane_e, 384, (size_t)tile);
+    } else {
     const bool full = ct.m0 + BM <= m_lim;
     f32x4 cs[4];
     auto run = [&](f32x4 (&acc)[2][4], const int (&noff)[4], const f32x4 (&bias)[4], int i0) {
@@ -1171,6 +1318,7 @@
     };
     group(std::integral_constant<int, 0>());
     group(std::integral_constant<int, 1>());
+    }
 #ifdef DEVIT_GEMMFR_STAMP
     st_sum[2] += __builtin_amdgcn_s_memtime() - ts1;
 #endif
@@ -1404,6 +1552,26 @@
   return g_reserved_cus;
 }
 
+int cu_count() {
+  static int cus = 0;
+  if (cus == 0) {
+    int dev = 0, n = 0;
+    if (hipGetDevice(&dev) == hipSuccess && hipDeviceGetAttribute(&n, hipDeviceAttributeMultiprocessorCount, dev) == hipSuccess && n >= 8) cus = n;
+  }
+  return cus;
+}
+long long persistent_grid(int cus, int occ) {
+  const int avail = cus - reserved_cus() >= 8 ? cus - reserved_cus() : 8;
+  return ((long long)avail * occ) / 8 * 8;
+}
+int gemm_force() {
+  static const int exact = getenv("DEVIT_GEMM_FORCE") ? atoi(getenv("DEVIT_GEMM_FORCE")) : 0;
+  return exact;
+}
+
+int gemm_launch(const devit_operand* Aop, const devit_operand* Bop, int M, int N, int K, int batch, int split_k, const devit_epilogue* ep,
+                const LnBwdArgs* ln, void* stream);
+
 }
 
 extern "C" int devit_gemm_full_row_selected(int M, int N, int K, int kind) {
@@ -1487,6 +1655,12 @@
 
 extern "C" int devit_gemm_bf16(const devit_operand* Aop, const devit_operand* Bop, int M, int N, int K, int batch,
                                int split_k, const devit_epilogue* ep, void* stream) {
+  return gemm_launch(Aop, Bop, M, N, K, batch, split_k, ep, nullptr, stream);
+}
+
+namespace {
+int gemm_launch(const devit_operand* Aop, const devit_operand* Bop, int M, int N, int K, int batch, int split_k, const devit_epilogue* ep,
+                const LnBwdArgs* ln, void* stream) {
   DEVIT_CHECK(Aop && Bop && Aop->ptr && Bop->ptr && ep && ep->out, DEVIT_ERR_ARG, "devit_gemm_bf16: null pointer");
   const void* A = Aop->ptr;
   const void* B = Bop->ptr;
@@ -1541,7 +1715,7 @@
   const bool resid_wide = ep->kind == DEVIT_EPI_RESIDUAL_F32 && K >= 768 && N % 256 == 0 && variant == 0 && !f16_in;
   if (M % 256 == 0 && (N % 256 == 0 || ragged_ok) && (K >= 1536 || (K >= DEVIT_RAGGED_MIN_K && light_epi) || gelu_epi || patch_wide || resid_wide) && variant != 3) cfg = 3;
   if (cfg == 3 && (long long)(M / 256) * ((N + 255) / 256) * batch < 64) cfg = 1;
-  static const int exact = getenv("DEVIT_GEMM_FORCE") ? atoi(getenv("DEVIT_GEMM_FORCE")) : 0;
+  const int exact = gemm_force();
   if (exact == 1 || (exact == 3 && M % 256 == 0 && (N % 256 == 0 || ragged_ok) && variant != 3)) cfg = exact;
   const bool b_dense = Bop->row_group == 0 && Bop->row_skip == 0;
   const bool use_fr = !f16 && split_k == 1 && batch == 1 && variant == 1 && b_dense && !(exact == 1 && ep->kind != DEVIT_EPI_RESIDUAL_F32) &&
@@ -1571,18 +1745,13 @@
   g.d_gn = make_fastdiv(g.gn);
   g.d_last = make_fastdiv(g.tiles_n % g.gn ? g.tiles_n % g.gn : g.gn);
   g.d_split = make_fastdiv(split_k);
-  static int cus = 0;
-  if (cus == 0) {
-    int dev = 0, n = 0;
-    DEVIT_CHECK(hipGetDevice(&dev) == hipSuccess &&
-                    hipDeviceGetAttribute(&n, hipDeviceAttributeMultiprocessorCount, dev) == hipSuccess && n >= 8,
-                DEVIT_ERR_DEVICE, "devit_gemm_bf16: cannot query the CU count");
-    cus = n;
-  }
+  const int cus = cu_count();
+  DEVIT_CHECK(cus >= 8, DEVIT_ERR_DEVICE, "devit_gemm_bf16: cannot query the CU count");
   static const int occ_env = getenv("DEVIT_GEMM_OCC") ? atoi(getenv("DEVIT_GEMM_OCC")) : 0;
   const int occ = cfg == 4 ? 1 : occ_env > 0 ? occ_env : (cfg == 1 ? 2 : 1);
-  const int avail = cus - reserved_cus() >= 8 ? cus - reserved_cus() : 8;
-  long long nwg = ((long long)avail * occ) / 8 * 8;
+  long long nwg = persistent_grid(cus, occ);
+  DEVIT_CHECK(!ln || (cfg == 4 && ep->kind == DEVIT_EPI_STORE_BF16 && tiles <= nwg), DEVIT_ERR_ARG,
+              "the fused dgrad + LayerNorm-backward launch needs the full-row kernel and one tile per workgroup: M=%d K=%d", M, K);
   if (nwg > (tiles + 7) / 8 * 8) nwg = (tiles + 7) / 8 * 8;
   hipStream_t s = (hipStream_t)stream;
 #define DEVIT_LAUNCH_ONE_T(BM_, BN_, WMM_, WNN_, NS_, AKM_, BKM_, KIND_, F16_)                                   \
@@ -1661,11 +1830,19 @@
       DEVIT_CHECK(e == hipSuccess, DEVIT_ERR_LAUNCH, "hipFuncSetAttribute: %s", hipGetErrorString(e));         \
       attr = true;                                                                                             \
     }                                                                                                          \
-    hipLaunchKernelGGL((gemmfr_kernel<KIND_>), dim3((unsigned)nwg), dim3(256), lds, s, g);                     \
+    hipLaunchKernelGGL((gemmfr_kernel<KIND_>), dim3((unsigned)nwg), dim3(256), lds, s, fa);                    \
   } while (0)
   if (cfg == 4) {
-    if (ep->kind == DEVIT_EPI_STORE_BF16) DEVIT_LAUNCH_GEMMFR(DEVIT_EPI_STORE_BF16);
-    else DEVIT_LAUNCH_GEMMFR(DEVIT_EPI_RESIDUAL_F32);
+    if (ln) {
+      FrArgs<DEVIT_EPI_LNBWD> fa{g, *ln};
+      DEVIT_LAUNCH_GEMMFR(DEVIT_EPI_LNBWD);
+    } else if (ep->kind == DEVIT_EPI_STORE_BF16) {
+      FrArgs<DEVIT_EPI_STORE_BF16> fa{g};
+      DEVIT_LAUNCH_GEMMFR(DEVIT_EPI_STORE_BF16);
+    } else {
+      FrArgs<DEVIT_EPI_RESIDUAL_F32> fa{g};
+      DEVIT_LAUNCH_GEMMFR(DEVIT_EPI_RESIDUAL_F32);
+    }
   } else if (use4) {
     switch (ep->kind) {
       case DEVIT_EPI_STORE_BF16: DEVIT_LAUNCH_GEMM4(DEVIT_EPI_STORE_BF16); break;
@@ -1686,3 +1863,42 @@
   DEVIT_LAUNCH_CHECK();
   return DEVIT_OK;
 }
+}
+
+extern "C" int devit_dgrad_layernorm_bwd_fused(int M_pad, int D, int K) {
+  const char* e = getenv("DEVIT_LNFUSE");
+  if (e && *e && atoi(e) == 0) return 0;
+  if (D != 384 || gemm_force() == 1 || !devit_gemm_full_row_selected(M_pad, D, K, DEVIT_EPI_STORE_BF16)) return 0;
+  const int cus = cu_count();
+  return cus >= 8 && M_pad / 256 <= persistent_grid(cus, 1);
+}
+
+extern "C" int devit_dgrad_layernorm_bwd(const void* dy, const void* w, int M_pad, int K, void* dln, const float* x, int rows, int D,
+                                         const float* mean, const float* rstd, const float* gamma, const float* dres, float* dx,
+                                         void* dx_bf16, const float* rowscale, int rows_per_scale, float* dgamma, float* dbeta,
+                                         float* dx_bf16_colsum, int accumulate, void* workspace, size_t workspace_bytes, void* stream) {
+  DEVIT_CHECK(dy && w && dln && rows > 0 && rows <= M_pad, DEVIT_ERR_ARG, "devit_dgrad_layernorm_bwd: bad argument");
+  devit_operand A = {dy, K, 0, 0, 0, 0}, Bo = {w, D, 1, 0, 0, 0};
+  devit_epilogue ep = {};
+  ep.kind = DEVIT_EPI_STORE_BF16;
+  ep.out = dln;
+  ep.ldc = D;
+  ep.m_valid = rows;
+  if (!devit_dgrad_layernorm_bwd_fused(M_pad, D, K)) {
+    int rc = devit_gemm_bf16(&A, &Bo, M_pad, D, K, 1, 1, &ep, stream);
+    if (rc != DEVIT_OK) return rc;
+    return devit_layernorm_bwd(dln, 0, x, rows, D, 0, 0, mean, rstd, gamma, dres, dx, dx_bf16, rowscale, rows_per_scale, dgamma, dbeta,
+                               dx_bf16_colsum, accumulate, workspace, workspace_bytes, stream);
+  }
+  DEVIT_CHECK(x && mean && rstd && gamma && dx && dgamma && dbeta && workspace, DEVIT_ERR_ARG, "devit_dgrad_layernorm_bwd: null pointer");
+  DEVIT_CHECK(workspace_bytes >= devit_layernorm_bwd_workspace(rows, D), DEVIT_ERR_ARG, "devit_dgrad_layernorm_bwd: workspace too small");
+  DEVIT_CHECK(!rowscale || rows_per_scale > 0, DEVIT_ERR_ARG, "devit_dgrad_layernorm_bwd: rows_per_scale");
+  DEVIT_CHECK(!dx_bf16_colsum || dx_bf16, DEVIT_ERR_ARG, "devit_dgrad_layernorm_bwd: dx_bf16_colsum needs dx_bf16");
+  DEVIT_CHECK(aligned16(x) && aligned16(dx) && (!dres || aligned16(dres)) && (!dx_bf16 || aligned16(dx_bf16)), DEVIT_ERR_ARG,
+              "devit_dgrad_layernorm_bwd: x / dres / dx / dx_bf16 must be 16-byte aligned");
+  const int tiles = M_pad / 256;
+  LnBwdArgs ln{nullptr, x, mean, rstd, gamma, dres, dx, (__bf16*)dx_bf16, rowscale, rows_per_scale, (float*)workspace, rows, D, 0, 0, 0};
+  int rc = gemm_launch(&A, &Bo, M_pad, D, K, 1, 1, &ep, &ln, stream);
+  if (rc != DEVIT_OK) return rc;
+  return devit_layernorm_bwd_finish((const float*)workspace, tiles, D, dgamma, dbeta, dx_bf16_colsum, accumulate, stream);
+}
diff --git a/devit_amd/csrc/layernorm.hip b/devit_amd/csrc/layernorm.hip
--- a/devit_amd/csrc/layernorm.hip
+++ b/devit_amd/csrc/layernorm.hip
@@ -1,6 +1,7 @@
 #include <type_traits>
 
 #include "devit_common.h"
+#include "ln_rows.h"
 
 namespace {
 
@@ -19,10 +20,6 @@
   int f16;
 };
 
-__device__ __forceinline__ size_t ln_in_row(int r, int group, int stride) {
-  return group > 0 ? (size_t)(r / group) * stride + (r % group) : (size_t)r;
-}
-
 template <int NV, bool RAG = false>
 __global__ __launch_bounds__(256) void ln_fwd_kernel(const LnFwdArgs a) {
   const int lane = threadIdx.x & 63, l32 = lane & 31, sub = lane >> 5;
@@ -81,37 +78,14 @@
   }
 }
 
-struct LnBwdArgs {
-  const void* dy;
-  const float* x;
-  const float* mean;
-  const float* rstd;
-  const float* gamma;
-  const float* dres;
-  float* dx;
-  __bf16* dx_bf16;
-  const float* rowscale;
-  int rows_per_scale;
-  float* partial;
-  int rows, D, in_group, in_stride, dy_is_f32;
-};
-
 template <int NV, bool RAG = false>
 __global__ __launch_bounds__(256) void ln_bwd_kernel(const LnBwdArgs a) {
   __shared__ float red[4][3][NV * 128];
   const int lane = threadIdx.x & 63, wv = threadIdx.x >> 6, hl = lane & 31, half = lane >> 5;
   const int slot = (blockIdx.x * 4 + wv) * 2 + half;
   const int nslots = gridDim.x * 8;
-  f32x4 gm[NV], dg[NV], db[NV], dsum[NV];
-  bool ok[NV];
-#pragma unroll
-  for (int v = 0; v < NV; ++v) {
-    ok[v] = !RAG || v * 128 + hl * 4 < a.D;
-    gm[v] = ok[v] ? *(const f32x4*)(a.gamma + v * 128 + hl * 4) : (f32x4){0.f, 0.f, 0.f, 0.f};
-    dg[v] = (f32x4){0.f, 0.f, 0.f, 0.f};
-    db[v] = (f32x4){0.f, 0.f, 0.f, 0.f};
-    dsum[v] = (f32x4){0.f, 0.f, 0.f, 0.f};
-  }
+  LnBwdCols<NV> s;
+  ln_bwd_cols_init<NV, RAG>(a, hl, s);
   const float invD = 1.0f / (float)a.D;
   const int nit = (a.rows + nslots - 1) / nslots;
   for (int it = 0; it < nit; ++it) {
@@ -119,76 +93,28 @@
     const bool live = r < a.rows;
     const size_t pr = ln_in_row(live ? r : 0, a.in_group, a.in_stride);
     const float* xr = a.x + pr * a.D;
-    const float mu = live ? a.mean[r] : 0.f, rs = live ? a.rstd[r] : 0.f;
-    f32x4 xh[NV], g[NV], dyv[NV];
-    float s1 = 0.f, s2 = 0.f;
+    LnBwdRow<NV> in;
+    in.mu = live ? a.mean[r] : 0.f;
+    in.rs = live ? a.rstd[r] : 0.f;
 #pragma unroll
     for (int v = 0; v < NV; ++v) {
       const int c = v * 128 + hl * 4;
-      f32x4 xv = {0.f, 0.f, 0.f, 0.f};
-      dyv[v] = (f32x4){0.f, 0.f, 0.f, 0.f};
-      if (live && ok[v]) {
-        xv = load_stream((const f32x4*)(xr + c));
+      in.xv[v] = (f32x4){0.f, 0.f, 0.f, 0.f};
+      in.dyv[v] = (f32x4){0.f, 0.f, 0.f, 0.f};
+      if (live && s.ok[v]) {
+        in.xv[v] = load_stream((const f32x4*)(xr + c));
         if (a.dy_is_f32) {
-          dyv[v] = load_stream((const f32x4*)((const float*)a.dy + (size_t)r * a.D + c));
+          in.dyv[v] = load_stream((const f32x4*)((const float*)a.dy + (size_t)r * a.D + c));
         } else {
           const bf16x4 t = load_stream((const bf16x4*)((const __bf16*)a.dy + (size_t)r * a.D + c));
-          dyv[v] = (f32x4){bf2f(t[0]), bf2f(t[1]), bf2f(t[2]), bf2f(t[3])};
+          in.dyv[v] = (f32x4){bf2f(t[0]), bf2f(t[1]), bf2f(t[2]), bf2f(t[3])};
         }
       }
-      xh[v] = ok[v] ? (xv - mu) * rs : (f32x4){0.f, 0.f, 0.f, 0.f};
-      g[v] = dyv[v] * gm[v];
-      dg[v] += dyv[v] * xh[v];
-      db[v] += dyv[v];
-#pragma unroll
-      for (int e = 0; e < 4; ++e) {
-        s1 += g[v][e];
-        s2 += g[v][e] * xh[v][e];
-      }
-    }
-#pragma unroll
-    for (int o = 16; o > 0; o >>= 1) {
-      s1 += __shfl_xor(s1, o, 64);
-      s2 += __shfl_xor(s2, o, 64);
-    }
-    const float m1 = s1 * invD, m2 = s2 * invD;
-    if (live) {
-      const float rsc = (a.dx_bf16 && a.rowscale) ? a.rowscale[pr / a.rows_per_scale] : 1.0f;
-#pragma unroll
-      for (int v = 0; v < NV; ++v) {
-        const size_t o = pr * a.D + v * 128 + hl * 4;
-        if (RAG && !ok[v]) continue;
-        f32x4 d = rs * (g[v] - m1 - xh[v] * m2);
-        if (a.dres) d += load_stream((const f32x4*)(a.dres + o));
-        *(f32x4*)(a.dx + o) = d;
-        if (a.dx_bf16) {
-          const bf16x4 ob = {f2bf(d[0] * rsc), f2bf(d[1] * rsc), f2bf(d[2] * rsc), f2bf(d[3] * rsc)};
-          *(bf16x4*)(a.dx_bf16 + o) = ob;
-          dsum[v] += (f32x4){bf2f(ob[0]), bf2f(ob[1]), bf2f(ob[2]), bf2f(ob[3])};
-        }
-      }
-    }
-  }
-#pragma unroll
-  for (int v = 0; v < NV; ++v) {
-#pragma unroll
-    for (int e = 0; e < 4; ++e) {
-      dg[v][e] += __shfl_xor(dg[v][e], 32, 64);
-      db[v][e] += __shfl_xor(db[v][e], 32, 64);
-      dsum[v][e] += __shfl_xor(dsum[v][e], 32, 64);
-    }
-    if (half == 0 && ok[v]) {
-      *(f32x4*)&red[wv][0][v * 128 + hl * 4] = dg[v];
-      *(f32x4*)&red[wv][1][v * 128 + hl * 4] = db[v];
-      *(f32x4*)&red[wv][2][v * 128 + hl * 4] = dsum[v];
-    }
-  }
-  __syncthreads();
-  for (int i = threadIdx.x; i < 3 * a.D; i += 256) {
-    const int which = i / a.D, c = i - which * a.D;
-    a.partial[((size_t)blockIdx.x * 3 + which) * a.D + c] =
-        red[0][which][c] + red[1][which][c] + red[2][which][c] + red[3][which][c];
-  }
+    }
+    const float rsc = (live && a.dx_bf16 && a.rowscale) ? a.rowscale[pr / a.rows_per_scale] : 1.0f;
+    ln_bwd_row<NV, RAG>(a, s, in, live, pr, lane, a.D, invD, rsc, [&](int, size_t o) { return load_stream((const f32x4*)(a.dres + o)); });
+  }
+  ln_bwd_cols_store<NV>(a, s, red, wv, lane, a.D, blockIdx.x);
 }
 
 __global__ __launch_bounds__(1024) void colsum_partials_kernel(const float* partial, int nparts, int D, float* out0,
@@ -279,8 +205,13 @@
   });
   DEVIT_CHECK(rc == 0, DEVIT_ERR_SHAPE, "devit_layernorm_bwd: unsupported D=%d", D);
   DEVIT_LAUNCH_CHECK();
-  hipLaunchKernelGGL(colsum_partials_kernel, dim3((3 * D + 31) / 32), dim3(1024), 0, (hipStream_t)stream,
-                     (const float*)workspace, grid, D, dgamma, dbeta, dx_bf16_colsum, accumulate);
+  return devit_layernorm_bwd_finish((const float*)workspace, grid, D, dgamma, dbeta, dx_bf16_colsum, accumulate, stream);
+}
+
+int devit_layernorm_bwd_finish(const float* partial, int nparts, int D, float* dgamma, float* dbeta, float* dx_bf16_colsum,
+                               int accumulate, void* stream) {
+  hipLaunchKernelGGL(colsum_partials_kernel, dim3((3 * D + 31) / 32), dim3(1024), 0, (hipStream_t)stream, partial, nparts, D, dgamma,
+                     dbeta, dx_bf16_colsum, accumulate);
   DEVIT_LAUNCH_CHECK();
   return DEVIT_OK;
 }
diff --git a/devit_amd/csrc/ln_rows.h b/devit_amd/csrc/ln_rows.h
--- /dev/null
+++ b/devit_amd/csrc/ln_rows.h
@@ -0,0 +1,157 @@
+#pragma once
+#include "devit_common.h"
+
+struct LnBwdArgs {
+  const void* dy;
+  const float* x;
+  const float* mean;
+  const float* rstd;
+  const float* gamma;
+  const float* dres;
+  float* dx;
+  __bf16* dx_bf16;
+  const float* rowscale;
+  int rows_per_scale;
+  float* partial;
+  int rows, D, in_group, in_stride, dy_is_f32;
+};
+
+__device__ __forceinline__ size_t ln_in_row(int r, int group, int stride) {
+  return group > 0 ? (size_t)(r / group) * stride + (r % group) : (size_t)r;
+}
+
+template <int NV>
+struct LnBwdCols {
+  f32x4 gm[NV], dg[NV], db[NV], dsum[NV];
+  bool ok[NV];
+};
+
+template <int NV>
+struct LnBwdRow {
+  f32x4 xv[NV], dyv[NV];
+  float mu, rs;
+};
+
+template <int NV, bool RAG>
+__device__ __forceinline__ void ln_bwd_cols_init(const LnBwdArgs& a, int hl, LnBwdCols<NV>& s, f32x4 zero = (f32x4){0.f, 0.f, 0.f, 0.f}) {
+#pragma unroll
+  for (int v = 0; v < NV; ++v) {
+    s.ok[v] = !RAG || v * 128 + hl * 4 < a.D;
+    s.gm[v] = s.ok[v] ? *(const f32x4*)(a.gamma + v * 128 + hl * 4) : zero;
+    s.dg[v] = zero;
+    s.db[v] = zero;
+    s.dsum[v] = zero;
+  }
+}
+
+__device__ __forceinline__ float ln_shfl_xor(float v, int o, int lane) {
+  return __builtin_bit_cast(float, __builtin_amdgcn_ds_bpermute((lane ^ o) << 2, __builtin_bit_cast(int, v)));
+}
+
+template <int NV, bool RAG>
+struct LnBwdMath {
+  static __device__ __forceinline__ void sums(const LnBwdRow<NV>& in, LnBwdCols<NV>& s, f32x4 (&xh)[NV], f32x4 (&g)[NV], float& s1, float& s2) {
+#pragma unroll
+    for (int v = 0; v < NV; ++v) {
+      xh[v] = s.ok[v] ? (in.xv[v] - in.mu) * in.rs : (f32x4){0.f, 0.f, 0.f, 0.f};
+      g[v] = in.dyv[v] * s.gm[v];
+      s.dg[v] += in.dyv[v] * xh[v];
+      s.db[v] += in.dyv[v];
+#pragma unroll
+      for (int e = 0; e < 4; ++e) {
+        s1 += g[v][e];
+        s2 += g[v][e] * xh[v][e];
+      }
+    }
+  }
+  static __device__ __forceinline__ f32x4 dx(int v, const f32x4& g, const f32x4& xh, float s1, float s2, float invD, float rs) {
+    const float m1 = s1 * invD, m2 = s2 * invD;
+    return rs * (g - m1 - xh * m2);
+  }
+};
+template <>
+struct LnBwdMath<3, false> {
+  static __device__ __forceinline__ void sums(const LnBwdRow<3>& in, LnBwdCols<3>& s, f32x4 (&xh)[3], f32x4 (&g)[3], float& s1, float& s2) {
+#pragma clang fp contract(off)
+#pragma unroll
+    for (int v = 0; v < 3; ++v) {
+#pragma unroll
+      for (int e = 0; e < 4; ++e) {
+        xh[v][e] = (in.xv[v][e] - in.mu) * in.rs;
+        g[v][e] = in.dyv[v][e] * s.gm[v][e];
+        s.dg[v][e] = __builtin_fmaf(in.dyv[v][e], xh[v][e], s.dg[v][e]);
+        s.db[v][e] += in.dyv[v][e];
+        s1 += g[v][e];
+        s2 = __builtin_fmaf(g[v][e], xh[v][e], s2);
+      }
+    }
+  }
+  static __device__ __forceinline__ f32x4 dx(int v, const f32x4& g, const f32x4& xh, float s1, float s2, float invD, float rs) {
+#pragma clang fp contract(off)
+    const float m1 = s1 * invD, m2 = s2 * invD;
+    f32x4 d;
+#pragma unroll
+    for (int e = 0; e < 4; ++e) {
+      const float t = v == 0 ? __builtin_fmaf(-invD, s1, g[e]) : g[e] - m1;
+      d[e] = rs * __builtin_fmaf(-m2, xh[e], t);
+    }
+    return d;
+  }
+};
+
+template <int NV, bool RAG, typename DRES>
+__device__ __forceinline__ void ln_bwd_row(const LnBwdArgs& a, LnBwdCols<NV>& s, const LnBwdRow<NV>& in, bool live, size_t pr, int lane,
+                                           int D, float invD, float rsc, DRES&& dres_at) {
+  const int hl = lane & 31;
+  f32x4 xh[NV], g[NV];
+  float s1 = 0.f, s2 = 0.f;
+  LnBwdMath<NV, RAG>::sums(in, s, xh, g, s1, s2);
+#pragma unroll
+  for (int o = 16; o > 0; o >>= 1) {
+    s1 += ln_shfl_xor(s1, o, lane);
+    s2 += ln_shfl_xor(s2, o, lane);
+  }
+  if (live) {
+#pragma unroll
+    for (int v = 0; v < NV; ++v) {
+      const size_t o = pr * D + v * 128 + hl * 4;
+      if (RAG && !s.ok[v]) continue;
+      f32x4 d = LnBwdMath<NV, RAG>::dx(v, g[v], xh[v], s1, s2, invD, in.rs);
+      if (a.dres) {
+        asm volatile("" : "+v"(d));
+        d += dres_at(v, o);
+      }
+      *(f32x4*)(a.dx + o) = d;
+      if (a.dx_bf16) {
+        const bf16x4 ob = {f2bf(d[0] * rsc), f2bf(d[1] * rsc), f2bf(d[2] * rsc), f2bf(d[3] * rsc)};
+        *(bf16x4*)(a.dx_bf16 + o) = ob;
+        s.dsum[v] += (f32x4){bf2f(ob[0]), bf2f(ob[1]), bf2f(ob[2]), bf2f(ob[3])};
+      }
+    }
+  }
+}
+
+template <int NV>
+__device__ __forceinline__ void ln_bwd_cols_store(const LnBwdArgs& a, LnBwdCols<NV>& s, float (*red)[3][NV * 128], int wv, int lane,
+                                                  int D, size_t part) {
+  const int hl = lane & 31, half = lane >> 5, tid = wv * 64 + lane;
+#pragma unroll
+  for (int v = 0; v < NV; ++v) {
+#pragma unroll
+    for (int e = 0; e < 4; ++e) {
+      s.dg[v][e] += ln_shfl_xor(s.dg[v][e], 32, lane);
+      s.db[v][e] += ln_shfl_xor(s.db[v][e], 32, lane);
+      s.dsum[v][e] += ln_shfl_xor(s.dsum[v][e], 32, lane);
+    }
+    if (half == 0 && s.ok[v]) {
+      *(f32x4*)&red[wv][0][v * 128 + hl * 4] = s.dg[v];
+      *(f32x4*)&red[wv][1][v * 128 + hl * 4] = s.db[v];
+      *(f32x4*)&red[wv][2][v * 128 + hl * 4] = s.dsum[v];
+    }
+  }
+  __syncthreads();
+  for (int i = tid; i < 3 * D; i += 256) {
+    const int which = i / D, c = i - which * D;
+    a.partial[(part * 3 + which) * D + c] = red[0][which][c] + red[1][which][c] + red[2][which][c] + red[3][which][c];
+  }
+}
diff --git a/include/devit_hip.h b/include/devit_hip.h
--- a/include/devit_hip.h
+++ b/include/devit_hip.h
@@ -88,6 +88,12 @@
                         void* dx_bf16, const float* rowscale, int rows_per_scale, float* dgamma, float* dbeta,
                         float* dx_bf16_colsum, int accumulate, void* workspace, size_t workspace_bytes, void* stream);
 
+DEVIT_API int devit_dgrad_layernorm_bwd_fused(int M_pad, int D, int K);
+DEVIT_API int devit_dgrad_layernorm_bwd(const void* dy, const void* w, int M_pad, int K, void* dln, const float* x, int rows, int D,
+                        const float* mean, const float* rstd, const float* gamma, const float* dres, float* dx, void* dx_bf16,
+                        const float* rowscale, int rows_per_scale, float* dgamma, float* dbeta, float* dx_bf16_colsum,
+                        int accumulate, void* workspace, size_t workspace_bytes, void* stream);
+
 DEVIT_API int devit_attn_fwd(const void* qkv, void* out, float* lse, const float* head_gate, int B, int N, int H, int head_dim,
                    float scale, int dtype16 , void* stream);
 DEVIT_API int devit_attn_bwd(const void* qkv, const void* out, const void* dout, const float* lse, const float* head_gate,
```

Measured after the change: 11380 images/sec (median of 6 runs). +1.8%, better.
